# ChanukyaVardhan/Video-Moment-Localization

Measured on AMD Instinct MI355X. Metric: proposals/sec (fwd+bwd), higher is better.
Workload: dtype f32; 1 GPU; activitynet_t256: SMIN T=256 L=64 C=4 d=512 dl=128 Nq=20 Din=500 layers=3, batch 64/GPU, default init seed 43; step = zero_grad+fwd+restated loss+bwd+Adam (torch fused); global_batch=64, parallelism=dp1, dist_world_size=1

## Files before the change

### include/smin_hip.h

```cpp
#ifndef SMIN_HIP_H
#define SMIN_HIP_H
#include <stddef.h>
#include <stdint.h>

#ifdef __cplusplus
extern "C" {
#endif

#define SMIN_HIP_ABI_VERSION 2

int smin_abi_version(void);
int smin_set_gemm_mode(int mode);
int smin_get_gemm_mode(void);
#define SMIN_PROF_MOMENT_FWD 1
#define SMIN_PROF_MOMENT_DX 2
#define SMIN_PROF_MOMENT_DW 3
#define SMIN_PROF_ATTN_FWD 4
#define SMIN_PROF_ATTN_BWD 5
int smin_prof_enable(int on);
int smin_prof_read(int32_t* tags, float* ms, int cap);
const char* smin_target_arch(void);
size_t smin_workspace_bytes(int N, int B, int C, int D, int dl, int Nq);

int smin_proposal_map_fwd(void* stream, const float* f, const int32_t* cells, int N, int B, int T, int L, int C, int D,
                          float* fc, float* fm, float* fb, void* ws, size_t ws_bytes );
int smin_clip_event_table(void* stream, int T, int L, int C, int32_t* counts, const int32_t* offsets, void* table);
int smin_proposal_map_bwd(void* stream, const float* dfc, const float* dfm, const float* dfb,
                          const int32_t* cells, const int32_t* row_ptr, const int32_t* cellmap,
                          int N, int B, int T, int L, int C, int D, float* df, void* ws, size_t ws_bytes,
                          const int32_t* ev_offsets, const void* ev_table);

int smin_gate_fwd(void* stream, const float* fm, const float* fs, const int32_t* cells, int N, int D, float* hbar);
int smin_gate_fwd_sum(void* stream, const float* fm, const float* fs, const int32_t* cells, int N, int D, float* hbar, const float* hsum_in,
                      float* hsum_out);
int smin_gate_bwd(void* stream, const float* const* dhbar, int n_dhbar, const float* const* dres, int n_dres,
                  const float* fm, const float* fs, const int32_t* row_ptr,
                  int N, int B, int L, int D, float* dfm, float* dfs, void* ws, size_t ws_bytes,
                  const int32_t* cells, const float* boundary_A, const float* boundary_dout);

int smin_content_unit_fwd(void* stream, const float* fc, const float* hbar, const int32_t* cells, const int32_t* row_ptr,
                          int N, int B, int L, int C, int D, int dl, int Nq,
                          const float* Wch, const float* bch, const float* Mq, const float* uq,
                          const float* what, const float* shat, const float* qmask, const float* Wc, const float* bc,
                          const float* fcmean_in, int last,
                          float* fc_out, float* fcmean, float* chat, float* cchat);
int smin_content_unit_bwd(void* stream, const float* dfc_out, const float* dfcmean,
                          const float* fc, const int32_t* cells, const int32_t* row_ptr,
                          int N, int B, int L, int C, int D, int dl, int Nq,
                          const float* WchT, const float* Mq, const float* uq,
                          const float* what, const float* shat, const float* qmask, const float* WcT,
                          const float* chat, const float* cchat,
                          float* dfc, float* dhbar, float* dWch, float* dbch, float* dMq, float* duq,
                          float* dwhat, float* dshat, float* dWc, float* dbc, void* ws, size_t ws_bytes, int last);

int smin_boundary_reduce_fwd(void* stream, const float* Ab, const float* hbar, const int32_t* cells,
                             const int32_t* row_ptr, int N, int B, int L, int D, float* fbm);
int smin_boundary_reduce_bwd(void* stream, const float* dfbm, const float* Ab, const float* hbar,
                             const int32_t* cells, const int32_t* row_ptr, int N, int B, int L, int D,
                             float* dAb, float* dhbar);

int smin_boundary_unit_fwd(void* stream, const float* fb, const float* fw, const float* fs, const float* hbar,
                           const int32_t* cells, const int32_t* row_ptr, int N, int B, int L, int Nq, int D,
                           const float* Wq, const float* bq, const float* Wk, const float* bk,
                           const float* qmask, const float* lmask,
                           float* out, float* Qb, float* Kb, float* P, float* baq, float* bqv, float* A);
size_t smin_boundary_unit_bwd_ws_bytes(int B, int L, int Nq, int D);
int smin_boundary_unit_bwd(void* stream, const float* dout, const float* fb, const float* fw, const float* fs, const float* hbar,
                           const int32_t* cells, const int32_t* row_ptr, int N, int B, int L, int Nq, int D,
                           const float* WqT, const float* WkT, const float* qmask, const float* lmask,
                           const float* Qb, const float* Kb, const float* P, const float* baq, const float* bqv, const float* A,
                           float* dfb, float* dfw, float* dfs, float* dhbar, float* dWq, float* dbq, float* dWk, float* dbk,
                           void* ws, size_t ws_bytes);

int smin_moment_unit_fwd(void* stream, const float* fcmean, const float* fm, const float* fb, const int32_t* cells,
                         int N, int B, int L, int D, const float* Wcat, const float* bcat, float* mu,
                         const float* x1 );
int smin_pair_product(void* stream, const float* fb, const int32_t* cells, int N, int L, int D, float* x1);
int smin_moment_unit_bwd(void* stream, const float* dmu, const float* fcmean, const float* fb, const int32_t* cells,
                         const int32_t* row_ptr, const int32_t* cellmap, int N, int B, int L, int D, const float* WcatT,
                         float* dfcmean, float* dfb, float* dWcat, float* dbcat, void* ws, size_t ws_bytes,
                         int all_valid ,
                         const float* dfcmean_acc ,
                         const float* x1 ,
                         const float* dfb_acc );
int smin_pair_product_bf16(void* stream, const float* fb, const int32_t* cells, int N, int L, int D, uint16_t* x1h);
int smin_moment_unit_fwd_x1h(void* stream, const float* fcmean, const float* fm, const float* fb, const int32_t* cells,
                             int N, int B, int L, int D, const float* Wcat, const float* bcat, float* mu, const uint16_t* x1h);
int smin_moment_unit_bwd_x1h(void* stream, const float* dmu, const float* fcmean, const float* fb, const int32_t* cells,
                             const int32_t* row_ptr, const int32_t* cellmap, int N, int B, int L, int D, const float* WcatT,
                             float* dfcmean, float* dfb, float* dWcat, float* dbcat, void* ws, size_t ws_bytes,
                             int all_valid, const float* dfcmean_acc, const uint16_t* x1h, const float* dfb_acc);

int smin_score_map_fwd(void* stream, const float* fm, const float* fb, const int32_t* cells, int N, int B, int L, int D,
                       const float* wm, const float* bm, const float* wb, const float* bb, const float* lmask,
                       float* pm, float* psea);
size_t smin_score_tail_ws_bytes(int B, int L, int D, int dl);
int smin_score_tail_fwd(void* stream, const float* ccmean, const float* cumean, const float* hbar , const float* fm, const float* fs,
                        const float* bu, const int32_t* cells, int N, int B, int L, int D, int dl, const float* Wc, const float* bc,
                        const float* Wcat, const float* bcat, const float* wm, const float* bm, const float* wb ,
                        const float* bb , const float* lmask, float* pm, float* psea, void* ws, size_t ws_bytes);
int smin_score_map_bwd(void* stream, const float* dpm, const float* dpsea, const float* pm, const float* psea,
                       const float* fm, const float* fb, const int32_t* cells, int N, int B, int L, int D,
                       const float* wm, const float* wb, const float* lmask,
                       float* dfm, float* dfb, float* dwm, float* dbm, float* dwb, float* dbb, void* ws, size_t ws_bytes);

int smin_loss_fwd(void* stream, const float* pm, const uint8_t* ym, const float* sm, const uint8_t* mm,
                  const float* ps, const uint8_t* ys, const float* ss, const float* pe, const uint8_t* ye, const float* se,
                  const float* pa, const uint8_t* ya, const uint8_t* lm, int B, int L, float* loss, float* part);
int smin_loss_bwd(void* stream, const float* dloss, const float* part,
                  const float* pm, const uint8_t* ym, const float* sm, const uint8_t* mm,
                  const float* ps, const uint8_t* ys, const float* ss, const float* pe, const uint8_t* ye, const float* se,
                  const float* pa, const uint8_t* ya, const uint8_t* lm, int B, int L,
                  float* dpm, float* dps, float* dpe, float* dpa);

int smin_build_targets(void* stream, const float* times, const float* duration, const int32_t* nfeats, const int32_t* qlen, int B, int T, int L, int Nq,
                       uint8_t* video_mask, uint8_t* query_mask, uint8_t* length_mask, uint8_t* moment_mask, float* sm, uint8_t* ym,
                       float* ss, uint8_t* ys, float* se, uint8_t* ye, uint8_t* ya,
                       const float* two_sigma_sq );

int smin_sample_clips(void* stream, const float* raw, const int64_t* offsets, const int32_t* spos, int B, int T, int Din, int mode,
                      float* video_features, int32_t* nfeats);
int smin_sample_clips_bwd(void* stream, const float* dout, const int64_t* offsets, const int32_t* spos, int B, int T, int Din, int mode,
                          int64_t rows, float* draw);
int smin_sample_windows(void* stream, const float* raw, const int64_t* row_begin, const int32_t* len, int W, int T, int Din, int mode,
                        float* video_features, int32_t* nfeats);
// ... 28 lines not shown
                            int B, int L, int rule, int k, float nms_thresh, const int* n_list, int nn, const float* m_list, int nm,
                            const float* loss, double* acc, void* ws, size_t ws_bytes);

int smin_span_ious(void* stream, const float* span, const int32_t* count, const float* gt, int B, int k, float* iou);
size_t smin_span_meter_ws_bytes(int B, int nn, int nm);
int smin_span_meter_update(void* stream, const float* span, const int32_t* count, const float* gt, int B, int k,
                           const int* n_list, int nn, const float* m_list, int nm, double* acc, void* ws, size_t ws_bytes);

size_t smin_corpus_meter_ws_bytes(int Q, int nn, int nm);
int smin_corpus_meter_update(void* stream, const int64_t* video, const float* span, const int32_t* count, const int64_t* gt_video,
                             const float* gt, int Q, int k, const int* n_list, int nn, const float* m_list, int nm, double* acc,
                             void* ws, size_t ws_bytes);


int smin_clip_window_means_fwd(void* stream, const float* g, const float* bias , int bias_len,
                               const int32_t* cells, int N, int B, int T, int L, int C,
                               int W, int nseg, float* out, void* ws, size_t ws_bytes);
int smin_clip_window_means_bwd(void* stream, const float* const* dout, const int32_t* cells, const int32_t* row_ptr,
                               const int32_t* cellmap, int N, int B, int T, int L, int C, int W, int nseg, float* dg,
                               void* ws, size_t ws_bytes, const int32_t* ev_offsets, const void* ev_table);

int smin_content_attn_fwd(void* stream, const float* chat, const int32_t* cells, const int32_t* row_ptr,
                          int N, int B, int L, int C, int dl, int Nq,
                          const float* Mq, const float* uq, const float* what, const float* shat, const float* qmask,
                          float* cc, float* ccmean);
int smin_content_attn_fwd_cch(void* stream, const float* chat, const int32_t* cells, const int32_t* row_ptr,
                              int N, int B, int L, int C, int dl, int Nq,
                              const float* Mq, const float* uq, const float* what, const float* shat, const float* qmask,
                              uint16_t* cc_h, float* ccmean);
int smin_content_attn_fwd_probs(void* stream, const float* chat, const int32_t* cells, const int32_t* row_ptr,
                                int N, int B, int L, int C, int dl, int Nq,
                                const float* Mq, const float* uq, const float* what, const float* shat, const float* qmask,
                                void* cc, int cc_bf16, float* ccmean, float* probs);
int smin_content_attn_maps_dense(void* stream, const float* probs, const int32_t* cellmap, const int32_t* cells,
                                 int B, int L, int C, int dl, int Nq, const float* uq, const float* qmask, float* out);
#define SMIN_ATTN_MAPS_MAX_LAYERS 8
int smin_attn_maps_gather(void* stream, const float* const* probs, const float* const* bmaps, int nl, const int32_t* cellmap,
                          const int64_t* idx, int B, int L, int C, int Nq, int k, float* content, float* boundary);
size_t smin_content_attn_bwd_workspace_bytes(int N, int B, int C, int dl);
int smin_content_attn_bwd(void* stream, const float* dcc, const float* dccmean, const float* chat,
                          const int32_t* cells, const int32_t* row_ptr, int N, int B, int L, int C, int dl, int Nq,
                          const float* Mq, const float* uq, const float* what, const float* shat, const float* qmask,
                          float* dchat, float* dMq, float* duq, float* dwhat, float* dshat, void* ws, size_t ws_bytes);

int smin_linear_rows_fwd(void* stream, const float* const* xs, int nseg, const float* W, const float* bias, const float* add_rows,
                         const float* add_cells, int C, int R, int O, int K, float* y);
size_t smin_linear_rows_bwd_workspace_bytes(int R, int O, int Ktot);
int smin_linear_rows_bwd(void* stream, const float* dy, const float* const* xs, int nseg, const float* WT, int R, int O, int K,
                         float* const* dxs, float* dW, float* dbias, void* ws, size_t ws_bytes);
int smin_linear_rows_fwd_xh(void* stream, const uint16_t* const* xs, int nseg, const float* W, const float* bias, const float* add_rows,
                            const float* add_cells, int C, int R, int O, int K, float* y);
int smin_linear_rows_bwd_xh(void* stream, const float* dy, const uint16_t* const* xs, int nseg, int R, int O, int K,
                            float* dW, float* dbias, void* ws, size_t ws_bytes);
int smin_linear_rows_dx_acc(void* stream, const float* dy, int nseg, const float* WT, int R, int O, int K, float* const* dxs);
int smin_group_sum(void* stream, const float* x, int groups, int C, int W, float* out);

int smin_word_prep_fwd(void* stream, const float* fw, const float* fs, const float* qmask, const float* const* params, int nl, int B, int Nq, int D,
                       int dl, float* what, float* shat, float* kb, float* Mq, float* uq);
size_t smin_word_prep_bwd_workspace_bytes(int nl, int B, int Nq, int D, int dl);
int smin_word_prep_bwd(void* stream, const float* const* dwhat, const float* const* dshat, const float* const* dMq, const float* const* duq,
                       const float* fw, const float* fs, const float* qmask, const float* what, const float* kb, const float* const* params,
                       int nl, int B, int Nq, int D, int dl, float* dfw, float* dfs, float* const* dparams, void* ws, size_t ws_bytes);

int smin_video_encoder_fwd(void* stream, const float* x, const float* W, const float* bias, const float* pe, const float* vmask,
                           const float* fs, int B, int T, int Din, int D, float* fv, float* f);
int smin_video_encoder_gate(void* stream, const float* fv, const float* fs, int B, int T, int D, float* f);
size_t smin_video_encoder_bwd_workspace_bytes(int B, int T, int Din, int D);
int smin_video_encoder_bwd(void* stream, const float* df, const float* fv, const float* fs, const float* vmask, const float* x,
                           int B, int T, int Din, int D, float* dW, float* dbias, float* dpe, float* dfs, void* ws, size_t ws_bytes);
int smin_video_encoder_bwd_input(void* stream, const float* WT, const float* vmask, int B, int T, int Din, int D, float* dx,
                                 const void* ws, size_t ws_bytes);

int smin_sentence_feature_fwd(void* stream, const float* fw, const int32_t* len, int B, int Nq, int H, float* fs);
int smin_sentence_feature_bwd(void* stream, const float* dfs, const int32_t* len, int B, int Nq, int H, float* dfw);
int smin_lstm_pack(void* stream, const float* const* w, int In, int H, float* Wih, float* bias, float* Whh, float* W4);
int smin_lstm_pack_layers(void* stream, int nlayers, const float* const* w, const int* In, int H, float* const* Wih, float* const* bias,
                          float* const* Whh, float* const* W4);
int smin_bilstm_layer_fwd(void* stream, const float* X, const float* Wih_cat, const float* bias_cat, const float* W4,
                          const int32_t* len, int B, int Nq, int In, int H, float* G, float* Hout, float* Cs);
size_t smin_bilstm_layer_bwd_workspace_bytes(int B, int Nq, int In, int H);
int smin_bilstm_layer_bwd(void* stream, const float* dHout, const float* X, const float* Hout, const float* G, const float* Cs,
                          const float* Wih_catT, const float* Whh, const int32_t* len, int B, int Nq, int In, int H,
                          float* dX, float* dWih_cat, float* dbias_cat, float* dWhh, void* ws, size_t ws_bytes);
int smin_bilstm_layer_bwd_weights(void* stream, int which, const float* X, const float* Hout, int B, int Nq, int In, int H,
                                  float* dWih_cat, float* dbias_cat, float* dbias_cat2, float* dWhh, void* ws, size_t ws_bytes);

int smin_lstm_cluster_error(void);

int smin_build_cells(void* stream, const uint8_t* mask, int B, int L, int all_cells,
                     int32_t* cells, int32_t* row_ptr, int32_t* cellmap);
int smin_build_cells_n(void* stream, const uint8_t* mask, int B, int L, int all_cells, int n_expected,
                       int32_t* cells, int32_t* row_ptr, int32_t* cellmap, int32_t* status);

int smin_step_prologue(void* stream, const uint8_t* query_mask, const uint8_t* video_mask, const uint8_t* length_mask, const uint8_t* moment_mask,
                       const float* const* w, const float* const* b, int B, int Nq, int T, int L, int D, int32_t* len32, float* qmf, float* vmaskf,
                       float* lmf, float* wb, float* bb, int64_t* count, void* acc);

int smin_pack_cells(void* stream, const float* dense, const int32_t* cells, int N, int L, int W, float* packed);
int smin_unpack_cells(void* stream, const float* packed, const int32_t* cells, int N, int L, int W, float* dense );

int smin_param_prep_fwd(void* stream, const float* const* params, int nl, int D, int dl, float* const* Pcat, float* consts, float* Wcat,
                        float* bcat, float* Wch_all);
int smin_param_prep_bwd(void* stream, const float* const* params, int nl, int D, int dl, const float* const* dPcat, const float* dconsts,
                        const float* dWcat, const float* dbcat, const float* dWch_all, const float* const* dWch_base,
                        const float* const* dWc_base, const float* const* dbc_base, float* const* grads);

// ... 41 lines not shown
```

### video-moment-localization_amd/_lib.py

```python
import ctypes
import os
import subprocess

import torch

_HERE = os.path.dirname(os.path.abspath(__file__))
LIB_PATH = os.path.join(_HERE, "libsmin_hip.so")
TORCH_LIB_PATH = os.path.join(_HERE, "libsmin_torch.so")
CSRC = os.path.join(_HERE, "csrc")

_vp, _i, _sz, _f = ctypes.c_void_p, ctypes.c_int, ctypes.c_size_t, ctypes.c_float
_i64, _d = ctypes.c_int64, ctypes.c_double
ABI_VERSION = 2

SIGNATURES = {
    "smin_abi_version": [],
    "smin_target_arch": [],
    "smin_set_gemm_mode": [_i],
    "smin_get_gemm_mode": [],
    "smin_prof_enable": [_i],
    "smin_prof_read": [_vp, _vp, _i],
    "smin_workspace_bytes": [_i] * 6,
    "smin_transpose_batch": [_vp] * 5 + [_i],
    "smin_param_prep_fwd": [_vp, _vp, _i, _i, _i] + [_vp] * 5,
    "smin_param_prep_bwd": [_vp, _vp, _i, _i, _i] + [_vp] * 9,
    "smin_sum_lists": [_vp, _vp, _i, _sz, _vp],
    "smin_col_sum_workspace_bytes": [_i, _i],
    "smin_col_sum": [_vp, _vp, _i, _i, _vp, _vp, _sz],
    "smin_proposal_map_fwd": [_vp, _vp, _vp] + [_i] * 6 + [_vp] * 3 + [_vp, _sz],
    "smin_proposal_map_bwd": [_vp] * 7 + [_i] * 6 + [_vp, _vp, _sz, _vp, _vp],
    "smin_clip_event_table": [_vp] + [_i] * 3 + [_vp] * 3,
    "smin_gate_fwd": [_vp] * 4 + [_i] * 2 + [_vp],
    "smin_gate_fwd_sum": [_vp] * 4 + [_i] * 2 + [_vp] * 3,
    "smin_gate_bwd": [_vp, _vp, _i, _vp, _i, _vp, _vp, _vp] + [_i] * 4 + [_vp] * 2 + [_vp, _sz] + [_vp] * 3,
    "smin_content_unit_fwd": [_vp] * 5 + [_i] * 7 + [_vp] * 9 + [_vp, _i] + [_vp] * 4,
    "smin_content_unit_bwd": [_vp] * 6 + [_i] * 7 + [_vp] * 9 + [_vp] * 10 + [_vp, _sz, _i],
    "smin_boundary_reduce_fwd": [_vp] * 5 + [_i] * 4 + [_vp],
    "smin_boundary_reduce_bwd": [_vp] * 6 + [_i] * 4 + [_vp] * 2,
    "smin_boundary_unit_fwd": [_vp] * 7 + [_i] * 5 + [_vp] * 6 + [_vp] * 7,
    "smin_boundary_unit_bwd_ws_bytes": [_i] * 4,
    "smin_boundary_unit_bwd": [_vp] * 8 + [_i] * 5 + [_vp] * 4 + [_vp] * 6 + [_vp] * 8 + [_vp, _sz],
    "smin_moment_unit_fwd": [_vp] * 5 + [_i] * 4 + [_vp] * 3 + [_vp],
    "smin_pair_product": [_vp] * 3 + [_i] * 3 + [_vp],
    "smin_moment_unit_bwd": [_vp] * 7 + [_i] * 4 + [_vp] * 5 + [_vp, _sz, _i, _vp, _vp, _vp],
    "smin_pair_product_bf16": [_vp] * 3 + [_i] * 3 + [_vp],
    "smin_moment_unit_fwd_x1h": [_vp] * 5 + [_i] * 4 + [_vp] * 3 + [_vp],
    "smin_moment_unit_bwd_x1h": [_vp] * 7 + [_i] * 4 + [_vp] * 5 + [_vp, _sz, _i, _vp, _vp, _vp],
    "smin_score_map_fwd": [_vp] * 4 + [_i] * 4 + [_vp] * 7,
    "smin_score_map_bwd": [_vp] * 8 + [_i] * 4 + [_vp] * 3 + [_vp] * 6 + [_vp, _sz],
    "smin_score_tail_ws_bytes": [_i] * 4,
    "smin_score_tail_fwd": [_vp] * 8 + [_i] * 5 + [_vp] * 11 + [_vp, _sz],
    "smin_loss_fwd": [_vp] * 14 + [_i] * 2 + [_vp] * 2,
    "smin_loss_bwd": [_vp] * 16 + [_i] * 2 + [_vp] * 4,
    "smin_compute_ious": [_vp] * 6 + [_i] * 2 + [_vp] * 2,
    "smin_top_moments_ws_bytes": [_i] * 3,
    "smin_top_moments": [_vp] * 5 + [_i] * 3 + [_f] + [_vp] * 4 + [_sz],
    "smin_merge_window_moments": [_vp] * 7 + [_i] * 6 + [_f] + [_vp] * 5,
    "smin_compute_ious_nms_ws_bytes": [_i] * 5,
    "smin_compute_ious_nms": [_vp] * 6 + [_i] * 3 + [_f, _vp, _i, _vp, _i] + [_vp, _vp, _sz],
    "smin_epoch_meter_ws_bytes": [_i] * 6,
    "smin_epoch_meter_update": [_vp] * 6 + [_i] * 4 + [_f, _vp, _i, _vp, _i] + [_vp, _vp, _vp, _sz],
    "smin_span_ious": [_vp] * 4 + [_i] * 2 + [_vp],
    "smin_span_meter_ws_bytes": [_i] * 3,
    "smin_span_meter_update": [_vp] * 4 + [_i] * 2 + [_vp, _i, _vp, _i] + [_vp, _vp, _sz],
    "smin_build_targets": [_vp] * 5 + [_i] * 4 + [_vp] * 12,
    "smin_sample_clips": [_vp] * 4 + [_i] * 4 + [_vp] * 2,
    "smin_embed_tokens": [_vp] * 3 + [_i] * 5 + [_vp] * 3,
    "smin_sample_clips_bwd": [_vp] * 4 + [_i] * 4 + [ctypes.c_int64, _vp],
    "smin_sample_windows": [_vp] * 4 + [_i] * 4 + [_vp] * 2,
    "smin_embed_tokens_bwd_workspace_bytes": [_i, _i],
    "smin_embed_tokens_bwd": [_vp] * 3 + [_i] * 4 + [_vp, _vp, _sz],
    "smin_embed_tokens_bwd_rows_workspace_bytes": [_i, _i],
    "smin_embed_tokens_bwd_rows": [_vp] * 3 + [_i] * 4 + [_vp] * 4 + [_vp, _sz],
    "smin_word_prep_fwd": [_vp] * 5 + [_i] * 5 + [_vp] * 5,
    "smin_word_prep_bwd_workspace_bytes": [_i] * 5,
    "smin_word_prep_bwd": [_vp] * 11 + [_i] * 5 + [_vp] * 3 + [_vp, _sz],
    "smin_build_cells": [_vp, _vp, _i, _i, _i, _vp, _vp, _vp],
    "smin_build_cells_n": [_vp, _vp, _i, _i, _i, _i, _vp, _vp, _vp, _vp],
    "smin_pack_cells": [_vp, _vp, _vp, _i, _i, _i, _vp],
    "smin_unpack_cells": [_vp, _vp, _vp, _i, _i, _i, _vp],
    "smin_gemm_nt": [_vp] * 4 + [_i] * 3,
    "smin_gemm_nt_acc": [_vp] * 4 + [_i] * 3,
    "smin_clip_window_means_fwd": [_vp] * 3 + [_i, _vp] + [_i] * 7 + [_vp, _vp, _sz],
    "smin_clip_window_means_bwd": [_vp] * 5 + [_i] * 7 + [_vp, _vp, _sz, _vp, _vp],
    "smin_content_attn_fwd": [_vp] * 4 + [_i] * 6 + [_vp] * 7,
    "smin_content_attn_fwd_cch": [_vp] * 4 + [_i] * 6 + [_vp] * 7,
    "smin_content_attn_fwd_probs": [_vp] * 4 + [_i] * 6 + [_vp] * 6 + [_i, _vp, _vp],
    "smin_content_attn_maps_dense": [_vp] * 4 + [_i] * 5 + [_vp] * 3,
    "smin_attn_maps_gather": [_vp] * 3 + [_i] + [_vp] * 2 + [_i] * 5 + [_vp] * 2,
    "smin_content_attn_bwd_workspace_bytes": [_i] * 4,
    "smin_content_attn_bwd": [_vp] * 6 + [_i] * 6 + [_vp] * 10 + [_vp, _sz],
    "smin_linear_rows_fwd": [_vp, _vp, _i] + [_vp] * 4 + [_i] * 4 + [_vp],
    "smin_linear_rows_fwd_xh": [_vp, _vp, _i] + [_vp] * 4 + [_i] * 4 + [_vp],
    "smin_linear_rows_bwd_xh": [_vp, _vp, _vp, _i, _i, _i, _i, _vp, _vp, _vp, _sz],
    "smin_linear_rows_bwd_workspace_bytes": [_i] * 3,
    "smin_linear_rows_bwd": [_vp, _vp, _vp, _i, _vp] + [_i] * 3 + [_vp] * 3 + [_vp, _sz],
    "smin_linear_rows_dx_acc": [_vp, _vp, _i, _vp] + [_i] * 3 + [_vp],
    "smin_group_sum": [_vp, _vp, _i, _i, _i, _vp],
    "smin_video_encoder_fwd": [_vp] * 7 + [_i] * 4 + [_vp] * 2,
    "smin_video_encoder_gate": [_vp] * 3 + [_i] * 3 + [_vp],
    "smin_video_encoder_bwd_workspace_bytes": [_i] * 4,
    "smin_video_encoder_bwd": [_vp] * 6 + [_i] * 4 + [_vp] * 4 + [_vp, _sz],
    "smin_video_encoder_bwd_input": [_vp] * 3 + [_i] * 4 + [_vp, _vp, _sz],
    "smin_bilstm_layer_fwd": [_vp] * 6 + [_i] * 4 + [_vp] * 3,
    "smin_lstm_pack": [_vp, _vp, _i, _i] + [_vp] * 4,
    "smin_lstm_pack_layers": [_vp, _i, _vp, _vp, _i] + [_vp] * 4,
    "smin_lstm_cluster_error": [],
    "smin_sentence_feature_fwd": [_vp, _vp, _vp, _i, _i, _i, _vp],
    "smin_sentence_feature_bwd": [_vp, _vp, _vp, _i, _i, _i, _vp],
    "smin_bilstm_layer_bwd_workspace_bytes": [_i] * 4,
    "smin_bilstm_layer_bwd": [_vp] * 9 + [_i] * 4 + [_vp] * 4 + [_vp, _sz],
    "smin_step_prologue": [_vp] * 7 + [_i] * 5 + [_vp] * 8,
    "smin_bilstm_layer_bwd_weights": [_vp, _i, _vp, _vp] + [_i] * 4 + [_vp] * 4 + [_vp, _sz],
    "smin_adam_ws_bytes": [_i64, _i],
    "smin_grad_norm": [_vp, _vp, _vp, _i, _d, _vp, _vp, _sz],
    "smin_adam_step": [_vp] * 5 + [_i] + [_vp] * 3 + [_d] * 4 + [_i, _i, _vp],
    "smin_row_adam_step": [_vp] * 8 + [_i] * 3 + [_vp] * 2 + [_d] * 3 + [_i],
    "smin_row_lists_merge_workspace_bytes": [_i, _i],
    "smin_row_lists_merge": [_vp] * 5 + [_i] * 3 + [_vp] * 5 + [_vp, _sz],
    "smin_pair_assemble": [_vp] * 6 + [_i] * 6 + [_vp] * 3,
    "smin_corpus_topk": [_vp] * 6 + [_i] * 3 + [_vp] * 4,
    "smin_search_merge": [_vp, _i] + [_vp] * 6 + [_i] * 2 + [_vp] * 4,
    "smin_corpus_meter_ws_bytes": [_i] * 3,
    "smin_corpus_meter_update": [_vp] * 6 + [_i] * 2 + [_vp, _i, _vp, _i] + [_vp, _vp, _sz],
}
_RESTYPE = {"smin_target_arch": ctypes.c_char_p, "smin_workspace_bytes": _sz,
            "smin_content_attn_bwd_workspace_bytes": _sz, "smin_linear_rows_bwd_workspace_bytes": _sz,
            "smin_bilstm_layer_bwd_workspace_bytes": _sz, "smin_video_encoder_bwd_workspace_bytes": _sz, "smin_embed_tokens_bwd_workspace_bytes": _sz,
            "smin_embed_tokens_bwd_rows_workspace_bytes": _sz,
            "smin_word_prep_bwd_workspace_bytes": _sz, "smin_score_tail_ws_bytes": _sz,
            "smin_col_sum_workspace_bytes": _sz, "smin_top_moments_ws_bytes": _sz, "smin_boundary_unit_bwd_ws_bytes": _sz, "smin_compute_ious_nms_ws_bytes": _sz,
            "smin_epoch_meter_ws_bytes": _sz, "smin_span_meter_ws_bytes": _sz, "smin_adam_ws_bytes": _sz,
            "smin_row_lists_merge_workspace_bytes": _sz, "smin_corpus_meter_ws_bytes": _sz}

_lib = None
_ws = {}


class SminHipError(RuntimeError):
    pass


def build(verbose=False):
    res = subprocess.run(["make", "-C", CSRC, "-j8"], capture_output=True, text=True)
    if verbose or res.returncode != 0:
        print(res.stdout[-4000:])
        print(res.stderr[-4000:])
    if res.returncode != 0:
        raise SminHipError("building libsmin_hip.so failed (see output above)")
# ... 110 lines not shown
```

### video-moment-localization_amd/csrc/boundary_unit.hip

```cpp
#include "gemm.h"
#include "smin_hip.h"

namespace smin {

__global__ __launch_bounds__(128)
void boundary_reduce_fwd_kernel(const float* __restrict__ Ab, const float* __restrict__ hbar, const float* base,
                                const int* __restrict__ cells, const int* __restrict__ row_ptr, int L, int D, float* fbm)
{
    const int i = blockIdx.x, b = blockIdx.y;
    const int r0 = row_ptr[b * L + i], r1 = row_ptr[b * L + i + 1];
    const float* arow = Ab + ((size_t)b * L + i) * L;
    for (int d = threadIdx.x * 4; d < D; d += 512) {
        float4 acc = base ? ldg4(base + ((size_t)b * L + i) * D + d) : f4zero();
        for (int n = r0; n < r1; ++n)
            acc = f4fma(ldg4(hbar + (size_t)n * D + d), arow[cells[4 * (size_t)n + 2]], acc);
        stg4(fbm + ((size_t)b * L + i) * D + d, acc);
    }
}

__global__ __launch_bounds__(256)
void boundary_reduce_bwd_kernel(const float* __restrict__ dfbm, const float* __restrict__ Ab, const float* __restrict__ hbar,
                                const int* __restrict__ cells, const int* __restrict__ row_ptr,
                                int L, int D, float* __restrict__ dAb, float* __restrict__ dhbar)
{
    const int i = blockIdx.x, b = blockIdx.y;
    const int r0 = row_ptr[b * L + i], r1 = row_ptr[b * L + i + 1];
    const int wave = threadIdx.x >> 6, lane = threadIdx.x & 63;
    const float* arow = Ab + ((size_t)b * L + i) * L;
    float* darow = dAb + ((size_t)b * L + i) * L;
    for (int j = threadIdx.x; j < L; j += 256) darow[j] = 0.f;
    __syncthreads();
    for (int n = r0 + wave; n < r1; n += 4) {
        const int j = cells[4 * (size_t)n + 2];
        const float a = arow[j];
        float dot = 0.f;
        for (int d = lane * 4; d < D; d += 256) {
            const float4 dy = ldg4(dfbm + ((size_t)b * L + i) * D + d);
            const float4 x = ldg4(hbar + (size_t)n * D + d);
            dot = fmaf(dy.x, x.x, dot); dot = fmaf(dy.y, x.y, dot); dot = fmaf(dy.z, x.z, dot); dot = fmaf(dy.w, x.w, dot);
            if (dhbar) stg4(dhbar + (size_t)n * D + d, f4scale(dy, a));
        }
        dot = wave_sum(dot);
        if (lane == 0) darow[j] = dot;
    }
}


__device__ __forceinline__ float block_dot_row(const float* __restrict__ a, const float* __restrict__ b, int D, int lane)
{
    float s = 0.f;
    for (int d = lane * 4; d < D; d += 256) {
        const float4 x = ldg4(a + d), y = ldg4(b + d);
        s = fmaf(x.x, y.x, s); s = fmaf(x.y, y.y, s); s = fmaf(x.z, y.z, s); s = fmaf(x.w, y.w, s);
    }
    return wave_sum(s);
}

__device__ __forceinline__ float4 block_dot_row4(const float* __restrict__ a, const float* __restrict__ b0, const float* __restrict__ b1,
                                                 const float* __restrict__ b2, const float* __restrict__ b3, int D, int lane)
{
    float s0 = 0.f, s1 = 0.f, s2 = 0.f, s3 = 0.f;
    for (int d = lane * 4; d < D; d += 256) {
        const float4 x = ldg4(a + d), y0 = ldg4(b0 + d), y1 = ldg4(b1 + d), y2 = ldg4(b2 + d), y3 = ldg4(b3 + d);
        s0 = fmaf(x.x, y0.x, s0); s0 = fmaf(x.y, y0.y, s0); s0 = fmaf(x.z, y0.z, s0); s0 = fmaf(x.w, y0.w, s0);
        s1 = fmaf(x.x, y1.x, s1); s1 = fmaf(x.y, y1.y, s1); s1 = fmaf(x.z, y1.z, s1); s1 = fmaf(x.w, y1.w, s1);
        s2 = fmaf(x.x, y2.x, s2); s2 = fmaf(x.y, y2.y, s2); s2 = fmaf(x.z, y2.z, s2); s2 = fmaf(x.w, y2.w, s2);
        s3 = fmaf(x.x, y3.x, s3); s3 = fmaf(x.y, y3.y, s3); s3 = fmaf(x.z, y3.z, s3); s3 = fmaf(x.w, y3.w, s3);
    }
    return make_float4(wave_sum(s0), wave_sum(s1), wave_sum(s2), wave_sum(s3));
}

__device__ __forceinline__ void block_softmax(float* sv, int n, int t)
{
    __syncthreads();
    if (t < 64) {
        float mx = -INFINITY;
        for (int k = t; k < n; k += 64) mx = fmaxf(mx, sv[k]);
        for (int o = 32; o >= 1; o >>= 1) mx = fmaxf(mx, __shfl_xor(mx, o));
        float den = 0.f;
        for (int k = t; k < n; k += 64) { const float e = expf(sv[k] - mx); sv[k] = e; den += e; }
        den = wave_sum(den);
        const float inv = 1.0f / den;
        for (int k = t; k < n; k += 64) sv[k] *= inv;
    }
    __syncthreads();
}

__global__ __launch_bounds__(256)
void boundary_rows_fwd_kernel(const float* __restrict__ Qb, const float* __restrict__ Kb, const float* __restrict__ fw,
                              const float* __restrict__ fb, const float* __restrict__ fs, const float* __restrict__ qmask,
                              const float* __restrict__ lmask, int L, int Nq, int D, float scale,
// ... 161 lines not shown
        stg4(dfw + ((size_t)b * Nq + w) * D + d, f);
    }
}

struct EpBias {
    const float* bias; float* out;
    __device__ __forceinline__ void chunk(const float* Ws, int row0, int col0, int ncols, int M, int N, int lane) const {
        chunk_rows_f4(Ws, row0, col0, ncols, M, N, lane, [&](int row, int col, float4 v) {
            stg4(out + (size_t)row * N + col, f4add(v, ldg4(bias + col)));
        });
    }
};
struct EpAccum {
    float* out;
    __device__ __forceinline__ void chunk(const float* Ws, int row0, int col0, int ncols, int M, int N, int lane) const {
        chunk_rows_f4(Ws, row0, col0, ncols, M, N, lane, [&](int row, int col, float4 v) {
            float* o = out + (size_t)row * N + col;
            stg4(o, f4add(v, ldg4(o)));
        });
    }
};

__global__ __launch_bounds__(256)
void rows_reduce_kernel(const float* __restrict__ partial, int L, int rows_per_slice, int D, float* __restrict__ out)
{
    __shared__ float4 sh[4][64];
    const int b = blockIdx.z, sl = blockIdx.y, c = threadIdx.x & 63, g = threadIdx.x >> 6;
    const int d = (blockIdx.x * 64 + c) * 4;
    const int r0 = sl * rows_per_slice, r1 = min(L, r0 + rows_per_slice);
    float4 s = f4zero();
    if (d < D) {
        const float* p = partial + (size_t)b * L * D + d;
        int i = r0 + g;
        for (; i + 12 < r1; i += 16) {
            const float4 a0 = ldg4(p + (size_t)i * D), a1 = ldg4(p + (size_t)(i + 4) * D), a2 = ldg4(p + (size_t)(i + 8) * D), a3 = ldg4(p + (size_t)(i + 12) * D);
            s = f4add(f4add(f4add(f4add(s, a0), a1), a2), a3);
        }
        for (; i < r1; i += 4) s = f4add(s, ldg4(p + (size_t)i * D));
    }
    sh[g][c] = s;
    __syncthreads();
    if (g == 0 && d < D) stg4(out + ((size_t)b * gridDim.y + sl) * D + d, f4add(f4add(sh[0][c], sh[1][c]), f4add(sh[2][c], sh[3][c])));
}

}

using namespace smin;

extern "C" int smin_boundary_reduce_fwd(void* stream, const float* Ab, const float* hbar, const int32_t* cells,
                                        const int32_t* row_ptr, int N, int B, int L, int D, float* fbm)
{
    (void)N;
    SMIN_REQUIRE(D % 4 == 0);
    hipLaunchKernelGGL(boundary_reduce_fwd_kernel, dim3(L, B), dim3(128), 0, (hipStream_t)stream, Ab, hbar, nullptr, cells, row_ptr, L, D, fbm);
    SMIN_LAUNCH_CHECK();
    return 0;
}

extern "C" int smin_boundary_reduce_bwd(void* stream, const float* dfbm, const float* Ab, const float* hbar,
                                        const int32_t* cells, const int32_t* row_ptr, int N, int B, int L, int D,
                                        float* dAb, float* dhbar)
{
    (void)N;
    hipStream_t st = (hipStream_t)stream;
    SMIN_REQUIRE(D % 4 == 0);
    hipLaunchKernelGGL(boundary_reduce_bwd_kernel, dim3(L, B), dim3(256), 0, st, dfbm, Ab, hbar, cells, row_ptr, L, D, dAb, dhbar);
    SMIN_LAUNCH_CHECK();
    return 0;
}


constexpr int BU_MAX_L = 8192;

static size_t bu_fwd_saved_floats(int B, int L, int Nq, int D)
{
    return (size_t)B * L * D * 3 + (size_t)B * Nq * D + (size_t)B * L * Nq + (size_t)B * L * L;
}

struct BuBwdWs {
    int sp1, sp2, slices;
    size_t dAbm, draw, dbaq_lm, dfs_part, dQK, dQb, dKb, mid, slab1, bslab1, slab2, bslab2, end;
    BuBwdWs(int B, int L, int Nq, int D)
        : sp1(tn_splits(B * L, D, D)), sp2(tn_splits(B * Nq, D, D)), slices(L > 96 ? cdiv(L, 32) : 1)
    {
        size_t off = 0;
        auto take = [&](size_t n) { const size_t o = off; off += (n + 3) & ~(size_t)3; return o; };
        dAbm = take((size_t)B * L * L);
        draw = take((size_t)B * L * L);
        dbaq_lm = take((size_t)B * L * D);
        dfs_part = take((size_t)B * L * D);
        dQK = take((size_t)B * L * Nq);
        dQb = take((size_t)B * L * D);
        dKb = take((size_t)B * Nq * D);
        mid = take(slices > 1 ? (size_t)B * slices * D : 0);
        slab1 = take((size_t)sp1 * D * D); bslab1 = take((size_t)sp1 * D);
        slab2 = take((size_t)sp2 * D * D); bslab2 = take((size_t)sp2 * D);
        end = off;
    }
};

extern "C" int smin_boundary_unit_fwd(void* stream, const float* fb, const float* fw, const float* fs, const float* hbar,
                                      const int32_t* cells, const int32_t* row_ptr, int N, int B, int L, int Nq, int D,
                                      const float* Wq, const float* bq, const float* Wk, const float* bk,
                                      const float* qmask, const float* lmask,
                                      float* out, float* Qb, float* Kb, float* P, float* baq, float* bqv, float* A)
{
    (void)N;
    hipStream_t st = (hipStream_t)stream;
    SMIN_REQUIRE(D % 4 == 0 && Nq >= 1 && Nq <= 64 && L >= 1 && L <= BU_MAX_L);
    const float scale = 1.0f / sqrtf((float)D);
    int rc = launch_gemm_nt(st, PlainMat{fb, D}, PlainMat{Wq, D}, EpBias{bq, Qb}, B * L, D, D);
    if (rc) return rc;
    rc = launch_gemm_nt(st, PlainMat{fw, D}, PlainMat{Wk, D}, EpBias{bk, Kb}, B * Nq, D, D);
    if (rc) return rc;
    hipLaunchKernelGGL(boundary_rows_fwd_kernel, dim3(L, B), dim3(256), 0, st, Qb, Kb, fw, fb, fs, qmask, lmask, L, Nq, D, scale, P, baq, bqv);
    SMIN_LAUNCH_CHECK();
    hipLaunchKernelGGL(boundary_self_fwd_kernel, dim3(L, B), dim3(256), sizeof(float) * L, st, bqv, fb, lmask, L, D, scale, A, out);
    SMIN_LAUNCH_CHECK();
    hipLaunchKernelGGL(boundary_reduce_fwd_kernel, dim3(L, B), dim3(128), 0, st, A, hbar, out, cells, row_ptr, L, D, out);
    SMIN_LAUNCH_CHECK();
    return 0;
}

extern "C" size_t smin_boundary_unit_bwd_ws_bytes(int B, int L, int Nq, int D)
{
    if (B < 1 || L < 1 || L > BU_MAX_L || Nq < 1 || Nq > 64 || D < 4 || D % 4 != 0) return 0;
    return BuBwdWs(B, L, Nq, D).end * sizeof(float);
}

extern "C" int smin_boundary_unit_bwd(void* stream, const float* dout, const float* fb, const float* fw, const float* fs, const float* hbar,
                                      const int32_t* cells, const int32_t* row_ptr, int N, int B, int L, int Nq, int D,
                                      const float* WqT, const float* WkT, const float* qmask, const float* lmask,
                                      const float* Qb, const float* Kb, const float* P, const float* baq, const float* bqv, const float* A,
                                      float* dfb, float* dfw, float* dfs, float* dhbar, float* dWq, float* dbq, float* dWk, float* dbk,
                                      void* ws, size_t ws_bytes)
{
    (void)N;
    hipStream_t st = (hipStream_t)stream;
    SMIN_REQUIRE(D % 4 == 0 && Nq >= 1 && Nq <= 64 && L >= 1 && L <= BU_MAX_L);
    const float scale = 1.0f / sqrtf((float)D);
    const BuBwdWs lay(B, L, Nq, D);
    SMIN_REQUIRE(lay.end * sizeof(float) <= ws_bytes);
    float* w = reinterpret_cast<float*>(ws);
    float* dAbm = w + lay.dAbm;
    float* draw = w + lay.draw;
    float* dbaq_lm = w + lay.dbaq_lm;
    float* dfs_part = w + lay.dfs_part;
    float* dQK = w + lay.dQK;
    float* dQb = w + lay.dQb;
    float* dKb = w + lay.dKb;
    const int sp1 = lay.sp1, sp2 = lay.sp2;
    float* slab1 = w + lay.slab1; float* bslab1 = w + lay.bslab1;
    float* slab2 = w + lay.slab2; float* bslab2 = w + lay.bslab2;
    const size_t cols_lds = sizeof(float) * (2 * (size_t)L + 64);
    if (cols_lds > 48 * 1024)
        if (int e = lds_optin(reinterpret_cast<const void*>(boundary_self_bwd_cols_kernel), cols_lds)) return e;

    hipLaunchKernelGGL(boundary_reduce_bwd_kernel, dim3(L, B), dim3(256), 0, st, dout, A, hbar, cells, row_ptr, L, D, dAbm, dhbar);
    SMIN_LAUNCH_CHECK();
    hipLaunchKernelGGL(boundary_self_bwd_rows_kernel, dim3(L, B), dim3(256), sizeof(float) * L, st, dout, dAbm, A, fb, lmask, L, D, scale, draw);
    SMIN_LAUNCH_CHECK();
    hipLaunchKernelGGL(boundary_self_bwd_cols_kernel, dim3(L, B), dim3(256), cols_lds, st, dout, draw, A, bqv, baq, fb, fs, fw, Kb,
                       P, qmask, lmask, L, Nq, D, scale, dfb, dbaq_lm, dfs_part, dQK, dQb);
    SMIN_LAUNCH_CHECK();
    {
        const int slices = lay.slices;
        if (slices == 1) {
            hipLaunchKernelGGL(rows_reduce_kernel, dim3(cdiv(D, 256), 1, B), dim3(256), 0, st, dfs_part, L, L, D, dfs);
        } else {
            float* mid = w + lay.mid;
            hipLaunchKernelGGL(rows_reduce_kernel, dim3(cdiv(D, 256), slices, B), dim3(256), 0, st, dfs_part, L, 32, D, mid);
            SMIN_LAUNCH_CHECK();
            hipLaunchKernelGGL(rows_reduce_kernel, dim3(cdiv(D, 256), 1, B), dim3(256), 0, st, mid, slices, slices, D, dfs);
        }
    }
    SMIN_LAUNCH_CHECK();
    hipLaunchKernelGGL(boundary_words_bwd_kernel, dim3(Nq, B), dim3(256), 0, st, dQK, P, Qb, dbaq_lm, L, Nq, D, dKb, dfw);
    SMIN_LAUNCH_CHECK();
    int rc = launch_gemm_nt(st, PlainMat{dQb, D}, PlainMat{WqT, D}, EpAccum{dfb}, B * L, D, D); if (rc) return rc;
    rc = launch_gemm_tn(st, PlainMat{dQb, D}, PlainMat{fb, D}, slab1, bslab1, B * L, D, D, sp1); if (rc) return rc;
    rc = launch_reduce_slabs2(st, slab1, dWq, D * D, bslab1, dbq, D, sp1); if (rc) return rc;
    rc = launch_gemm_nt(st, PlainMat{dKb, D}, PlainMat{WkT, D}, EpAccum{dfw}, B * Nq, D, D); if (rc) return rc;
    rc = launch_gemm_tn(st, PlainMat{dKb, D}, PlainMat{fw, D}, slab2, bslab2, B * Nq, D, D, sp2); if (rc) return rc;
    rc = launch_reduce_slabs2(st, slab2, dWk, D * D, bslab2, dbk, D, sp2); if (rc) return rc;
    return 0;
}
```

### video-moment-localization_amd/csrc/common.h

```cpp
#pragma once
#include <hip/hip_runtime.h>
#include <stdint.h>

typedef float f32x16 __attribute__((ext_vector_type(16)));

#define SMIN_LAUNCH_CHECK()                                  \
    do {                                                     \
        hipError_t e__ = hipGetLastError();                  \
        if (e__ != hipSuccess) return (int)e__;              \
    } while (0)

#define SMIN_REQUIRE(cond)                                   \
    do {                                                     \
        if (!(cond)) return -1000 - __LINE__;                \
    } while (0)

namespace smin {
extern volatile int g_prof_on;
void prof_record(hipStream_t st, int tag, bool begin);
struct ProfScope {
    hipStream_t st; int tag; bool on;
    ProfScope(hipStream_t s, int t) : st(s), tag(t), on(g_prof_on != 0) { if (on) prof_record(st, tag, true); }
    ~ProfScope() { if (on) prof_record(st, tag, false); }
};
// ... 23 lines not shown
    if (mc > 512) mc = 512;
    if (mc < 1) mc = 1;
    const int cpc = cdiv(max_cells, mc);
    *cells_per_chunk = cpc;
    *max_chunks = cdiv(max_cells, cpc);
}

struct Cell { int b, i, j, m; };

__device__ __forceinline__ Cell load_cell(const int* __restrict__ cells, int n) {
    const int4 v = *reinterpret_cast<const int4*>(cells + 4 * (size_t)n);
    Cell c; c.b = v.x; c.i = v.y; c.j = v.z; c.m = v.w; return c;
}

__device__ __forceinline__ float sigmoidf_(float x) { return 1.0f / (1.0f + __expf(-x)); }

template <int CTRL, int ROW_MASK>
__device__ __forceinline__ float dpp_f(float v) {
    return __int_as_float(__builtin_amdgcn_update_dpp(0, __float_as_int(v), CTRL, ROW_MASK, 0xF, false));
}
__device__ __forceinline__ float wave_sum(float v) {
    v += dpp_f<0xB1, 0xF>(v);
    v += dpp_f<0x4E, 0xF>(v);
    v += dpp_f<0x141, 0xF>(v);
    v += dpp_f<0x140, 0xF>(v);
    v += dpp_f<0x142, 0xA>(v);
    v += dpp_f<0x143, 0xC>(v);
    return __int_as_float(__builtin_amdgcn_readlane(__float_as_int(v), 63));
}
__device__ __forceinline__ float half_sum(float v) {
    v += dpp_f<0xB1, 0xF>(v);
    v += dpp_f<0x4E, 0xF>(v);
    v += dpp_f<0x141, 0xF>(v);
    v += dpp_f<0x140, 0xF>(v);
    v += __shfl_xor(v, 16);
    return v;
}
__device__ __forceinline__ float half_max(float v) {
    v = fmaxf(v, __shfl_xor(v, 1));
    v = fmaxf(v, __shfl_xor(v, 2));
    v = fmaxf(v, __shfl_xor(v, 4));
    v = fmaxf(v, __shfl_xor(v, 8));
    v = fmaxf(v, __shfl_xor(v, 16));
    return v;
}

__device__ __forceinline__ float4 f4zero() { return make_float4(0.f, 0.f, 0.f, 0.f); }
__device__ __forceinline__ float4 f4add(float4 a, float4 b) { return make_float4(a.x + b.x, a.y + b.y, a.z + b.z, a.w + b.w); }
__device__ __forceinline__ float4 f4mul(float4 a, float4 b) { return make_float4(a.x * b.x, a.y * b.y, a.z * b.z, a.w * b.w); }
__device__ __forceinline__ float4 f4scale(float4 a, float s) { return make_float4(a.x * s, a.y * s, a.z * s, a.w * s); }
__device__ __forceinline__ float4 f4fma(float4 a, float s, float4 c) { return make_float4(fmaf(a.x, s, c.x), fmaf(a.y, s, c.y), fmaf(a.z, s, c.z), fmaf(a.w, s, c.w)); }
__device__ __forceinline__ float4 ldg4(const float* p) { return *reinterpret_cast<const float4*>(p); }
__device__ __forceinline__ void stg4(float* p, float4 v) { *reinterpret_cast<float4*>(p) = v; }
```

### video-moment-localization_amd/csrc/gate.hip

```cpp
#include "common.h"
#include "smin_hip.h"

namespace smin {

template <bool SUM>
__global__ void gate_fwd_kernel(const float* __restrict__ fm, const float* __restrict__ fs, const int* __restrict__ cells,
                                int N, int D4, float* __restrict__ hbar, const float* __restrict__ hsum_in, float* __restrict__ hsum_out)
{
    const size_t idx = (size_t)blockIdx.x * blockDim.x + threadIdx.x;
    if (idx >= (size_t)N * D4) return;
    const size_t n = idx / D4; const int d4 = (int)(idx % D4);
    const int b = cells[4 * n];
    const float4 x = ldg4(fm + idx * 4), s = ldg4(fs + ((size_t)b * D4 + d4) * 4);
    const float4 h = make_float4(x.x / (1.0f + expf(-x.x * s.x)), x.y / (1.0f + expf(-x.y * s.y)),
                                 x.z / (1.0f + expf(-x.z * s.z)), x.w / (1.0f + expf(-x.w * s.w)));
    stg4(hbar + idx * 4, h);
    if (SUM) stg4(hsum_out + idx * 4, f4add(ldg4(hsum_in + idx * 4), h));
}

struct GradList { const float* p[4]; int n; };

__device__ __forceinline__ float4 grad_sum(const GradList& g, size_t off) {
    float4 v = ldg4(g.p[0] + off);
    if (g.n > 1) v = f4add(v, ldg4(g.p[1] + off));
    if (g.n > 2) v = f4add(v, ldg4(g.p[2] + off));
    if (g.n > 3) v = f4add(v, ldg4(g.p[3] + off));
    return v;
}

__global__ __launch_bounds__(128)
void gate_bwd_kernel(GradList dh, GradList dres, const float* __restrict__ fm, const float* __restrict__ fs,
                     const int* __restrict__ row_ptr, int L, int D, int cells_per_chunk, int max_chunks,
                     float* __restrict__ dfm, float* __restrict__ partial,
                     const int* __restrict__ cells, const float* __restrict__ bA, const float* __restrict__ dbm)
{
    const int b = blockIdx.y, chunk = blockIdx.x;
    const int s0 = row_ptr[b * L], s1 = row_ptr[(b + 1) * L];
    const int n_begin = s0 + chunk * cells_per_chunk;
    if (n_begin >= s1) return;
    const int n_end = min(s1, n_begin + cells_per_chunk);
    for (int d = threadIdx.x * 4; d < D; d += 512) {
        const float4 s4 = ldg4(fs + (size_t)b * D + d);
        float4 acc = f4zero();
        for (int n0 = n_begin; n0 < n_end; n0 += 4) {
            float4 ds[4], x[4], dr[4];
#pragma unroll
            for (int u = 0; u < 4; ++u) {
                const int nn = min(n0 + u, n_end - 1);
                const size_t off = (size_t)nn * D + d;
                ds[u] = grad_sum(dh, off);
                if (bA) {
                    const int ci = cells[4 * (size_t)nn + 1], cj = cells[4 * (size_t)nn + 2];
                    const float a = bA[((size_t)b * L + ci) * L + cj];
                    ds[u] = f4fma(ldg4(dbm + ((size_t)b * L + ci) * D + d), a, ds[u]);
                }
                x[u] = ldg4(fm + off);
                dr[u] = dres.n > 0 ? grad_sum(dres, off) : f4zero();
            }
#pragma unroll
            for (int u = 0; u < 4; ++u) {
                if (n0 + u >= n_end) break;
                float4 o;
#define GATE1(F)                                                                  \
                {                                                                 \
                    const float g = 1.0f / (1.0f + expf(-x[u].F * s4.F));         \
                    const float gg = g * (1.0f - g);                              \
                    o.F = ds[u].F * (g + x[u].F * gg * s4.F);                     \
                    acc.F = fmaf(ds[u].F, x[u].F * x[u].F * gg, acc.F);           \
// ... 79 lines not shown
```

### video-moment-localization_amd/csrc/linear_rows.hip

```cpp
#include "gemm.h"
#include "smin_hip.h"

namespace smin {

template <bool HAS_BIAS, bool HAS_ROWS, bool HAS_CELLS>
struct EpLinearRows {
    const float* bias; const float* add_rows; const float* add_cells; int C; float* out;
    struct Add { float4 r, c; };
    __device__ __forceinline__ void chunk(const float* Ws, int row0, int col0, int ncols, int M, int N, int lane) const {
        chunk_rows_f4_pre<Add>(Ws, row0, col0, ncols, M, N, lane,
            [&](int row, int col) {
                Add a;
                a.r = HAS_ROWS ? ldg4(add_rows + (size_t)row * N + col) : f4zero();
                a.c = HAS_CELLS ? ldg4(add_cells + (size_t)(row / C) * N + col) : f4zero();
                return a;
            },
            [&](int row, int col, float4 v, const Add& a) {
                if (HAS_BIAS) v = f4add(v, ldg4(bias + col));
                if (HAS_ROWS) v = f4add(v, a.r);
                if (HAS_CELLS) v = f4add(v, a.c);
                stg4(out + (size_t)row * N + col, v);
            });
    }
};
template <bool ACC = false>
struct EpStoreRows {
    float* out;
    __device__ __forceinline__ void chunk(const float* Ws, int row0, int col0, int ncols, int M, int N, int lane) const {
        chunk_rows_f4(Ws, row0, col0, ncols, M, N, lane, [&](int row, int col, float4 v) {
            float* o = out + (size_t)row * N + col;
            stg4(o, ACC ? f4add(v, ldg4(o)) : v);
        });
    }
};

template <bool ACC = false>
struct EpSplitCols {
    float* out[4]; int w;
    __device__ __forceinline__ void chunk(const float* Ws, int row0, int col0, int ncols, int M, int N, int lane) const {
        chunk_rows_f4(Ws, row0, col0, ncols, M, N, lane, [&](int row, int col, float4 v) {
            const int sg = (col >= w) + (col >= 2 * w) + (col >= 3 * w);
            float* q = sg == 0 ? out[0] : sg == 1 ? out[1] : sg == 2 ? out[2] : out[3];
            float* o = q + (size_t)row * w + (col - sg * w);
            stg4(o, ACC ? f4add(v, ldg4(o)) : v);
        });
    }
};

__global__ void group_sum_kernel(const float* __restrict__ x, float* __restrict__ out, size_t groups, int C, int W4)
{
    const size_t idx = (size_t)blockIdx.x * blockDim.x + threadIdx.x;
    if (idx >= groups * W4) return;
    const size_t g = idx / W4; const int d4 = (int)(idx % W4);
    float4 s = f4zero();
    for (int c = 0; c < C; ++c) s = f4add(s, ldg4(x + ((g * C + c) * W4 + d4) * 4));
    stg4(out + idx * 4, s);
}

}

using namespace smin;

static CatMat cat_of(const float* const* xs, int nseg, int K)
{
    CatMat m;
    for (int k = 0; k < 4; ++k) m.p[k] = xs[k < nseg ? k : 0];
    m.w = K;
    return m;
}

extern "C" int smin_linear_rows_fwd(void* stream, const float* const* xs, int nseg, const float* W, const float* bias, const float* add_rows,
                                    const float* add_cells, int C, int R, int O, int K, float* y)
{
    SMIN_REQUIRE(O % 4 == 0 && K % 4 == 0 && C >= 1 && nseg >= 1 && nseg <= 4);
    if (R == 0) return 0;
    hipStream_t st = (hipStream_t)stream;
    auto run = [&](auto ep) {
        if (nseg == 1) return launch_gemm_nt(st, PlainMat{xs[0], K}, PlainMat{W, K}, ep, R, O, K);
        return launch_gemm_nt(st, cat_of(xs, nseg, K), PlainMat{W, nseg * K}, ep, R, O, nseg * K);
    };
    if (!add_rows && !add_cells) return bias ? run(EpLinearRows<true, false, false>{bias, add_rows, add_cells, C, y})
                                             : run(EpLinearRows<false, false, false>{bias, add_rows, add_cells, C, y});
    if (add_rows && add_cells) return bias ? run(EpLinearRows<true, true, true>{bias, add_rows, add_cells, C, y})
                                           : run(EpLinearRows<false, true, true>{bias, add_rows, add_cells, C, y});
    if (add_rows) return bias ? run(EpLinearRows<true, true, false>{bias, add_rows, add_cells, C, y})
                              : run(EpLinearRows<false, true, false>{bias, add_rows, add_cells, C, y});
    return bias ? run(EpLinearRows<true, false, true>{bias, add_rows, add_cells, C, y})
                : run(EpLinearRows<false, false, true>{bias, add_rows, add_cells, C, y});
}

extern "C" size_t smin_linear_rows_bwd_workspace_bytes(int R, int O, int Ktot)
{
    const int sp = R > 0 ? tn_splits(R, O, Ktot) : 1;
    return sizeof(float) * ((size_t)sp * O * Ktot + (size_t)sp * O + 64);
}

extern "C" int smin_linear_rows_bwd(void* stream, const float* dy, const float* const* xs, int nseg, const float* WT, int R, int O, int K,
                                    float* const* dxs, float* dW, float* dbias, void* ws, size_t ws_bytes)
{
    hipStream_t st = (hipStream_t)stream;
    SMIN_REQUIRE(O % 4 == 0 && K % 4 == 0 && nseg >= 1 && nseg <= 4);
    const int Kt = nseg * K;
    if (R == 0) {
        if (dW) (void)hipMemsetAsync(dW, 0, sizeof(float) * (size_t)O * Kt, st);
        if (dW && dbias) (void)hipMemsetAsync(dbias, 0, sizeof(float) * (size_t)O, st);
        return 0;
    }
    SMIN_REQUIRE(ws_bytes >= smin_linear_rows_bwd_workspace_bytes(R, O, Kt));
    SMIN_REQUIRE(dW != nullptr || dbias == nullptr);
    int rc;
    if (dxs) {
        if (nseg == 1) {
            rc = launch_gemm_nt(st, PlainMat{dy, O}, PlainMat{WT, O}, EpStoreRows<false>{dxs[0]}, R, K, O);
        } else {
            EpSplitCols<false> ep;
            for (int k = 0; k < 4; ++k) ep.out[k] = dxs[k < nseg ? k : 0];
            ep.w = K;
            rc = launch_gemm_nt(st, PlainMat{dy, O}, PlainMat{WT, O}, ep, R, Kt, O);
        }
        if (rc) return rc;
    }
    if (!dW) return 0;
    const int sp = tn_splits(R, O, Kt);
    float* slab = reinterpret_cast<float*>(ws);
    float* bslab = slab + (size_t)sp * O * Kt;
    if (nseg == 1) rc = launch_gemm_tn(st, PlainMat{dy, O}, PlainMat{xs[0], K}, slab, bslab, R, O, Kt, sp);
    else rc = launch_gemm_tn(st, PlainMat{dy, O}, cat_of(xs, nseg, K), slab, bslab, R, O, Kt, sp);
    if (rc) return rc;
    rc = launch_reduce_slabs2(st, slab, dW, O * Kt, bslab, dbias, O, sp); if (rc) return rc;
    return 0;
}

static CatMatH cat_of_h(const uint16_t* const* xs, int nseg, int K)
{
    CatMatH m;
    for (int k = 0; k < 4; ++k) m.p[k] = xs[k < nseg ? k : 0];
    m.w = K;
    return m;
}

extern "C" int smin_linear_rows_fwd_xh(void* stream, const uint16_t* const* xs, int nseg, const float* W, const float* bias, const float* add_rows,
                                       const float* add_cells, int C, int R, int O, int K, float* y)
{
// ... 55 lines not shown
```

### video-moment-localization_amd/csrc/score_tail.hip

```cpp
#include "common.h"
#include "smin_hip.h"

namespace smin {

constexpr int TAIL_COLS = 64;
constexpr int TAIL_CPW = 8;

__device__ __forceinline__ void column_dots(const float* __restrict__ M, int rows, int ld, int cols, int col0, const float* __restrict__ v,
                                            float* __restrict__ out, float (*part)[TAIL_COLS])
{
    const int lc = threadIdx.x & (TAIL_COLS - 1), g = threadIdx.x / TAIL_COLS, col = col0 + lc;
    float s = 0.f;
    if (col < cols)
        for (int r = g; r < rows; r += 16) s = fmaf(M[(size_t)r * ld + col], v[r], s);
    part[g][lc] = s;
    __syncthreads();
    if (g == 0 && col < cols) {
        float t = part[0][lc];
        for (int k = 1; k < 16; ++k) t += part[k][lc];
        out[col] = t;
    }
    __syncthreads();
}

__global__ __launch_bounds__(1024)
void tail_vectors_kernel(const float* __restrict__ Wcat, const float* __restrict__ wm, int D, float* __restrict__ ac)
{
    __shared__ float part[16][TAIL_COLS];
    column_dots(Wcat, D, 2 * D, 2 * D, blockIdx.x * TAIL_COLS, wm, ac, part);
}

__global__ __launch_bounds__(1024)
void tail_consts_kernel(const float* __restrict__ Wc, const float* __restrict__ bc, const float* __restrict__ bcat, const float* __restrict__ wm,
                        const float* __restrict__ bm, int D, int dl, const float* __restrict__ c, float* __restrict__ u, float* __restrict__ k0)
{
    __shared__ float part[16][TAIL_COLS];
    for (int col0 = 0; col0 < dl; col0 += TAIL_COLS) column_dots(Wc, D, dl, dl, col0, c, u, part);
    if (threadIdx.x < 64) {
        float s = 0.f;
        for (int d = threadIdx.x; d < D; d += 64) { s = fmaf(bc[d], c[d], s); s = fmaf(wm[d], bcat[d], s); }
        s = wave_sum(s);
        if (threadIdx.x == 0) k0[0] = s + bm[0];
    }
}

__device__ __forceinline__ float4 gate4(float4 x, float4 s)
{
    return make_float4(x.x / (1.0f + expf(-x.x * s.x)), x.y / (1.0f + expf(-x.y * s.y)), x.z / (1.0f + expf(-x.z * s.z)), x.w / (1.0f + expf(-x.w * s.w)));
}
__device__ __forceinline__ float tail_dot4(float acc, float4 a, float4 c, float4 w, float4 bi, float4 bj, float4 q, float4 h, float4 x)
{
    acc = fmaf(a.x, bi.x * bj.x, acc); acc = fmaf(c.x, q.x + h.x, acc); acc = fmaf(w.x, x.x, acc);
    acc = fmaf(a.y, bi.y * bj.y, acc); acc = fmaf(c.y, q.y + h.y, acc); acc = fmaf(w.y, x.y, acc);
    acc = fmaf(a.z, bi.z * bj.z, acc); acc = fmaf(c.z, q.z + h.z, acc); acc = fmaf(w.z, x.z, acc);
    acc = fmaf(a.w, bi.w * bj.w, acc); acc = fmaf(c.w, q.w + h.w, acc); acc = fmaf(w.w, x.w, acc);
    return acc;
}
__device__ __forceinline__ float dot4(float acc, float4 u, float4 x)
{
    acc = fmaf(u.x, x.x, acc); acc = fmaf(u.y, x.y, acc); acc = fmaf(u.z, x.z, acc); acc = fmaf(u.w, x.w, acc);
    return acc;
}

template <int NV, bool HBAR>
__global__ __launch_bounds__(256)
void score_tail_kernel(const float* __restrict__ ccmean, const float* __restrict__ cumean, const float* __restrict__ hbar, const float* __restrict__ fm,
                       const float* __restrict__ fs, const float* __restrict__ bu, const int* __restrict__ cells, int N, int L, int D, int dl,
                       const float* __restrict__ ac, const float* __restrict__ u, const float* __restrict__ k0p, const float* __restrict__ wm,
                       float* __restrict__ pm)
{
    const int lane = threadIdx.x & 63;
    const int n0 = (blockIdx.x * 4 + (threadIdx.x >> 6)) * TAIL_CPW;
    if (n0 >= N) return;
    const int n1 = min(N, n0 + TAIL_CPW);
    const float k0 = k0p[0];
    constexpr int NR = NV > 0 ? NV : 1;
    float4 a4[NR], c4[NR], w4[NR], u4 = f4zero();
    if (NV > 0) {
#pragma unroll
        for (int v = 0; v < NR; ++v) {
            const int d = lane * 4 + v * 256;
            const bool ok = d < D;
            a4[v] = ok ? ldg4(ac + d) : f4zero(); c4[v] = ok ? ldg4(ac + D + d) : f4zero(); w4[v] = ok ? ldg4(wm + d) : f4zero();
        }
        if (lane * 4 < dl) u4 = ldg4(u + lane * 4);
    }
    for (int n = n0; n < n1; ++n) {
        const Cell cl = load_cell(cells, n);
        const float* __restrict__ bi = bu + ((size_t)cl.b * L + cl.i) * D;
        const float* __restrict__ bj = bu + ((size_t)cl.b * L + cl.j) * D;
        const float* __restrict__ sb = fs + (size_t)cl.b * D;
        const size_t row = (size_t)n * D;
        float acc = 0.f;
        if (NV > 0) {
#pragma unroll
            for (int v = 0; v < NR; ++v) {
                const int d = lane * 4 + v * 256;
                if (d < D) {
                    const float4 x = ldg4(fm + row + d);
                    const float4 h = HBAR ? ldg4(hbar + row + d) : gate4(x, ldg4(sb + d));
                    acc = tail_dot4(acc, a4[v], c4[v], w4[v], ldg4(bi + d), ldg4(bj + d), ldg4(cumean + row + d), h, x);
                }
// ... 79 lines not shown
```

### video-moment-localization_amd/csrc/torch_binding.cpp

```cpp
#include <ATen/ATen.h>
#include <c10/hip/HIPGuard.h>
#include <c10/hip/HIPStream.h>
#include <hip/hip_runtime_api.h>
#include <torch/csrc/autograd/custom_function.h>
#include <torch/library.h>
#include <ATen/core/dispatch/Dispatcher.h>
#include <ATen/core/stack.h>

#include <cmath>
#include <map>
#include <mutex>
#include <tuple>
#include <vector>

#include "smin_hip.h"

namespace {

using at::Tensor;
using torch::autograd::AutogradContext;
using torch::autograd::variable_list;
using HStream = c10::hip::HIPStream;

#define SMIN_CK(call)                                                                           \
// ... 257 lines not shown
    if (ts.size() == 1) return ts[0];
    const float* p[SMIN_BATCH_MAX];
    for (size_t k = 0; k < ts.size(); ++k) { TORCH_CHECK(ts[k].is_contiguous() && ts[k].numel() == ts[0].numel(), "sum_list: shapes differ"); p[k] = fp(ts[k]); }
    Tensor out = at::empty_like(ts[0]);
    SMIN_CK(smin_sum_lists(cur(), p, i32(ts.size()), (size_t)ts[0].numel(), fpm(out)));
    return out;
}

struct PairBank { Tensor fv, fw, fs, vi, qi; };

std::pair<Tensor, Tensor> query_encoder(LstmState (&lstm)[2], const std::vector<Tensor>& all, const Tensor& query_features, const Tensor& len32, int64_t maxq,
                                        int64_t H, bool scoring)
{
    const auto opt = query_features.options();
    Tensor x = cont(query_features);
    const int64_t Bq = x.size(0), Nq_in = x.size(1);
    const int B = i32(Bq);
    Tensor lstm_bias[2], lstm_W4[2];
    {
        const float* raw[16]; int ins[2]; float *wih[2], *bs[2], *whh[2], *w4[2];
        for (int layer = 0; layer < 2; ++layer) {
            LstmState& ls = lstm[layer];
            const int64_t In = layer == 0 ? x.size(2) : 2 * H;
            ls.Wih = at::empty({8 * H, In}, opt);
            lstm_bias[layer] = at::empty({8 * H}, opt);
            ls.Whh = at::empty({2, 4 * H, H}, opt);
            lstm_W4[layer] = at::empty({2, H, H, 4}, opt);
            for (int q = 0; q < 8; ++q) raw[8 * layer + q] = fp(all[P_LSTM + 8 * layer + q]);
            ins[layer] = i32(In); wih[layer] = fpm(ls.Wih); bs[layer] = fpm(lstm_bias[layer]); whh[layer] = fpm(ls.Whh); w4[layer] = fpm(lstm_W4[layer]);
        }
        SMIN_CK(smin_lstm_pack_layers(cur(), 2, raw, ins, i32(H), wih, bs, whh, w4));
    }
    for (int layer = 0; layer < 2; ++layer) {
        LstmState& ls = lstm[layer];
        const int In = i32(x.size(2)), Hh = i32(H);
        ls.x = x;
        const Tensor &bias = lstm_bias[layer], &W4 = lstm_W4[layer];
        ls.G = at::empty({Bq, Nq_in, 2, 4 * H}, opt); ls.Hout = at::empty({Bq, Nq_in, 2 * H}, opt); ls.Cs = at::empty({Bq, Nq_in, 2, H}, opt);
        SMIN_CK(smin_bilstm_layer_fwd(cur(), fp(x), fp(ls.Wih), fp(bias), fp(W4), ip(len32), B, i32(Nq_in), In, Hh, fpm(ls.G), fpm(ls.Hout), fpm(ls.Cs)));
        x = ls.Hout;
    }
    if (scoring)
        for (auto& l : lstm) { l.G = Tensor(); l.Cs = Tensor(); }
    Tensor fw = x;
    if (Nq_in < maxq) fw = at::constant_pad_nd(fw, {0, 0, 0, maxq - Nq_in}, 0);
    fw = fw.contiguous();
    Tensor fs = at::empty({Bq, 2 * H}, opt);
    SMIN_CK(smin_sentence_feature_fwd(cur(), fp(fw), ip(len32), B, i32(fw.size(1)), i32(H), fpm(fs)));
    return {fw, fs};
}

struct SminCore : torch::autograd::Function<SminCore> {
    enum { F_OVERLAP_BOUNDARY = 1, F_OVERLAP_PREP = 2, F_ASYNC_WEIGHTS = 4, F_BF16_OPERANDS = 8, F_GRAD_SYNC = 16, F_TAIL_SPLIT = 32, F_KEEP_ATTENTION = 64,
           F_ATTN_PACKED = 128, F_INPUT_GRADS = 256, F_PARAM_PREP_KERNEL = 512 };
    enum { N_FIXED = 14 };

    static int64_t run(CoreState& st, std::vector<Tensor>& all, std::vector<Tensor>& cmaps, std::vector<Tensor>& bmaps, bool scoring, const Tensor& video_features,
                       const Tensor& video_mask, const Tensor& query_features, const Tensor& query_mask, const Tensor& length_mask, const Tensor& moment_mask, int64_t T,
                       int64_t L, int64_t C, int64_t nl, int64_t maxq, int64_t H, int64_t flags, int64_t n_known, at::TensorList prm_in, const PairBank* bank = nullptr)
    {
        TORCH_CHECK(!bank || scoring, "banks are scored, not trained through");
        for (const Tensor& p : prm_in) all.push_back(cont(p));
        std::vector<Tensor> prm(all.begin() + P_LAYER0, all.end());
        const at::Device dev = bank ? bank->fv.device() : video_features.device();
        const auto opt = bank ? bank->fv.options() : video_features.options();
        const int64_t Bq = bank ? bank->vi.size(0) : video_features.size(0), Tn = bank ? bank->fv.size(1) : video_features.size(1);
        TORCH_CHECK(Tn == T, "ProposalGeneration was built for T=", T, " but got ", Tn, " frames");
        const int B = i32(Bq), D = i32(all[P_VE_W].size(0)), Nq = i32(maxq), dl = i32(prm[L_CH_W].size(0)), Li = i32(L), Ci = i32(C), Ti = i32(T);
        auto lp = [&](int64_t k, int which) -> const Tensor& { return prm[k * L_COUNT + which]; };
        const Tensor* loc = &prm[nl * L_COUNT];
        HStream curs = c10::hip::getCurrentHIPStream(dev.index());
        HStream side = (flags & F_OVERLAP_BOUNDARY) ? side_stream(dev.index()) : curs;
        HStream prep = (flags & F_OVERLAP_PREP) ? side : curs;
        size_state(st, nl);

        auto mark = [](HStream on) { hipEvent_t e = next_event(); TORCH_CHECK(hipEventRecord(e, on.stream()) == hipSuccess, "hipEventRecord failed"); return e; };
        auto await = [](HStream waiter, hipEvent_t e) { TORCH_CHECK(hipStreamWaitEvent(waiter.stream(), e, 0) == hipSuccess, "hipStreamWaitEvent failed"); };
        std::vector<Tensor> bcat(nl);
        Tensor bb;
        hipEvent_t products_ready;
        const bool prep_kernel = (flags & F_PARAM_PREP_KERNEL) != 0;
        wait_stream(prep, curs);
        {
            StreamScope sc(prep);
            if (prep_kernel) {
                Tensor consts_all = at::empty({nl, dl}, opt), Wcat_all = at::empty({nl, D, 2 * D}, opt), bcat_all = at::empty({nl, D}, opt);
                st.Wch_all = at::empty({nl * dl, D}, opt);
                std::vector<const float*> pp;
                std::vector<float*> pc(nl * 2, nullptr);
                for (int64_t k = 0; k < nl; ++k) {
                    for (int which : {L_CH_W, L_CH_B, L_C_W, L_C_B, L_FB_W, L_FB_B, L_FC_W, L_FC_B}) pp.push_back(fp(lp(k, which)));
                    LayerState& ls = st.layer[k];
                    for (int64_t lo = 0; lo < k; lo += 4) {
                        ls.Pcat[lo / 4] = at::empty({dl, std::min<int64_t>(4, k - lo) * dl}, opt);
                        pc[k * 2 + lo / 4] = fpm(ls.Pcat[lo / 4]);
                    }
                    ls.consts = consts_all[k]; ls.Wcat = Wcat_all[k]; bcat[k] = bcat_all[k];
                }
                SMIN_CK(smin_param_prep_fwd(cur(), pp.data(), i32(nl), D, dl, pc.data(), fpm(consts_all), fpm(Wcat_all), fpm(bcat_all), fpm(st.Wch_all)));
            } else {
                Tensor bsum;
                std::vector<Tensor> wch;
                for (int64_t k = 0; k < nl; ++k) {
                    LayerState& ls = st.layer[k];
                    ls.consts = bsum.defined() ? lp(k, L_CH_B) + at::mv(lp(k, L_CH_W), bsum) : lp(k, L_CH_B);
                    bsum = bsum.defined() ? bsum + lp(k, L_C_B) : lp(k, L_C_B);
                    wch.push_back(lp(k, L_CH_W));
// ... 83 lines not shown
        const int64_t N = n_known < 0 ? host_n.const_data_ptr<int64_t>()[0] : n_known;
        const int n = i32(N);
        Tensor cells, row_ptr, cellmap;
        Tensor mask8 = mm.contiguous().view(at::kByte);
        hipEvent_t layout_ready;
        if (prep != curs) await(prep, count_ready);
        {
            StreamScope sc(prep);
            auto io = at::TensorOptions().dtype(at::kInt).device(dev);
            cells = at::empty({N, 4}, io); row_ptr = at::empty({Bq * L + 1}, io); cellmap = at::empty({Bq, L, L}, io);
            if (n_known < 0)
                SMIN_CK(smin_build_cells(cur(), static_cast<const uint8_t*>(mask8.const_data_ptr()), B, Li, 0, cells.data_ptr<int32_t>(), row_ptr.data_ptr<int32_t>(),
                                         cellmap.data_ptr<int32_t>()));
            else
                SMIN_CK(smin_build_cells_n(cur(), static_cast<const uint8_t*>(mask8.const_data_ptr()), B, Li, 0, n, cells.data_ptr<int32_t>(), row_ptr.data_ptr<int32_t>(),
                                           cellmap.data_ptr<int32_t>(), layout_status(dev).data_ptr<int32_t>()));
            layout_ready = mark(prep);
        }
        st.f = f; st.fw = fw; st.fs = fs; st.qmf = qmf; st.lmf = lmf; st.cells = cells; st.row_ptr = row_ptr; st.cellmap = cellmap;

        hipEvent_t words_ready;
        wait_stream(prep, curs);
        {
            StreamScope sc(prep);
            std::vector<const float*> pp;
            for (int64_t k = 0; k < nl; ++k)
                for (int which : {L_WH_W, L_WH_B, L_SH_W, L_SH_B, L_AK_W, L_AK_B, L_AQ_W, L_AQ_B}) pp.push_back(fp(lp(k, which)));
            st.what = at::empty({nl, B, Nq, dl}, opt); st.kb = at::empty({nl, B, Nq, dl}, opt); st.Mq = at::empty({nl, B, Nq, dl}, opt);
            st.shat = at::empty({nl, B, dl}, opt); st.uq = at::empty({nl, B, Nq}, opt);
            SMIN_CK(smin_word_prep_fwd(cur(), fp(fw), fp(fs), fp(qmf), pp.data(), i32(nl), B, Nq, D, dl, fpm(st.what), fpm(st.shat), fpm(st.kb), fpm(st.Mq), fpm(st.uq)));
            words_ready = mark(prep);
        }
        if (prep != curs) { await(curs, products_ready); await(curs, layout_ready); }

        Tensor fm = at::empty({N, D}, opt), fb = at::empty({B, L, D}, opt);
        {
            auto ws = scratch((size_t)8 * B * (T + 1) * std::max<int64_t>(D, nl * dl), dev);
            SMIN_CK(smin_proposal_map_fwd(cur(), fp(f), ip(cells), n, B, Ti, Li, Ci, D, nullptr, fpm(fm), fpm(fb), ws.p, ws.n));
        }
        Tensor pgs = at::empty({nl, N * C, dl}, opt);
        {
            Tensor g_all = at::empty({(int64_t)B * T, nl * dl}, opt);
            const float* xs[1] = {fp(f)};
            SMIN_CK(smin_linear_rows_fwd(cur(), xs, 1, fp(st.Wch_all), nullptr, nullptr, nullptr, 1, i32(B * T), i32(nl * dl), D, fpm(g_all)));
            auto ws = scratch((size_t)8 * B * (T + 1) * std::max<int64_t>(D, nl * dl), dev);
            SMIN_CK(smin_clip_window_means_fwd(cur(), fp(g_all), fp(st.layer[0].consts), dl, ip(cells), n, B, Ti, Li, Ci, dl, i32(nl), fpm(pgs), ws.p, ws.n));
        }

        Tensor cumean = fm, Hs;
        const bool bf16_operands = (flags & F_BF16_OPERANDS) && smin_get_gemm_mode() == 2;
        const bool cc_bf16 = bf16_operands && dl % 8 == 0;
        const bool keep_maps = (flags & F_KEEP_ATTENTION) != 0;
        TORCH_CHECK(!(scoring && keep_maps), "smin_score keeps no attention maps");
        for (int64_t k = 0; k < nl; ++k) {
            LayerState& ls = st.layer[k];
            const bool lastl = k == nl - 1;
            ls.fm = fm; ls.fb = fb;
            ls.hbar = at::empty_like(fm);
            ls.Hs = Hs;
            if (k > 0 && !lastl && N > 0) {
                Tensor Hs_next = at::empty_like(fm);
                SMIN_CK(smin_gate_fwd_sum(cur(), fp(fm), fp(fs), ip(cells), n, D, fpm(ls.hbar), fp(Hs), fpm(Hs_next)));
                Hs = Hs_next;
            } else {
                SMIN_CK(smin_gate_fwd(cur(), fp(fm), fp(fs), ip(cells), n, D, fpm(ls.hbar)));
                if (!lastl) Hs = Hs.defined() ? Hs + ls.hbar : ls.hbar;
            }
            Tensor bmap = keep_maps ? at::empty({B, L, Nq}, opt) : Tensor();
            wait_stream(side, curs);
            {
                StreamScope sc(side);
                ls.bu = at::empty_like(fb); ls.Qb = at::empty_like(fb); ls.baq = at::empty_like(fb); ls.bqv = at::empty_like(fb); ls.Kb = at::empty_like(fw);
                ls.P = at::empty({B, L, Nq}, opt); ls.A = at::empty({B, L, L}, opt);
                SMIN_CK(smin_boundary_unit_fwd(cur(), fp(fb), fp(fw), fp(fs), fp(ls.hbar), ip(cells), ip(row_ptr), n, B, Li, Nq, D, fp(lp(k, L_BQ_W)), fp(lp(k, L_BQ_B)),
                                               fp(lp(k, L_BK_W)), fp(lp(k, L_BK_B)), fp(qmf), fp(lmf), fpm(ls.bu), fpm(ls.Qb), fpm(ls.Kb), fpm(ls.P), fpm(ls.baq),
                                               fpm(ls.bqv), fpm(ls.A)));
                if (keep_maps)
                    TORCH_CHECK(hipMemcpyAsync(bmap.data_ptr(), ls.P.const_data_ptr(), sizeof(float) * ls.P.numel(), hipMemcpyDeviceToDevice, side.stream()) == hipSuccess,
                                "hipMemcpyAsync failed");
            }
            if (keep_maps) bmaps.push_back(bmap);
            Tensor chat = pgs[k];
            const Tensor& Hs_k = ls.Hs;
            for (int64_t part = 0, lo = 0; lo < k; ++part, lo += 4) {
                Tensor hp;
                if (lo == 0) {
                    hp = at::empty({N, dl}, opt);
                    const float* xs[1] = {fp(Hs_k)};
                    SMIN_CK(smin_linear_rows_fwd(cur(), xs, 1, fp(lp(k, L_CH_W)), nullptr, nullptr, nullptr, 1, n, dl, D, fpm(hp)));
                }
                const int nseg = i32(std::min<int64_t>(4, k - lo));
                Tensor y = at::empty({N * C, dl}, opt);
                if (cc_bf16) {
                    const uint16_t* xh[4];
                    for (int sgm = 0; sgm < nseg; ++sgm) xh[sgm] = hp16(st.layer[lo + sgm].cc);
                    SMIN_CK(smin_linear_rows_fwd_xh(cur(), xh, nseg, fp(ls.Pcat[part]), lo == 0 ? fp(ls.consts) : nullptr, fp(chat), fp(hp), Ci, i32(N * C), dl, dl, fpm(y)));
                } else {
                    const float* xs[4];
                    for (int sgm = 0; sgm < nseg; ++sgm) xs[sgm] = fp(st.layer[lo + sgm].cc);
                    SMIN_CK(smin_linear_rows_fwd(cur(), xs, nseg, fp(ls.Pcat[part]), lo == 0 ? fp(ls.consts) : nullptr, fp(chat), fp(hp), Ci, i32(N * C), dl, dl, fpm(y)));
                }
                chat = y;
            }
            ls.chat = chat;
            if (k == 0 && prep != curs) await(curs, words_ready);
            ls.cc = at::empty({lastl ? 0 : N * C, dl}, cc_bf16 ? opt.dtype(at::kBFloat16) : opt); ls.ccmean = at::empty({N, dl}, opt);
            if (keep_maps) {
                Tensor probs = at::empty({N * C, (int64_t)Nq}, opt);
                SMIN_CK(smin_content_attn_fwd_probs(cur(), fp(chat), ip(cells), ip(row_ptr), n, B, Li, Ci, dl, Nq, fp(st.Mq[k]), fp(st.uq[k]), fp(st.what[k]),
                                                    fp(st.shat[k]), fp(qmf), lastl ? nullptr : ls.cc.data_ptr(), cc_bf16 && !lastl ? 1 : 0, fpm(ls.ccmean), fpm(probs)));
                if (flags & F_ATTN_PACKED) {
                    cmaps.push_back(probs);
                } else {
                    Tensor dense = at::empty({Bq, L, L, C, (int64_t)Nq}, opt);
                    SMIN_CK(smin_content_attn_maps_dense(cur(), fp(probs), ip(cellmap), ip(cells), B, Li, Ci, dl, Nq, fp(st.uq[k]), fp(qmf), fpm(dense)));
                    cmaps.push_back(dense);
                }
            } else if (cc_bf16 && !lastl)
                SMIN_CK(smin_content_attn_fwd_cch(cur(), fp(chat), ip(cells), ip(row_ptr), n, B, Li, Ci, dl, Nq, fp(st.Mq[k]), fp(st.uq[k]), fp(st.what[k]), fp(st.shat[k]),
                                                  fp(qmf), reinterpret_cast<uint16_t*>(ls.cc.data_ptr()), fpm(ls.ccmean)));
            else
                SMIN_CK(smin_content_attn_fwd(cur(), fp(chat), ip(cells), ip(row_ptr), n, B, Li, Ci, dl, Nq, fp(st.Mq[k]), fp(st.uq[k]), fp(st.what[k]), fp(st.shat[k]), fp(qmf),
                                              lastl ? nullptr : fpm(ls.cc), fpm(ls.ccmean)));
            if (scoring && lastl) {
                wait_stream(curs, side);
                st.pm = at::empty({B, L, L}, opt); st.psea = at::empty({3, B, L}, opt);
                SMIN_CK(smin_score_tail_fwd(cur(), fp(ls.ccmean), fp(cumean), nullptr, fp(fm), fp(fs), fp(ls.bu), ip(cells), n, B, Li, D, dl, nullptr, nullptr, nullptr,
                                            nullptr, fp(loc[0]), nullptr, fp(st.wb), fp(bb), fp(lmf), fpm(st.pm), fpm(st.psea), st.tailv.data_ptr(),
                                            (size_t)st.tailv.numel()));
                break;
            }
            ls.cum = at::empty({N, D}, opt);
            {
                const float* xs[1] = {fp(ls.ccmean)};
                SMIN_CK(smin_linear_rows_fwd(cur(), xs, 1, fp(lp(k, L_C_W)), fp(lp(k, L_C_B)), fp(cumean), fp(ls.hbar), 1, n, D, dl, fpm(ls.cum)));
            }
            wait_stream(curs, side);
            const bool x1h = bf16_operands;
            Tensor mu = at::empty_like(fm);
            if (!scoring) ls.x1 = x1h ? at::empty({N, D}, opt.dtype(at::kBFloat16)) : at::empty_like(fm);
            if (scoring) {
                SMIN_CK(smin_moment_unit_fwd(cur(), fp(ls.cum), fp(fm), fp(ls.bu), ip(cells), n, B, Li, D, fp(ls.Wcat), fp(bcat[k]), fpm(mu), nullptr));
            } else if (x1h) {
                uint16_t* xh = reinterpret_cast<uint16_t*>(ls.x1.data_ptr());
                SMIN_CK(smin_pair_product_bf16(cur(), fp(ls.bu), ip(cells), n, Li, D, xh));
                SMIN_CK(smin_moment_unit_fwd_x1h(cur(), fp(ls.cum), fp(fm), fp(ls.bu), ip(cells), n, B, Li, D, fp(ls.Wcat), fp(bcat[k]), fpm(mu), xh));
            } else {
                SMIN_CK(smin_pair_product(cur(), fp(ls.bu), ip(cells), n, Li, D, fpm(ls.x1)));
                SMIN_CK(smin_moment_unit_fwd(cur(), fp(ls.cum), fp(fm), fp(ls.bu), ip(cells), n, B, Li, D, fp(ls.Wcat), fp(bcat[k]), fpm(mu), fp(ls.x1)));
            }
            fm = mu; cumean = ls.cum; fb = ls.bu;
            if (scoring) {
                LayerState keep;
                keep.cc = ls.cc;
                ls = keep;
            }
        }
        if (scoring) return N;
        Tensor pm = at::empty({B, L, L}, opt), psea = at::empty({3, B, L}, opt);
        SMIN_CK(smin_score_map_fwd(cur(), fp(fm), fp(fb), ip(cells), n, B, Li, D, fp(loc[0]), fp(loc[1]), fp(st.wb), fp(bb), fp(lmf), fpm(pm), fpm(psea)));
        st.pm = pm; st.psea = psea; st.fm_out = fm;
        return N;
    }

    static variable_list forward(AutogradContext* ctx, Tensor video_features, Tensor video_mask, Tensor query_features, Tensor query_mask, Tensor length_mask,
                                 Tensor moment_mask, int64_t T, int64_t L, int64_t C, int64_t nl, int64_t maxq, int64_t H, int64_t flags, int64_t n_known,
                                 at::TensorList prm_in)
    {
        CoreState st;
        std::vector<Tensor> all, cmaps, bmaps;
        const int64_t N = run(st, all, cmaps, bmaps, false, video_features, video_mask, query_features, query_mask, length_mask, moment_mask, T, L, C, nl, maxq, H, flags,
                              n_known, prm_in);
        const bool keep_maps = (flags & F_KEEP_ATTENTION) != 0;
        const int64_t Nq_in = query_features.size(1);
        const Tensor &pm = st.pm, &psea = st.psea, &cellmap = st.cellmap;

        variable_list flat;
        visit_state(st, [&](Tensor& t) { flat.push_back(t); });
        for (auto& p : all) flat.push_back(p);
        ctx->save_for_backward(flat);
        ctx->saved_data["d"] = std::vector<int64_t>{N, T, L, C, nl, flags, H, Nq_in};
        if (!keep_maps) return {pm, psea[0], psea[1], psea[2]};
        if (flags & F_ATTN_PACKED) cmaps.push_back(cellmap.clone());
        variable_list out{pm, psea[0], psea[1], psea[2]};
        for (auto& t : cmaps) out.push_back(t);
        for (auto& t : bmaps) out.push_back(t);
        ctx->mark_non_differentiable(variable_list(out.begin() + 4, out.end()));
        return out;
    }

    static variable_list backward(AutogradContext* ctx, variable_list g)
    {
        auto d = ctx->saved_data["d"].toIntVector();
        const int64_t N = d[0], T = d[1], L = d[2], C = d[3], nl = d[4], flags = d[5], H = d[6], Nq_in = d[7];
        const bool prep_kernel = (flags & F_PARAM_PREP_KERNEL) != 0;
        auto sv = ctx->get_saved_variables();
        CoreState st;
        size_state(st, nl);
        size_t cursor = 0;
        visit_state(st, [&](Tensor& t) { t = sv[cursor++]; });
        std::vector<Tensor> all(sv.begin() + cursor, sv.end());
        std::vector<Tensor> prm(all.begin() + P_LAYER0, all.end());
        auto lp = [&](int64_t k, int which) -> const Tensor& { return prm[k * L_COUNT + which]; };
        const Tensor* loc = &prm[nl * L_COUNT];
        const Tensor &f = st.f, &fw = st.fw, &fs = st.fs, &qmf = st.qmf, &lmf = st.lmf, &cells = st.cells, &row_ptr = st.row_ptr, &cellmap = st.cellmap;
        const at::Device dev = f.device();
        const auto opt = f.options();
        const int B = i32(f.size(0)), D = i32(f.size(2)), Nq = i32(fw.size(1)), dl = i32(prm[L_CH_W].size(0)), n = i32(N), Li = i32(L), Ci = i32(C), Ti = i32(T);
        HStream curs = c10::hip::getCurrentHIPStream(dev.index());
        HStream side = (flags & F_OVERLAP_BOUNDARY) ? side_stream(dev.index()) : curs;
        HStream wstr = (flags & F_ASYNC_WEIGHTS) ? weight_stream(dev.index()) : curs;
        std::vector<Tensor> keep;
        GradSync sync;
        sync.on = (flags & F_GRAD_SYNC) != 0;
        TORCH_CHECK(!sync.on || prep_kernel, "smin_forward: the in-node gradient exchange needs param_prep_kernel (SMIN._param_prep_kernel)");
        const bool want_dx = (flags & F_INPUT_GRADS) && ctx->needs_input_grad(0), want_dX = (flags & F_INPUT_GRADS) && ctx->needs_input_grad(2);
        TORCH_CHECK(!sync.on || !grad_sync_config().group.empty(), "smin_forward: grad_sync requested but no process group was set (smin_hip::set_grad_sync)");
        std::vector<Tensor> dprm(prm.size());
        auto dlp = [&](int64_t k, int which) -> Tensor& { return dprm[k * L_COUNT + which]; };
        auto acc = [](Tensor& into, const Tensor& t) { if (into.defined()) into.add_(t); else into = t; };

        enum { TR_CH = 0, TR_C, TR_CAT, TR_BQ, TR_BK, TR_PER_LAYER };
        std::vector<Tensor> tr_in;
        for (int64_t k = 0; k < nl; ++k) {
            tr_in.push_back(lp(k, L_CH_W)); tr_in.push_back(lp(k, L_C_W)); tr_in.push_back(st.layer[k].Wcat); tr_in.push_back(lp(k, L_BQ_W)); tr_in.push_back(lp(k, L_BK_W));
        }
        const size_t tr_pcat0 = tr_in.size();
        for (int64_t k = 0; k < nl; ++k) for (auto& p : st.layer[k].Pcat) tr_in.push_back(p);
        const size_t tr_tail = tr_in.size();
        tr_in.push_back(st.Wch_all);
        tr_in.push_back(st.lstm[0].Wih); tr_in.push_back(st.lstm[1].Wih);
        if (want_dx) tr_in.push_back(all[P_VE_W]);
        HStream early = (side != curs && (flags & F_OVERLAP_PREP)) ? side : curs;
        auto mark0 = [](HStream on) { hipEvent_t e = next_event(); TORCH_CHECK(hipEventRecord(e, on.stream()) == hipSuccess, "hipEventRecord failed"); return e; };
        wait_stream(early, curs);
        std::vector<Tensor> tr;
        {
            StreamScope sc(early);
            tr = transpose_all(tr_in);
        }
        auto trk = [&](int64_t k, int which) -> const Tensor& { return tr[k * TR_PER_LAYER + which]; };
        std::vector<std::vector<Tensor>> PcatT(nl);
        { size_t i = tr_pcat0; for (int64_t k = 0; k < nl; ++k) for (size_t p = 0; p < st.layer[k].Pcat.size(); ++p) PcatT[k].push_back(tr[i++]); }
        const Tensor &Wch_allT = tr[tr_tail], *WihT = &tr[tr_tail + 1];

        const Tensor& bu_last = st.layer[nl - 1].bu;
        Tensor dpm = g[0].defined() ? cont(g[0]) : at::zeros_like(st.pm), dpsea;
        {
// ... 1 lines not shown
            bool rows = g[1].defined() && g[2].defined() && g[3].defined();
            for (int h = 1; rows && h <= 3; ++h) rows = g[h].scalar_type() == at::kFloat && g[h].is_contiguous() && g[h].numel() == BL;
            if (rows && fp(g[2]) == fp(g[1]) + BL && fp(g[3]) == fp(g[1]) + 2 * BL) dpsea = g[1];
            else {
                std::vector<Tensor> parts;
                for (int h = 1; h <= 3; ++h) parts.push_back(g[h].defined() ? fl(g[h]).reshape({B, L}) : at::zeros({B, L}, opt));
                dpsea = at::stack(parts);
            }
        }
        Tensor dfm = at::empty({N, D}, opt), dfb_next = at::empty({B, L, D}, opt);
        std::vector<Tensor> loc_bufs;
        {
            Tensor dwm = at::empty({D}, opt), dbm = at::empty({1}, opt), dwb = at::empty({3, D}, opt), dbb = at::empty({3}, opt);
            if (early != curs) {
                wait_stream(early, curs);
                {
                    StreamScope sc(early);
                    auto ws = scratch(smin_workspace_bytes(n, B, 4, D, 4, 1), dev);
                    SMIN_CK(smin_score_map_bwd(cur(), nullptr, fp(dpsea), fp(st.pm), fp(st.psea), fp(st.fm_out), fp(bu_last), ip(cells), n, B, Li, D, fp(loc[0]), fp(st.wb),
                                               fp(lmf), nullptr, fpm(dfb_next), nullptr, nullptr, fpm(dwb), fpm(dbb), ws.p, ws.n));
                }
                hipEvent_t early_done = mark0(early);
                auto ws = scratch(smin_workspace_bytes(n, B, 4, D, 4, 1), dev);
                SMIN_CK(smin_score_map_bwd(cur(), fp(dpm), nullptr, fp(st.pm), fp(st.psea), fp(st.fm_out), fp(bu_last), ip(cells), n, B, Li, D, fp(loc[0]), fp(st.wb), fp(lmf),
                                           fpm(dfm), nullptr, fpm(dwm), fpm(dbm), nullptr, nullptr, ws.p, ws.n));
                TORCH_CHECK(hipStreamWaitEvent(curs.stream(), early_done, 0) == hipSuccess, "hipStreamWaitEvent failed");
            } else {
                auto ws = scratch(smin_workspace_bytes(n, B, 4, D, 4, 1), dev);
                SMIN_CK(smin_score_map_bwd(cur(), fp(dpm), fp(dpsea), fp(st.pm), fp(st.psea), fp(st.fm_out), fp(bu_last), ip(cells), n, B, Li, D, fp(loc[0]), fp(st.wb), fp(lmf),
                                           fpm(dfm), fpm(dfb_next), fpm(dwm), fpm(dbm), fpm(dwb), fpm(dbb), ws.p, ws.n));
            }
            Tensor* dloc = &dprm[nl * L_COUNT];
            loc_bufs = {dwm, dbm, dwb, dbb};
            dloc[0] = dwm.view_as(loc[0]); dloc[1] = dbm.view_as(loc[1]);
            for (int h = 0; h < 3; ++h) { dloc[2 + 2 * h] = dwb[h].view_as(loc[2 + 2 * h]); dloc[3 + 2 * h] = dbb.slice(0, h, h + 1).view_as(loc[3 + 2 * h]); }
        }

        std::vector<Tensor> dcc(nl), dHs(nl), dchat(nl), dconsts(nl), dfs_parts, dfw_parts;
        Tensor dconsts_all, dWcat_all, dbcat_all, dWch_all;
        std::vector<Tensor> base_ch(nl), base_c(nl), base_bc(nl);
        if (prep_kernel) {
            dconsts_all = at::empty({nl, dl}, opt); dWcat_all = at::empty({nl, D, 2 * D}, opt); dbcat_all = at::empty({nl, D}, opt);
            for (int64_t k = 0; k < nl; ++k) dconsts[k] = dconsts_all[k];
        }
        std::vector<std::vector<Tensor>> dPcat(nl);
        Tensor dwhat = at::empty_like(st.what), dshat = at::empty_like(st.shat), dMq = at::empty_like(st.Mq), duq = at::empty_like(st.uq);
        if (N == 0) { dwhat.zero_(); dshat.zero_(); dMq.zero_(); duq.zero_(); }
        Tensor dcum_next;
        auto mark_on = [](HStream on) { hipEvent_t e = next_event(); TORCH_CHECK(hipEventRecord(e, on.stream()) == hipSuccess, "hipEventRecord failed"); return e; };
        hipEvent_t attn0_done = nullptr;
        hipEvent_t boundary_done = nullptr;
        for (int64_t k = nl - 1; k >= 0; --k) {
            LayerState& ls = st.layer[k];
            Tensor dcum = at::empty({N, D}, opt), dfb_mu = at::empty({B, L, D}, opt);
            keep.push_back(dfm); keep.push_back(dcum);
            {
                wait_stream(wstr, curs);
                StreamScope sc(wstr);
                Tensor dWcat = prep_kernel ? dWcat_all[k] : at::empty_like(ls.Wcat), dbcat = prep_kernel ? dbcat_all[k] : at::empty({D}, opt);
                auto ws = scratch(smin_workspace_bytes(n, B, 4, D, 4, 1), dev);
                if (ls.x1.scalar_type() == at::kBFloat16)
                    SMIN_CK(smin_moment_unit_bwd_x1h(cur(), fp(dfm), fp(ls.cum), fp(ls.bu), ip(cells), ip(row_ptr), ip(cellmap), n, B, Li, D, fp(trk(k, TR_CAT)), nullptr, nullptr,
                                                     fpm(dWcat), fpm(dbcat), ws.p, ws.n, 1, nullptr, reinterpret_cast<const uint16_t*>(ls.x1.const_data_ptr()), nullptr));
                else
                    SMIN_CK(smin_moment_unit_bwd(cur(), fp(dfm), fp(ls.cum), fp(ls.bu), ip(cells), ip(row_ptr), ip(cellmap), n, B, Li, D, fp(trk(k, TR_CAT)), nullptr, nullptr,
                                                 fpm(dWcat), fpm(dbcat), ws.p, ws.n, 1, nullptr, fp(ls.x1), nullptr));
                if (!prep_kernel) {
                    dlp(k, L_FB_W) = dWcat.slice(1, 0, D).contiguous().view_as(lp(k, L_FB_W)); dlp(k, L_FC_W) = dWcat.slice(1, D).contiguous().view_as(lp(k, L_FC_W));
                    dlp(k, L_FB_B) = dbcat; dlp(k, L_FC_B) = dbcat;
                }
                sync.reduce({dWcat, dbcat}, wstr);
            }
            if (boundary_done) { TORCH_CHECK(hipStreamWaitEvent(curs.stream(), boundary_done, 0) == hipSuccess, "hipStreamWaitEvent failed"); boundary_done = nullptr; }
            {
                auto ws = scratch(smin_workspace_bytes(n, B, 4, D, 4, 1), dev);
                SMIN_CK(smin_moment_unit_bwd(cur(), fp(dfm), fp(ls.cum), fp(ls.bu), ip(cells), ip(row_ptr), ip(cellmap), n, B, Li, D, fp(trk(k, TR_CAT)), fpm(dcum), fpm(dfb_mu),
                                             nullptr, nullptr, ws.p, ws.n, 1, fp(dcum_next), nullptr, fp(dfb_next)));
            }
            Tensor dfb_k, dbu;
            wait_stream(side, curs);
            {
                StreamScope sc(side);
                dbu = dfb_mu;
                dfb_k = at::empty({B, L, D}, opt);
                Tensor dfw = at::empty_like(fw), dfs = at::empty_like(fs);
                Tensor dWq = at::empty({D, D}, opt), dbq = at::empty({D}, opt), dWk = at::empty({D, D}, opt), dbk = at::empty({D}, opt);
                auto ws = scratch(smin_boundary_unit_bwd_ws_bytes(B, Li, Nq, D), dev);
                SMIN_CK(smin_boundary_unit_bwd(cur(), fp(dbu), fp(ls.fb), fp(fw), fp(fs), fp(ls.hbar), ip(cells), ip(row_ptr), n, B, Li, Nq, D, fp(trk(k, TR_BQ)), fp(trk(k, TR_BK)),
                                               fp(qmf), fp(lmf), fp(ls.Qb), fp(ls.Kb), fp(ls.P), fp(ls.baq), fp(ls.bqv), fp(ls.A), fpm(dfb_k), fpm(dfw), fpm(dfs), nullptr,
                                               fpm(dWq), fpm(dbq), fpm(dWk), fpm(dbk), ws.p, ws.n));
                dlp(k, L_BQ_W) = dWq; dlp(k, L_BQ_B) = dbq; dlp(k, L_BK_W) = dWk; dlp(k, L_BK_B) = dbk;
                sync.reduce({dWq, dbq, dWk, dbk}, side);
                dfs_parts.push_back(dfs); dfw_parts.push_back(dfw);
                keep.push_back(dfb_next); keep.push_back(dfb_mu); keep.push_back(dbu);
            }
            if (side != curs) boundary_done = mark_on(side);
            Tensor dccmean = at::empty({N, dl}, opt);
            {
                const float* xs[1] = {fp(ls.ccmean)}; float* dxs[1] = {fpm(dccmean)};
                auto ws = scratch(smin_linear_rows_bwd_workspace_bytes(n, D, dl), dev);
                SMIN_CK(smin_linear_rows_bwd(cur(), fp(dcum), xs, 1, fp(trk(k, TR_C)), n, D, dl, dxs, nullptr, nullptr, ws.p, ws.n));
            }
            dchat[k] = at::empty({N * C, dl}, opt);
            if (N > 0) {
                auto ws = scratch(smin_content_attn_bwd_workspace_bytes(n, B, Ci, dl), dev);
                SMIN_CK(smin_content_attn_bwd(cur(), fp(dcc[k]), fp(dccmean), fp(ls.chat), ip(cells), ip(row_ptr), n, B, Li, Ci, dl, Nq, fp(st.Mq[k]), fp(st.uq[k]), fp(st.what[k]),
                                              fp(st.shat[k]), fp(qmf), fpm(dchat[k]), fpm(dMq[k]), fpm(duq[k]), fpm(dwhat[k]), fpm(dshat[k]), ws.p, ws.n));
            }
            if (k == 0) attn0_done = mark_on(curs);
            Tensor dhp;
            for (int64_t part = 0, lo = 0; lo < k; ++part, lo += 4) {
                const int nseg = i32(std::min<int64_t>(4, k - lo));
                const float* xs[4]; float* dxs[4];
                const bool have = dcc[lo].defined();
                for (int sgm = 0; sgm < nseg; ++sgm) {
                    TORCH_CHECK(dcc[lo + sgm].defined() == have, "content stream: inconsistent gradient state of the attention outputs");
                    xs[sgm] = nullptr;
                    if (!have) dcc[lo + sgm] = at::empty({N * C, dl}, opt);
                    dxs[sgm] = fpm(dcc[lo + sgm]);
                }
                if (have) {
                    SMIN_CK(smin_linear_rows_dx_acc(cur(), fp(dchat[k]), nseg, fp(PcatT[k][part]), i32(N * C), dl, dl, dxs));
                } else {
                    auto ws = scratch(smin_linear_rows_bwd_workspace_bytes(i32(N * C), dl, nseg * dl), dev);
                    SMIN_CK(smin_linear_rows_bwd(cur(), fp(dchat[k]), xs, nseg, fp(PcatT[k][part]), i32(N * C), dl, dl, dxs, nullptr, nullptr, ws.p, ws.n));
                }
            }
            if (k > 0) {
                dhp = at::empty({N, dl}, opt);
                keep.push_back(dhp);
                SMIN_CK(smin_group_sum(cur(), fp(dchat[k]), n, Ci, dl, fpm(dhp)));
                dHs[k] = at::empty({N, D}, opt);
                const float* xs[1] = {fp(ls.Hs)}; float* dxs[1] = {fpm(dHs[k])};
                auto ws = scratch(smin_linear_rows_bwd_workspace_bytes(n, dl, D), dev);
                SMIN_CK(smin_linear_rows_bwd(cur(), fp(dhp), xs, 1, fp(trk(k, TR_CH)), n, dl, D, dxs, nullptr, nullptr, ws.p, ws.n));
            }
            wait_stream(wstr, curs);
            {
                StreamScope sc(wstr);
                {
                    Tensor dWc = at::empty_like(lp(k, L_C_W)), dbc = at::empty({D}, opt);
                    const float* xs[1] = {fp(ls.ccmean)};
                    auto ws = scratch(smin_linear_rows_bwd_workspace_bytes(n, D, dl), dev);
                    SMIN_CK(smin_linear_rows_bwd(cur(), fp(dcum), xs, 1, nullptr, n, D, dl, nullptr, fpm(dWc), fpm(dbc), ws.p, ws.n));
                    if (prep_kernel) { base_c[k] = dWc; base_bc[k] = dbc; }
                    else { acc(dlp(k, L_C_W), dWc); acc(dlp(k, L_C_B), dbc); }
                }
                for (int64_t part = 0, lo = 0; lo < k; ++part, lo += 4) {
                    const int nseg = i32(std::min<int64_t>(4, k - lo));
                    Tensor dP = at::empty_like(ls.Pcat[part]);
                    if (lo == 0 && !prep_kernel) dconsts[k] = at::empty({dl}, opt);
                    auto ws = scratch(smin_linear_rows_bwd_workspace_bytes(i32(N * C), dl, nseg * dl), dev);
                    if (st.layer[lo].cc.scalar_type() == at::kBFloat16) {
                        const uint16_t* xh[4];
                        for (int sgm = 0; sgm < nseg; ++sgm) xh[sgm] = hp16(st.layer[lo + sgm].cc);
                        SMIN_CK(smin_linear_rows_bwd_xh(cur(), fp(dchat[k]), xh, nseg, i32(N * C), dl, dl, fpm(dP), lo == 0 ? fpm(dconsts[k]) : nullptr, ws.p, ws.n));
                    } else {
                        const float* xs[4];
                        for (int sgm = 0; sgm < nseg; ++sgm) xs[sgm] = fp(st.layer[lo + sgm].cc);
                        SMIN_CK(smin_linear_rows_bwd(cur(), fp(dchat[k]), xs, nseg, nullptr, i32(N * C), dl, dl, nullptr, fpm(dP), lo == 0 ? fpm(dconsts[k]) : nullptr, ws.p, ws.n));
                    }
                    dPcat[k].push_back(dP);
                }
                if (k > 0) {
                    Tensor dWch = at::empty_like(lp(k, L_CH_W));
                    const float* xs[1] = {fp(ls.Hs)};
                    auto ws = scratch(smin_linear_rows_bwd_workspace_bytes(n, dl, D), dev);
                    SMIN_CK(smin_linear_rows_bwd(cur(), fp(dhp), xs, 1, nullptr, n, dl, D, nullptr, fpm(dWch), nullptr, ws.p, ws.n));
                    if (prep_kernel) base_ch[k] = dWch; else acc(dlp(k, L_CH_W), dWch);
                }
            }
            {
                std::vector<Tensor> later;
                for (int64_t kk = k + 1; kk < nl; ++kk) later.push_back(dHs[kk]);
                std::vector<const float*> dh{fp(dcum)}, dr{fp(dfm)};
                Tensor later_sum;
                if (later.size() <= 3) for (auto& t : later) dh.push_back(fp(t));
                else { later_sum = sum_list(later); dh.push_back(fp(later_sum)); }
                if (k == 0) dr.push_back(fp(dcum));
                Tensor dfm_k = at::empty({N, D}, opt), dfs = at::empty_like(fs);
                auto ws = scratch((size_t)4 * B * 512 * D + 4096, dev);
                SMIN_CK(smin_gate_bwd(cur(), dh.data(), i32(dh.size()), dr.data(), i32(dr.size()), fp(ls.fm), fp(fs), ip(row_ptr), n, B, Li, D, fpm(dfm_k), fpm(dfs), ws.p, ws.n,
                                      ip(cells), fp(ls.A), fp(dbu)));
                dfs_parts.push_back(dfs);
                dfm = dfm_k;
            }
            dcum_next = dcum; dfb_next = dfb_k;
        }

        hipStreamCaptureStatus capture = hipStreamCaptureStatusNone;
        TORCH_CHECK(hipStreamIsCapturing(curs.stream(), &capture) == hipSuccess, "hipStreamIsCapturing failed");
        const bool tail_split = (flags & F_TAIL_SPLIT) && capture == hipStreamCaptureStatusNone;
        HStream tail = (flags & F_OVERLAP_PREP) ? side_stream(dev.index()) : curs;
        HStream wordst = !(flags & F_OVERLAP_PREP) ? curs : tail_split ? side_stream(dev.index(), 1) : tail;
        HStream cw = tail_split ? tail : curs;
        auto mark = mark_on;
        auto await = [](HStream waiter, hipEvent_t e) { TORCH_CHECK(hipStreamWaitEvent(waiter.stream(), e, 0) == hipSuccess, "hipStreamWaitEvent failed"); };
        if (!attn0_done) attn0_done = mark(curs);
        hipEvent_t words_done;
        if (!tail_split) wait_stream(wordst, curs);
        else if (wordst != curs) await(wordst, attn0_done);
        {
            StreamScope sc(wordst);
            std::vector<const float*> gp[4], pp;
            std::vector<float*> dp;
            for (int64_t k = 0; k < nl; ++k) {
                gp[0].push_back(fp(dwhat[k])); gp[1].push_back(fp(dshat[k])); gp[2].push_back(fp(dMq[k])); gp[3].push_back(fp(duq[k]));
                for (int which : {L_WH_W, L_WH_B, L_SH_W, L_SH_B, L_AK_W, L_AK_B, L_AQ_W, L_AQ_B}) {
                    pp.push_back(fp(lp(k, which)));
                    dlp(k, which) = at::empty_like(lp(k, which));
                    dp.push_back(fpm(dlp(k, which)));
                }
            }
            Tensor dfw = at::empty_like(fw), dfs = at::empty_like(fs);
            auto ws = scratch(smin_word_prep_bwd_workspace_bytes(i32(nl), B, Nq, D, dl), dev);
            SMIN_CK(smin_word_prep_bwd(cur(), gp[0].data(), gp[1].data(), gp[2].data(), gp[3].data(), fp(fw), fp(fs), fp(qmf), fp(st.what), fp(st.kb), pp.data(), i32(nl), B, Nq, D,
                                       dl, fpm(dfw), fpm(dfs), dp.data(), ws.p, ws.n));
            dfw_parts.push_back(dfw); dfs_parts.push_back(dfs);
            words_done = mark(wordst);
            if (sync.on) {
                std::vector<Tensor> ws_grads = loc_bufs;
// ... 139 lines not shown
                for (int pc = 0; pc < 3; ++pc) {
                    int which = 1 << pc;
                    while (pc + 1 < 3 && piece[pc + 1] == piece[pc]) which |= 1 << ++pc;
                    wait_stream(piece[pc], curs);
                    StreamScope sc(piece[pc]);
                    SMIN_CK(smin_bilstm_layer_bwd_weights(cur(), which, fp(ls.x), fp(ls.Hout), B, i32(Nq_in), In, Hh, fpm(dWih), fpm(dbias), fpm(dbias2), fpm(dWhh),
                                                          wsl.data_ptr(), (size_t)wsl.numel()));
                }
                if (dX.defined()) keep.push_back(dX);
                const int64_t H4 = 4 * H;
                Tensor* o = &dbb[P_LSTM + 8 * layer];
                o[0] = dWih.slice(0, 0, H4); o[1] = dWhh[0]; o[2] = dbias.slice(0, 0, H4); o[3] = dbias2.slice(0, 0, H4);
                o[4] = dWih.slice(0, H4); o[5] = dWhh[1]; o[6] = dbias.slice(0, H4); o[7] = dbias2.slice(0, H4);
                dH = dX;
            }
            dquery = dH;
            if (want_dx) {
                dvideo = at::empty_like(st.vx);
                SMIN_CK(smin_video_encoder_bwd_input(cur(), fp(tr[tr_tail + 3]), fp(st.vmaskf), B, Ti, Din, D, fpm(dvideo), wsv.data_ptr(), (size_t)wsv.numel()));
            }
        }
        wait_stream(curs, tail);
        wait_stream(curs, wstr);
        wait_stream(curs, wordst);
        if (sync.on) {
            std::vector<Tensor> late{dbb[P_VE_W], dbb[P_VE_B], dbb[P_PE]};
            for (auto& t : lstm_bufs) late.push_back(t);
            sync.reduce(late, curs);
            sync.join(curs);
        }

        variable_list out(N_FIXED + all.size());
        if (want_dx) out[0] = dvideo;
        if (want_dX) out[2] = dquery;
        for (size_t i = 0; i < all.size(); ++i) out[N_FIXED + i] = i < (size_t)P_LAYER0 ? dbb[i] : dprm[i - P_LAYER0];
        return out;
    }
};


Tensor padded_query_mask(const char* op, const Tensor& query_features, const Tensor& query_mask_in, int64_t maxq)
{
    TORCH_CHECK(query_features.dim() == 3, op, ": query_features (B, words, dim)");
    Tensor query_mask = query_mask_in.reshape({query_features.size(0), -1});
    TORCH_CHECK((query_mask.size(1) == query_features.size(1) || query_mask.size(1) == maxq) && query_features.size(1) <= maxq, op, ": query_mask has ",
                query_mask.size(1), " columns for ", query_features.size(1), " words (max_query_length ", maxq, ")");
    if (query_mask.size(1) < maxq) query_mask = at::constant_pad_nd(query_mask, {0, maxq - query_mask.size(1)}, 0);
    return query_mask;
}

std::tuple<Tensor, Tensor, Tensor, Tensor, std::vector<Tensor>, std::vector<Tensor>> smin_forward(
    const Tensor& video_features, const Tensor& video_mask, const Tensor& query_features, const Tensor& query_mask_in, const Tensor& length_mask,
    const Tensor& moment_mask, at::TensorList prm, int64_t T, int64_t L, int64_t C, int64_t num_smi_layers, int64_t max_query_length, int64_t lstm_hidden_size,
    bool overlap_boundary, bool overlap_prep, bool param_prep_kernel, bool async_weights, bool bf16_operand_storage, bool grad_sync,
    std::optional<int64_t> known_cell_count, bool tail_split, bool input_grads, std::optional<c10::string_view> attention)
{
    TORCH_CHECK(video_features.is_cuda(), "smin_forward runs on a HIP device only (there is no CPU fallback)");
    TORCH_CHECK(input_grads || (!video_features.requires_grad() && !query_features.requires_grad()), "smin_forward forms no gradients of video_features / "
                "query_features unless input_grads = True (SMIN.input_grads); otherwise inputs that require grad go through the Python host "
                "(SMIN.fused_core = False)");
    const bool packed = attention && *attention == "packed";
    TORCH_CHECK(!attention || packed || *attention == "dense", "smin_forward: attention is None, \"dense\" or \"packed\" (got \"", *attention, "\")");
    const int64_t nl = num_smi_layers, maxq = max_query_length;
    Tensor query_mask = padded_query_mask("smin_forward", query_features, query_mask_in, maxq);
    TORCH_CHECK((int64_t)prm.size() == P_LAYER0 + nl * L_COUNT + 8, "smin_forward: expected ", P_LAYER0 + nl * L_COUNT + 8, " parameters, got ", prm.size());
    c10::hip::HIPGuard device_guard(video_features.device().index());
    const int64_t flags = (overlap_boundary ? SminCore::F_OVERLAP_BOUNDARY : 0) | (overlap_prep ? SminCore::F_OVERLAP_PREP : 0) |
                          (param_prep_kernel ? SminCore::F_PARAM_PREP_KERNEL : 0) | (async_weights ? SminCore::F_ASYNC_WEIGHTS : 0) |
                          (bf16_operand_storage ? SminCore::F_BF16_OPERANDS : 0) | (grad_sync ? SminCore::F_GRAD_SYNC : 0) |
                          (tail_split ? SminCore::F_TAIL_SPLIT : 0) | (input_grads ? SminCore::F_INPUT_GRADS : 0) |
                          (attention ? SminCore::F_KEEP_ATTENTION : 0) | (packed ? SminCore::F_ATTN_PACKED : 0);
    auto out = SminCore::apply(video_features, video_mask, query_features, query_mask, length_mask, moment_mask, T, L, C, nl, maxq, lstm_hidden_size, flags,
                               known_cell_count.value_or(-1), prm);
    const int64_t nc = attention ? nl + (packed ? 1 : 0) : 0, nb = attention ? nl : 0;
    TORCH_CHECK((int64_t)out.size() == 4 + nc + nb, "smin_forward: ", out.size(), " outputs");
    std::vector<Tensor> content(out.begin() + 4, out.begin() + 4 + nc), boundary(out.begin() + 4 + nc, out.end());
    return std::make_tuple(out[0], out[1], out[2], out[3], content, boundary);
}

std::tuple<Tensor, Tensor, Tensor, Tensor> smin_score(
    const Tensor& video_features, const Tensor& video_mask, const Tensor& query_features, const Tensor& query_mask_in, const Tensor& length_mask,
    const Tensor& moment_mask, at::TensorList prm, int64_t T, int64_t L, int64_t C, int64_t num_smi_layers, int64_t max_query_length, int64_t lstm_hidden_size,
    bool overlap_boundary, bool overlap_prep, bool param_prep_kernel, bool bf16_operand_storage, std::optional<int64_t> known_cell_count)
{
    TORCH_CHECK(video_features.is_cuda(), "smin_score runs on a HIP device only (there is no CPU fallback)");
    at::NoGradGuard no_grad;
    const int64_t nl = num_smi_layers;
    Tensor query_mask = padded_query_mask("smin_score", query_features, query_mask_in, max_query_length);
    TORCH_CHECK((int64_t)prm.size() == P_LAYER0 + nl * L_COUNT + 8, "smin_score: expected ", P_LAYER0 + nl * L_COUNT + 8, " parameters, got ", prm.size());
    c10::hip::HIPGuard device_guard(video_features.device().index());
    const int64_t flags = (overlap_boundary ? SminCore::F_OVERLAP_BOUNDARY : 0) | (overlap_prep ? SminCore::F_OVERLAP_PREP : 0) |
                          (param_prep_kernel ? SminCore::F_PARAM_PREP_KERNEL : 0) | (bf16_operand_storage ? SminCore::F_BF16_OPERANDS : 0);
    CoreState st;
    std::vector<Tensor> all, cmaps, bmaps;
    SminCore::run(st, all, cmaps, bmaps, true, video_features.detach(), video_mask, query_features.detach(), query_mask, length_mask, moment_mask, T, L, C, nl,
                  max_query_length, lstm_hidden_size, flags, known_cell_count.value_or(-1), prm);
    return std::make_tuple(st.pm, st.psea[0], st.psea[1], st.psea[2]);
}


Tensor smin_encode_videos(const Tensor& video_features, const Tensor& video_mask, at::TensorList prm)
{
    TORCH_CHECK(video_features.is_cuda() && video_mask.is_cuda(), "smin_encode_videos runs on a HIP device only (there is no CPU fallback)");
    at::NoGradGuard no_grad;
    TORCH_CHECK(video_features.dim() == 3 && video_features.scalar_type() == at::kFloat, "smin_encode_videos: video_features float32 (V, T, Din)");
    TORCH_CHECK((int64_t)prm.size() >= P_LSTM, "smin_encode_videos: the parameter list starts with the video encoder's three");
    const int64_t V = video_features.size(0), T = video_features.size(1), Din = video_features.size(2);
    Tensor W = cont(prm[P_VE_W].detach()), bias = cont(prm[P_VE_B].detach()), pe = cont(prm[P_PE].detach());
    const int64_t D = W.size(0);
    TORCH_CHECK(W.dim() == 2 && W.size(1) == Din && bias.numel() == D && pe.dim() == 2 && pe.size(1) == D && pe.size(0) >= T && video_mask.numel() == V * T,
                "smin_encode_videos: shapes of the video encoder's parameters or of video_mask do not fit video_features");
    c10::hip::HIPGuard device_guard(video_features.device().index());
    Tensor vx = cont(video_features.detach());
    Tensor vm = video_mask.reshape({V * T});
    Tensor vmaskf = cont(vm.is_floating_point() ? fl(vm) : vm.ne(0).to(at::kFloat));
    Tensor fv = at::empty({V, T, D}, vx.options());
    SMIN_CK(smin_video_encoder_fwd(cur(), fp(vx), fp(W), fp(bias), fp(pe), fp(vmaskf), nullptr, i32(V), i32(T), i32(Din), i32(D), fpm(fv), nullptr));
    return fv;
}

std::tuple<Tensor, Tensor> smin_encode_queries(const Tensor& query_features, const Tensor& query_mask_in, at::TensorList prm, int64_t max_query_length,
                                               int64_t lstm_hidden_size)
{
    TORCH_CHECK(query_features.is_cuda() && query_mask_in.is_cuda(), "smin_encode_queries runs on a HIP device only (there is no CPU fallback)");
    at::NoGradGuard no_grad;
    TORCH_CHECK(query_features.scalar_type() == at::kFloat, "smin_encode_queries: query_features float32 (Q, words, dim)");
    TORCH_CHECK((int64_t)prm.size() >= P_LAYER0, "smin_encode_queries: the parameter list starts with the video encoder's three and the LSTM's sixteen");
    Tensor query_mask = padded_query_mask("smin_encode_queries", query_features, query_mask_in, max_query_length);
    c10::hip::HIPGuard device_guard(query_features.device().index());
    std::vector<Tensor> all;
    for (int64_t i = 0; i < P_LAYER0; ++i) all.push_back(cont(prm[i].detach()));
    Tensor len32 = query_mask.ne(0).sum(1).to(at::kInt).contiguous();
    LstmState lstm[2];
    auto out = query_encoder(lstm, all, query_features.detach(), len32, max_query_length, lstm_hidden_size, true);
    return std::make_tuple(out.first, out.second);
}

std::tuple<Tensor, Tensor, Tensor, Tensor> smin_score_pairs(
    const Tensor& fv, const Tensor& fw, const Tensor& fs, const Tensor& video_mask, const Tensor& query_mask_in, const Tensor& length_mask, const Tensor& moment_mask,
    const Tensor& video_index, const Tensor& query_index, at::TensorList prm, int64_t T, int64_t L, int64_t C, int64_t num_smi_layers, int64_t max_query_length,
    int64_t lstm_hidden_size, bool overlap_boundary, bool overlap_prep, bool param_prep_kernel, bool bf16_operand_storage, std::optional<int64_t> known_cell_count)
{
    for (const Tensor* t : {&fv, &fw, &fs, &video_mask, &query_mask_in, &length_mask, &moment_mask, &video_index, &query_index})
        TORCH_CHECK(t->is_cuda(), "smin_score_pairs runs on a HIP device only (there is no CPU fallback)");
    at::NoGradGuard no_grad;
// ... 33 lines not shown

void adam_step(at::TensorList params, at::TensorList grads, const Tensor& exp_avg_flat, const Tensor& exp_avg_sq_flat, at::IntArrayRef offsets,
               const Tensor& state, const std::optional<Tensor>& ws, double beta1, double beta2, double eps, double weight_decay, bool decoupled,
               double max_norm, bool skip_nonfinite)
{
    const size_t n = params.size();
    TORCH_CHECK(grads.size() == n && offsets.size() == n, "adam_step: ", n, " parameters, ", grads.size(), " gradients, ", offsets.size(), " offsets");
    TORCH_CHECK(exp_avg_flat.is_cuda(), "adam_step runs on a HIP device only (there is no CPU fallback)");
    const auto dev = exp_avg_flat.device();
    auto flat_ok = [&](const Tensor& t, at::ScalarType ty) { return t.device() == dev && t.scalar_type() == ty && t.is_contiguous(); };
    TORCH_CHECK(flat_ok(exp_avg_flat, at::kFloat) && flat_ok(exp_avg_sq_flat, at::kFloat) && exp_avg_flat.numel() == exp_avg_sq_flat.numel(),
                "adam_step: the moment buffers must be contiguous fp32 tensors of one size on one HIP device");
    TORCH_CHECK(flat_ok(state, at::kDouble) && state.numel() == 8, "adam_step: state must be 8 contiguous doubles on the parameters' device");
    std::vector<float*> pp(n);
    std::vector<const float*> gp(n);
    std::vector<int64_t> ne(n), mo(n);
    int64_t total = 0;
    for (size_t i = 0; i < n; ++i) {
        const Tensor &p = params[i], &g = grads[i];
        TORCH_CHECK(p.is_cuda() && g.is_cuda(), "adam_step runs on a HIP device only (there is no CPU fallback): parameter ", i);
        TORCH_CHECK(p.device() == dev && g.device() == dev, "adam_step: parameter ", i, " or its gradient is on another device");
        TORCH_CHECK(p.scalar_type() == at::kFloat && g.scalar_type() == at::kFloat, "adam_step: parameter ", i, " or its gradient is not fp32");
        TORCH_CHECK(p.is_contiguous() && g.is_contiguous(), "adam_step: parameter ", i, " or its gradient is not contiguous");
        TORCH_CHECK(p.sizes() == g.sizes(), "adam_step: gradient ", i, " has not its parameter's shape");
        ne[i] = p.numel();
        mo[i] = offsets[i];
        TORCH_CHECK(mo[i] >= 0 && mo[i] + ne[i] <= exp_avg_flat.numel(), "adam_step: moment segment ", i, " lies outside the flat buffers");
        pp[i] = p.numel() ? p.data_ptr<float>() : nullptr;
        gp[i] = g.numel() ? g.const_data_ptr<float>() : nullptr;
        total += ne[i];
        torch::autograd::impl::bump_version(p);
    }
    const bool norm = max_norm >= 0.0 || skip_nonfinite;
    c10::hip::HIPGuard device_guard(dev.index());
    void* wsp = nullptr;
    if (norm) {
        const size_t need = smin_adam_ws_bytes(total, i32((int64_t)n));
        TORCH_CHECK(ws && ws->defined() && ws->device() == dev && ws->scalar_type() == at::kByte && ws->is_contiguous() && (size_t)ws->numel() >= need,
                    "adam_step: the norm needs a uint8 workspace of ", need, " bytes on the parameters' device");
        wsp = ws->data_ptr();
        SMIN_CK(smin_grad_norm(cur(), gp.data(), ne.data(), i32((int64_t)n), max_norm >= 0.0 ? max_norm : -1.0, state.data_ptr<double>(), wsp,
                               (size_t)ws->numel()));
    }
    SMIN_CK(smin_adam_step(cur(), pp.data(), gp.data(), ne.data(), mo.data(), i32((int64_t)n), exp_avg_flat.data_ptr<float>(),
                           exp_avg_sq_flat.data_ptr<float>(), state.data_ptr<double>(), beta1, beta2, eps, weight_decay, decoupled ? 1 : 0,
                           skip_nonfinite ? 1 : 0, wsp));
}

}

TORCH_LIBRARY(smin_hip, m)
{
    m.def("smin_forward(Tensor video_features, Tensor video_mask, Tensor query_features, Tensor query_mask, Tensor length_mask, Tensor moment_mask, "
          "Tensor[] params, int T, int L, int C, int num_smi_layers, int max_query_length, int lstm_hidden_size, *, bool overlap_boundary, "
          "bool overlap_prep, bool param_prep_kernel, bool async_weights, bool bf16_operand_storage, bool grad_sync, int? known_cell_count, "
          "bool tail_split, bool input_grads, str? attention) -> (Tensor, Tensor, Tensor, Tensor, Tensor[], Tensor[])", &smin_forward);
    m.def("smin_score(Tensor video_features, Tensor video_mask, Tensor query_features, Tensor query_mask, Tensor length_mask, Tensor moment_mask, "
          "Tensor[] params, int T, int L, int C, int num_smi_layers, int max_query_length, int lstm_hidden_size, *, bool overlap_boundary, "
          "bool overlap_prep, bool param_prep_kernel, bool bf16_operand_storage, int? known_cell_count) -> (Tensor, Tensor, Tensor, Tensor)", &smin_score);
    m.def("smin_encode_videos(Tensor video_features, Tensor video_mask, Tensor[] params) -> Tensor", &smin_encode_videos);
    m.def("smin_encode_queries(Tensor query_features, Tensor query_mask, Tensor[] params, int max_query_length, int lstm_hidden_size) -> (Tensor, Tensor)",
          &smin_encode_queries);
    m.def("smin_score_pairs(Tensor fv, Tensor fw, Tensor fs, Tensor video_mask, Tensor query_mask, Tensor length_mask, Tensor moment_mask, Tensor video_index, "
          "Tensor query_index, Tensor[] params, int T, int L, int C, int num_smi_layers, int max_query_length, int lstm_hidden_size, *, bool overlap_boundary, "
          "bool overlap_prep, bool param_prep_kernel, bool bf16_operand_storage, int? known_cell_count) -> (Tensor, Tensor, Tensor, Tensor)", &smin_score_pairs);
    m.def("smin_loss(Tensor pm, Tensor ym, Tensor sm, Tensor moment_mask, Tensor ps, Tensor ys, Tensor ss, Tensor pe, Tensor ye, Tensor se, Tensor pa, Tensor ya, "
          "Tensor length_mask) -> Tensor", &smin_loss);
    m.def("adam_step(Tensor[] params, Tensor[] grads, Tensor exp_avg_flat, Tensor exp_avg_sq_flat, int[] offsets, Tensor state, Tensor? ws, float beta1, "
          "float beta2, float eps, float weight_decay, bool decoupled, float max_norm, bool skip_nonfinite) -> ()", &adam_step);
    m.def("abi_version() -> int", []() -> int64_t { return smin_abi_version(); });
    m.def("layout_status(Device device) -> Tensor", [](c10::Device dev) { return layout_status(dev); });
    m.def("set_grad_sync(str group_name, int world, bool coalesced_avg) -> ()", [](std::string group, int64_t world, bool coalesced_avg) {
        GradSyncConfig& c = grad_sync_config();
        c.group = std::move(group); c.world = (int)world; c.coalesced_avg = coalesced_avg;
    });
}
```

### video-moment-localization_amd/modules.py

```python
import functools
import math

import os

import torch
import torch.nn as nn

from . import _lib
from ._host import _AttnMaps, query_mask_rows
from ._lib import SminHipError

from .cells import CellLayout
from .functional import (VideoFuseFn, WordPrepFn, BiLstmLayerFn, BoundaryUnitFn, ClipWindowMeansFn, ContentAttnFn, ContentUnitFn, GateFn, LinearRowsFn, MomentUnitFn,
                         ProposalMapFn, ProposalMeansFn, ScoreMapFn, content_attn_maps_dense)
from .retrieval import QueryBank, VideoBank, _Retrieval


def _hip_forward(fn):
    @functools.wraps(fn)
    def wrapper(self, x, *args, **kwargs):
        if not (isinstance(x, torch.Tensor) and x.is_cuda):
            raise SminHipError(f"{type(self).__name__}.forward runs on a HIP device only (got a CPU tensor); there is no CPU fallback")
        if x.device.index != torch.cuda.current_device():
            with torch.cuda.device(x.device):
# ... 313 lines not shown

    def __init__(self, D):
        super().__init__()
        self.conv_layer_pm = nn.Conv2d(D, 1, 1)
        self.conv_layer_ps = nn.Conv1d(D, 1, 1)
        self.conv_layer_pe = nn.Conv1d(D, 1, 1)
        self.conv_layer_pa = nn.Conv1d(D, 1, 1)
        self.sigmoid = nn.Sigmoid()

    def forward_packed(self, fm, f_b, length_mask, layout):
        D = f_b.shape[-1]
        heads = (self.conv_layer_ps, self.conv_layer_pe, self.conv_layer_pa)
        wb = torch.stack([h.weight.view(D) for h in heads])
        bb = torch.cat([h.bias for h in heads])
        pm, psea = ScoreMapFn.apply(fm, f_b, self.conv_layer_pm.weight.view(D), self.conv_layer_pm.bias, wb, bb,
                                    length_mask.float(), layout)
        return pm, psea[0], psea[1], psea[2]

    @_hip_forward
    def forward(self, f_m, f_b, length_mask, moment_mask):
        layout = CellLayout.all_cells(moment_mask)
        return self.forward_packed(layout.pack(f_m), f_b, length_mask, layout)


class SMIN(nn.Module, _Retrieval):

    def __init__(self, T, L, C, D, dl, num_smi_layers, input_video_dim, max_query_length, lstm_hidden_size, device='cpu'):
        super().__init__()
        self.T, self.L, self.C, self.D, self.dl = T, L, C, D, dl
        self.num_smi_layers, self.input_video_dim = num_smi_layers, input_video_dim
        self.max_query_length, self.lstm_hidden_size, self.device = max_query_length, lstm_hidden_size, device
        if D != 2 * lstm_hidden_size:
            raise ValueError("SMIN needs D == 2 * lstm_hidden_size (reference models.py:62,81)")
        limits = [(T % L == 0, f"L | T (T={T}, L={L}): the reference's AvgPool1d gives {T // max(T // L, 1)} != L boundary rows otherwise (SURVEY 8a-2)"),
                  (2 <= C <= 4, f"2 <= C <= 4 clips per moment (C={C}): csrc/content_attn.hip keeps the clips of a cell in one lane quad"),
                  (D % 4 == 0, f"D % 4 == 0 (D={D}): 16-byte row segments everywhere"),
                  (dl % 16 == 0 and 16 <= dl <= 128, f"dl a multiple of 16 in [16, 128] (dl={dl}): csrc/content_attn.hip tiles the attention rows in 16-feature blocks, csrc/word_prep.hip holds dl <= 128"),
                  (1 <= max_query_length <= 32, f"max_query_length <= 32 (got {max_query_length}): the word-side kernels keep a query in 32 LDS slots"),
                  (num_smi_layers >= 1, f"num_smi_layers >= 1 (got {num_smi_layers})")]
        bad = [msg for ok, msg in limits if not ok]
        if bad:
            raise ValueError("SMIN: outside the limits of the HIP kernels -- needs " + "; ".join(bad))
        self.backbone = Backbone(T, D, input_video_dim, max_query_length, lstm_hidden_size, device)
        self.pgm = ProposalGeneration(T, L, C, device)
        self.smis = nn.ModuleList([SMI(D, dl) for _ in range(num_smi_layers)])
        self.localization = Localization(D)

    fused_core = True
    async_weights = True
    known_cell_count = None
    tail_split = True
    grad_sync = False
    bf16_operand_storage = True
    content_stream = True
    overlap_boundary = True
    overlap_prep = True
    keep_attention = False
    forward_only_scoring = False
    input_grads = False

    def _forward_stream(self, f, fs, fw, query_mask, length_mask, layout, maps=None):
        T, L, C, dl = self.T, self.L, self.C, self.dl
        N = layout.N
        nl = len(self.smis)
        cus = [smi.content_unit for smi in self.smis]
        cur = torch.cuda.current_stream(f.device)
        side = _side_stream(f.device) if self.overlap_boundary else cur
        prep = side if (self.overlap_prep and self._torch_beside_contractions()) else cur
        prep.wait_stream(cur)
        with torch.cuda.stream(prep):
            consts, bsum = [], None
            for cu in cus:
                consts.append(cu.linear_c_hat.bias if bsum is None else cu.linear_c_hat.bias + torch.mv(cu.linear_c_hat.weight, bsum))
                bsum = cu.linear_c.bias if bsum is None else bsum + cu.linear_c.bias
            Wch_all = torch.cat([cu.linear_c_hat.weight for cu in cus])
            const_all = consts[0]
            qmr = _rows(query_mask)
            wo = WordPrepFn.apply(fw, fs, qmr, *[p for cu in cus for p in cu.word_params()])
            words = [(wo[4 * k + 2], wo[4 * k + 3], wo[4 * k], wo[4 * k + 1], qmr) for k in range(nl)]
            Pcats = [[torch.cat([torch.matmul(cus[k].linear_c_hat.weight, cus[l].linear_c.weight) for l in range(lo, min(lo + 4, k))], dim=1)
                      for lo in range(0, k, 4)] for k in range(nl)]
            mu_w = [smi.moment_unit.cat_weights() for smi in self.smis]
        cur.wait_stream(prep)
        if prep is not cur:
            for t in [Wch_all] + consts + [x for w in words for x in w] + [x for ps in Pcats for x in ps] + [x for w in mu_w for x in w]:
                t.record_stream(cur)
        if side is not cur:
            for t in (fw, fs, query_mask, length_mask, layout.cells, layout.row_ptr, layout.cellmap):
                t.record_stream(side)
        fm, fb = ProposalMeansFn.apply(f, layout, T, L, C)
        g_all = LinearRowsFn.apply(Wch_all, None, None, None, 1, f.reshape(-1, self.D))
        pgs = ClipWindowMeansFn.apply(g_all.view(f.shape[0], T, -1), const_all, layout, T, L, C, nl)
        cumean, H, hist = None, None, []
        for k, smi in enumerate(self.smis):
            last = k == nl - 1
            cu = smi.content_unit
            n_hbar = 2 if last else (3 if k > 0 or nl < 3 else 4)
            views = GateFn.apply(fm, fs, layout, n_hbar, 2 if k == 0 else 1)
            hbar_c, hbar_b, fm_res = views[0], views[1], views[n_hbar]
            if k == 0:
                cumean = views[n_hbar + 1]
            side.wait_stream(cur)
            with torch.cuda.stream(side):
                bu = smi.boundary_unit.forward_packed(fb, fw, fs, hbar_b, query_mask, length_mask, layout, maps is not None)
                if maps is not None:
                    bu, bmap = bu
# ... 34 lines not shown

    def _native_params(self):
        ve, lstm = self.backbone.videoencoder, self.backbone.queryencoder.lstm
        ps = [ve.ve.weight, ve.ve.bias, ve.pe.weight]
        for layer in range(2):
            for sfx in ("", "_reverse"):
                ps += [getattr(lstm, f"{n}_l{layer}{sfx}") for n in ("weight_ih", "weight_hh", "bias_ih", "bias_hh")]
        for smi in self.smis:
            cu, bu, mu = smi.content_unit, smi.boundary_unit.attn_layer, smi.moment_unit
            for m in (cu.linear_c_hat, cu.linear_w_hat, cu.linear_s_hat, cu.linear_c, cu.attn_layer.W_q, cu.attn_layer.W_k, bu.W_q, bu.W_k,
                      mu.conv_layer_fb, mu.conv_layer_fc):
                ps += [m.weight, m.bias]
        lo = self.localization
        for m in (lo.conv_layer_pm, lo.conv_layer_ps, lo.conv_layer_pe, lo.conv_layer_pa):
            ps += [m.weight, m.bias]
        return ps

    @staticmethod
    def _torch_beside_contractions():
        return _lib.get_gemm_mode() == "f32" or bool(os.environ.get("SMIN_STREAMS_IN_ALL_MODES"))

    def _param_prep_kernel(self):
        return self.D % 32 == 0 and self.D <= 1056 and self.dl % 32 == 0 and len(self.smis) <= 8

    def _plan(self, video_features, query_features):
        nl = len(self.smis)
        if not (self.content_stream and self.dl < self.D and nl <= 8 and nl * self.dl <= 2048):
            return "units"
        node = (self.fused_core and (self.input_grads or not (video_features.requires_grad or query_features.requires_grad))
                and self.backbone.queryencoder.fused() and query_features.dtype == torch.float32
                and self.backbone.videoencoder.fused(video_features) and video_features.shape[1] == self.T)
        return "node" if node else "stream"

    def _node_options(self, attention=None):
        o = self._score_options()
        bf16, known = o.pop("bf16_operand_storage"), o.pop("known_cell_count")
        return dict(**o, async_weights=self.async_weights, bf16_operand_storage=bf16, grad_sync=self.grad_sync and torch.is_grad_enabled(),
                    known_cell_count=known, tail_split=self.tail_split, input_grads=self.input_grads, attention=attention)

    def _score_options(self):
        prep_kernel = self._param_prep_kernel()
        return dict(overlap_boundary=self.overlap_boundary, overlap_prep=self.overlap_prep and (prep_kernel or self._torch_beside_contractions()),
                    param_prep_kernel=prep_kernel, bf16_operand_storage=self.bf16_operand_storage,
                    known_cell_count=None if self.known_cell_count is None else int(self.known_cell_count))

    @_hip_forward
    def score(self, video_features, video_mask, query_features, query_mask, length_mask, moment_mask):
        with torch.no_grad():
            if self.keep_attention or self._plan(video_features, query_features) != "node":
                return self(video_features, video_mask, query_features, query_mask, length_mask, moment_mask)
            query_mask = query_mask_rows(query_features, query_mask, self.max_query_length)
            return _lib.load_torch().smin_score(
                video_features, video_mask, query_features, query_mask, length_mask, moment_mask, self._native_params(), self.T, self.L, self.C,
                len(self.smis), self.max_query_length, self.lstm_hidden_size, **self._score_options())

    def _record_attention(self, maps):
        for smi, (cmap, bmap) in zip(self.smis, maps):
            smi.content_unit.attn_layer.attn_weights = cmap
            smi.boundary_unit.attn_layer.attn_weights = bmap

    @_hip_forward
    def forward(self, video_features, video_mask, query_features, query_mask, length_mask, moment_mask):
        maps = None
        if self.keep_attention:
            for smi in self.smis:
                smi.content_unit.attn_layer.keep_weights = smi.boundary_unit.attn_layer.keep_weights = True
            maps = _AttnMaps("dense")
        out = self._forward(video_features, video_mask, query_features, query_mask, length_mask, moment_mask, maps)
        if maps is not None:
            self._record_attention(maps)
        return out

    @_hip_forward
    def _forward(self, video_features, video_mask, query_features, query_mask, length_mask, moment_mask, maps):
        query_mask = query_mask_rows(query_features, query_mask, self.max_query_length)
        if query_mask.shape[1] < self.max_query_length:
            query_mask = torch.nn.functional.pad(query_mask, (0, self.max_query_length - query_mask.shape[1]))
        plan = self._plan(video_features, query_features)
        if self.grad_sync and not self._torch_beside_contractions():
            raise RuntimeError("SMIN.grad_sync: the in-node gradient exchange runs RCCL beside the contraction kernels and is limited to the exact "
                               "fp32 mode; call distributed.wrap after set_gemm_mode (it then uses torch DDP)")
        if self.grad_sync and plan != "node":
            raise RuntimeError("SMIN.grad_sync (distributed.wrap's in-node gradient exchange) needs the one-node extension path; this "
                               "call does not qualify (see SMIN._plan) -- wrap the model with SMIN_TORCH_DDP=1 instead")
        if plan == "node":
            pm, ps, pe, pa, content, boundary = _lib.load_torch().smin_forward(
                video_features, video_mask, query_features, query_mask, length_mask, moment_mask, self._native_params(), self.T, self.L, self.C,
                len(self.smis), self.max_query_length, self.lstm_hidden_size, **self._node_options(None if maps is None else maps.mode))
            if maps is not None:
                if maps.mode == "packed":
                    maps.cellmap, content = content[-1], content[:-1]
                maps.extend(zip(content, boundary))
            return pm, ps, pe, pa
        if maps is not None and plan == "units":
            raise RuntimeError("SMIN.keep_attention / localize(attention=True): the word-attention maps come out of the content stream's attention "
                               "core; this configuration runs the content units as written (ContentUnitFn, see SMIN._plan), which cannot "
                               "deliver them")
        pending = CellLayout.begin(moment_mask)
        f, fs, fw = self.backbone(video_features, video_mask, query_features, query_mask, input_grads=self.input_grads)
        layout = pending.finish()
        if plan == "stream":
            if maps is not None:
                maps.cellmap = layout.cellmap
            return self._forward_stream(f, fs, fw, query_mask, length_mask, layout, maps)
        fc, fm, fb = self.pgm.forward_packed(f, layout)
        fcmean = fm
        for k, smi in enumerate(self.smis):
            last = k == len(self.smis) - 1
            fc, fm, fb, fcmean = smi.forward_packed(fc, fm, fb, fw, fs, query_mask, length_mask, layout, fcmean if last else None)
        return self.localization.forward_packed(fm, fb, length_mask, layout)
```

Before: 15.17 million proposals/s.

## Recompute the sigmoid gate inside consumers instead of storing hbar

Adds gated variants of the boundary reduce kernels, a gated row-linear forward, and gate-sum row kernels. They recompute hbar = fm*sigmoid(fm*fs) on the fly from fm and fs instead of reading a stored hbar or running hidden-state sums. The old materialising path is kept behind a new store_gate flag, which defaults to False, so the recompute path is the default. This cuts memory traffic and the separate gate kernel launch, at the cost of repeated expf work in each consumer and in backward.

Result: slower. 15.01 million proposals/s (-1.0%).

```diff
diff --git a/include/smin_hip.h b/include/smin_hip.h
--- a/include/smin_hip.h
+++ b/include/smin_hip.h
@@ -71,6 +71,17 @@
                            const float* Qb, const float* Kb, const float* P, const float* baq, const float* bqv, const float* A,
                            float* dfb, float* dfw, float* dfs, float* dhbar, float* dWq, float* dbq, float* dWk, float* dbk,
                            void* ws, size_t ws_bytes);
+int smin_boundary_unit_fwd_fm(void* stream, const float* fb, const float* fw, const float* fs, const float* fm,
+                              const int32_t* cells, const int32_t* row_ptr, int N, int B, int L, int Nq, int D,
+                              const float* Wq, const float* bq, const float* Wk, const float* bk,
+                              const float* qmask, const float* lmask,
+                              float* out, float* Qb, float* Kb, float* P, float* baq, float* bqv, float* A);
+int smin_boundary_unit_bwd_fm(void* stream, const float* dout, const float* fb, const float* fw, const float* fs, const float* fm,
+                              const int32_t* cells, const int32_t* row_ptr, int N, int B, int L, int Nq, int D,
+                              const float* WqT, const float* WkT, const float* qmask, const float* lmask,
+                              const float* Qb, const float* Kb, const float* P, const float* baq, const float* bqv, const float* A,
+                              float* dfb, float* dfw, float* dfs, float* dhbar, float* dWq, float* dbq, float* dWk, float* dbk,
+                              void* ws, size_t ws_bytes);
 
 int smin_moment_unit_fwd(void* stream, const float* fcmean, const float* fm, const float* fb, const int32_t* cells,
                          int N, int B, int L, int D, const float* Wcat, const float* bcat, float* mu,
@@ -205,6 +216,12 @@
                             const float* add_cells, int C, int R, int O, int K, float* y);
 int smin_linear_rows_bwd_xh(void* stream, const float* dy, const uint16_t* const* xs, int nseg, int R, int O, int K,
                             float* dW, float* dbias, void* ws, size_t ws_bytes);
+int smin_linear_rows_gate_fwd(void* stream, const float* x, const float* W, const float* bias, const float* add_rows, const float* fm,
+                              const float* fs, const int32_t* cells, int R, int O, int K, float* y);
+int smin_gate_sum_rows_fwd(void* stream, const float* const* fms, int nfm, const float* fs, const int32_t* cells, const float* W,
+                           int R, int O, int K, float* y);
+int smin_gate_sum_rows_bwd_w(void* stream, const float* dy, const float* const* fms, int nfm, const float* fs, const int32_t* cells,
+                             int R, int O, int K, float* dW, void* ws, size_t ws_bytes);
 int smin_linear_rows_dx_acc(void* stream, const float* dy, int nseg, const float* WT, int R, int O, int K, float* const* dxs);
 int smin_group_sum(void* stream, const float* x, int groups, int C, int W, float* out);
 
diff --git a/video-moment-localization_amd/_lib.py b/video-moment-localization_amd/_lib.py
--- a/video-moment-localization_amd/_lib.py
+++ b/video-moment-localization_amd/_lib.py
@@ -40,6 +40,8 @@
     "smin_boundary_unit_fwd": [_vp] * 7 + [_i] * 5 + [_vp] * 6 + [_vp] * 7,
     "smin_boundary_unit_bwd_ws_bytes": [_i] * 4,
     "smin_boundary_unit_bwd": [_vp] * 8 + [_i] * 5 + [_vp] * 4 + [_vp] * 6 + [_vp] * 8 + [_vp, _sz],
+    "smin_boundary_unit_fwd_fm": [_vp] * 7 + [_i] * 5 + [_vp] * 6 + [_vp] * 7,
+    "smin_boundary_unit_bwd_fm": [_vp] * 8 + [_i] * 5 + [_vp] * 4 + [_vp] * 6 + [_vp] * 8 + [_vp, _sz],
     "smin_moment_unit_fwd": [_vp] * 5 + [_i] * 4 + [_vp] * 3 + [_vp],
     "smin_pair_product": [_vp] * 3 + [_i] * 3 + [_vp],
     "smin_moment_unit_bwd": [_vp] * 7 + [_i] * 4 + [_vp] * 5 + [_vp, _sz, _i, _vp, _vp, _vp],
@@ -95,6 +97,9 @@
     "smin_linear_rows_bwd_xh": [_vp, _vp, _vp, _i, _i, _i, _i, _vp, _vp, _vp, _sz],
     "smin_linear_rows_bwd_workspace_bytes": [_i] * 3,
     "smin_linear_rows_bwd": [_vp, _vp, _vp, _i, _vp] + [_i] * 3 + [_vp] * 3 + [_vp, _sz],
+    "smin_linear_rows_gate_fwd": [_vp] * 8 + [_i] * 3 + [_vp],
+    "smin_gate_sum_rows_fwd": [_vp, _vp, _i] + [_vp] * 3 + [_i] * 3 + [_vp],
+    "smin_gate_sum_rows_bwd_w": [_vp, _vp, _vp, _i, _vp, _vp] + [_i] * 3 + [_vp, _vp, _sz],
     "smin_linear_rows_dx_acc": [_vp, _vp, _i, _vp] + [_i] * 3 + [_vp],
     "smin_group_sum": [_vp, _vp, _i, _i, _i, _vp],
     "smin_video_encoder_fwd": [_vp] * 7 + [_i] * 4 + [_vp] * 2,
diff --git a/video-moment-localization_amd/csrc/boundary_unit.hip b/video-moment-localization_amd/csrc/boundary_unit.hip
--- a/video-moment-localization_amd/csrc/boundary_unit.hip
+++ b/video-moment-localization_amd/csrc/boundary_unit.hip
@@ -3,8 +3,9 @@
 
 namespace smin {
 
+template <bool GATED>
 __global__ __launch_bounds__(128)
-void boundary_reduce_fwd_kernel(const float* __restrict__ Ab, const float* __restrict__ hbar, const float* base,
+void boundary_reduce_fwd_kernel(const float* __restrict__ Ab, const float* __restrict__ hbar, const float* __restrict__ fs, const float* base,
                                 const int* __restrict__ cells, const int* __restrict__ row_ptr, int L, int D, float* fbm)
 {
     const int i = blockIdx.x, b = blockIdx.y;
@@ -12,15 +13,19 @@
     const float* arow = Ab + ((size_t)b * L + i) * L;
     for (int d = threadIdx.x * 4; d < D; d += 512) {
         float4 acc = base ? ldg4(base + ((size_t)b * L + i) * D + d) : f4zero();
-        for (int n = r0; n < r1; ++n)
-            acc = f4fma(ldg4(hbar + (size_t)n * D + d), arow[cells[4 * (size_t)n + 2]], acc);
+        const float4 s4 = GATED ? ldg4(fs + (size_t)b * D + d) : f4zero();
+        for (int n = r0; n < r1; ++n) {
+            const float4 x = ldg4(hbar + (size_t)n * D + d);
+            acc = f4fma(GATED ? gate4(x, s4) : x, arow[cells[4 * (size_t)n + 2]], acc);
+        }
         stg4(fbm + ((size_t)b * L + i) * D + d, acc);
     }
 }
 
+template <bool GATED>
 __global__ __launch_bounds__(256)
 void boundary_reduce_bwd_kernel(const float* __restrict__ dfbm, const float* __restrict__ Ab, const float* __restrict__ hbar,
-                                const int* __restrict__ cells, const int* __restrict__ row_ptr,
+                                const float* __restrict__ fs, const int* __restrict__ cells, const int* __restrict__ row_ptr,
                                 int L, int D, float* __restrict__ dAb, float* __restrict__ dhbar)
 {
     const int i = blockIdx.x, b = blockIdx.y;
@@ -36,7 +41,8 @@
         float dot = 0.f;
         for (int d = lane * 4; d < D; d += 256) {
             const float4 dy = ldg4(dfbm + ((size_t)b * L + i) * D + d);
-            const float4 x = ldg4(hbar + (size_t)n * D + d);
+            const float4 h = ldg4(hbar + (size_t)n * D + d);
+            const float4 x = GATED ? gate4(h, ldg4(fs + (size_t)b * D + d)) : h;
             dot = fmaf(dy.x, x.x, dot); dot = fmaf(dy.y, x.y, dot); dot = fmaf(dy.z, x.z, dot); dot = fmaf(dy.w, x.w, dot);
             if (dhbar) stg4(dhbar + (size_t)n * D + d, f4scale(dy, a));
         }
@@ -304,7 +310,8 @@
 {
     (void)N;
     SMIN_REQUIRE(D % 4 == 0);
-    hipLaunchKernelGGL(boundary_reduce_fwd_kernel, dim3(L, B), dim3(128), 0, (hipStream_t)stream, Ab, hbar, nullptr, cells, row_ptr, L, D, fbm);
+    hipLaunchKernelGGL(boundary_reduce_fwd_kernel<false>, dim3(L, B), dim3(128), 0, (hipStream_t)stream, Ab, hbar, (const float*)nullptr, (const float*)nullptr, cells,
+                       row_ptr, L, D, fbm);
     SMIN_LAUNCH_CHECK();
     return 0;
 }
@@ -316,7 +323,7 @@
     (void)N;
     hipStream_t st = (hipStream_t)stream;
     SMIN_REQUIRE(D % 4 == 0);
-    hipLaunchKernelGGL(boundary_reduce_bwd_kernel, dim3(L, B), dim3(256), 0, st, dfbm, Ab, hbar, cells, row_ptr, L, D, dAb, dhbar);
+    hipLaunchKernelGGL(boundary_reduce_bwd_kernel<false>, dim3(L, B), dim3(256), 0, st, dfbm, Ab, hbar, (const float*)nullptr, cells, row_ptr, L, D, dAb, dhbar);
     SMIN_LAUNCH_CHECK();
     return 0;
 }
@@ -351,11 +358,11 @@
     }
 };
 
-extern "C" int smin_boundary_unit_fwd(void* stream, const float* fb, const float* fw, const float* fs, const float* hbar,
-                                      const int32_t* cells, const int32_t* row_ptr, int N, int B, int L, int Nq, int D,
-                                      const float* Wq, const float* bq, const float* Wk, const float* bk,
-                                      const float* qmask, const float* lmask,
-                                      float* out, float* Qb, float* Kb, float* P, float* baq, float* bqv, float* A)
+static int boundary_unit_fwd(bool gated, void* stream, const float* fb, const float* fw, const float* fs, const float* hbar,
+                             const int32_t* cells, const int32_t* row_ptr, int N, int B, int L, int Nq, int D,
+                             const float* Wq, const float* bq, const float* Wk, const float* bk,
+                             const float* qmask, const float* lmask,
+                             float* out, float* Qb, float* Kb, float* P, float* baq, float* bqv, float* A)
 {
     (void)N;
     hipStream_t st = (hipStream_t)stream;
@@ -369,9 +376,28 @@
     SMIN_LAUNCH_CHECK();
     hipLaunchKernelGGL(boundary_self_fwd_kernel, dim3(L, B), dim3(256), sizeof(float) * L, st, bqv, fb, lmask, L, D, scale, A, out);
     SMIN_LAUNCH_CHECK();
-    hipLaunchKernelGGL(boundary_reduce_fwd_kernel, dim3(L, B), dim3(128), 0, st, A, hbar, out, cells, row_ptr, L, D, out);
+    if (gated) hipLaunchKernelGGL(boundary_reduce_fwd_kernel<true>, dim3(L, B), dim3(128), 0, st, A, hbar, fs, out, cells, row_ptr, L, D, out);
+    else hipLaunchKernelGGL(boundary_reduce_fwd_kernel<false>, dim3(L, B), dim3(128), 0, st, A, hbar, fs, out, cells, row_ptr, L, D, out);
     SMIN_LAUNCH_CHECK();
     return 0;
+}
+
+extern "C" int smin_boundary_unit_fwd(void* stream, const float* fb, const float* fw, const float* fs, const float* hbar,
+                                      const int32_t* cells, const int32_t* row_ptr, int N, int B, int L, int Nq, int D,
+                                      const float* Wq, const float* bq, const float* Wk, const float* bk,
+                                      const float* qmask, const float* lmask,
+                                      float* out, float* Qb, float* Kb, float* P, float* baq, float* bqv, float* A)
+{
+    return boundary_unit_fwd(false, stream, fb, fw, fs, hbar, cells, row_ptr, N, B, L, Nq, D, Wq, bq, Wk, bk, qmask, lmask, out, Qb, Kb, P, baq, bqv, A);
+}
+
+extern "C" int smin_boundary_unit_fwd_fm(void* stream, const float* fb, const float* fw, const float* fs, const float* fm,
+                                         const int32_t* cells, const int32_t* row_ptr, int N, int B, int L, int Nq, int D,
+                                         const float* Wq, const float* bq, const float* Wk, const float* bk,
+                                         const float* qmask, const float* lmask,
+                                         float* out, float* Qb, float* Kb, float* P, float* baq, float* bqv, float* A)
+{
+    return boundary_unit_fwd(true, stream, fb, fw, fs, fm, cells, row_ptr, N, B, L, Nq, D, Wq, bq, Wk, bk, qmask, lmask, out, Qb, Kb, P, baq, bqv, A);
 }
 
 extern "C" size_t smin_boundary_unit_bwd_ws_bytes(int B, int L, int Nq, int D)
@@ -380,12 +406,12 @@
     return BuBwdWs(B, L, Nq, D).end * sizeof(float);
 }
 
-extern "C" int smin_boundary_unit_bwd(void* stream, const float* dout, const float* fb, const float* fw, const float* fs, const float* hbar,
-                                      const int32_t* cells, const int32_t* row_ptr, int N, int B, int L, int Nq, int D,
-                                      const float* WqT, const float* WkT, const float* qmask, const float* lmask,
-                                      const float* Qb, const float* Kb, const float* P, const float* baq, const float* bqv, const float* A,
-                                      float* dfb, float* dfw, float* dfs, float* dhbar, float* dWq, float* dbq, float* dWk, float* dbk,
-                                      void* ws, size_t ws_bytes)
+static int boundary_unit_bwd(bool gated, void* stream, const float* dout, const float* fb, const float* fw, const float* fs, const float* hbar,
+                             const int32_t* cells, const int32_t* row_ptr, int N, int B, int L, int Nq, int D,
+                             const float* WqT, const float* WkT, const float* qmask, const float* lmask,
+                             const float* Qb, const float* Kb, const float* P, const float* baq, const float* bqv, const float* A,
+                             float* dfb, float* dfw, float* dfs, float* dhbar, float* dWq, float* dbq, float* dWk, float* dbk,
+                             void* ws, size_t ws_bytes)
 {
     (void)N;
     hipStream_t st = (hipStream_t)stream;
@@ -408,7 +434,8 @@
     if (cols_lds > 48 * 1024)
         if (int e = lds_optin(reinterpret_cast<const void*>(boundary_self_bwd_cols_kernel), cols_lds)) return e;
 
-    hipLaunchKernelGGL(boundary_reduce_bwd_kernel, dim3(L, B), dim3(256), 0, st, dout, A, hbar, cells, row_ptr, L, D, dAbm, dhbar);
+    if (gated) hipLaunchKernelGGL(boundary_reduce_bwd_kernel<true>, dim3(L, B), dim3(256), 0, st, dout, A, hbar, fs, cells, row_ptr, L, D, dAbm, dhbar);
+    else hipLaunchKernelGGL(boundary_reduce_bwd_kernel<false>, dim3(L, B), dim3(256), 0, st, dout, A, hbar, fs, cells, row_ptr, L, D, dAbm, dhbar);
     SMIN_LAUNCH_CHECK();
     hipLaunchKernelGGL(boundary_self_bwd_rows_kernel, dim3(L, B), dim3(256), sizeof(float) * L, st, dout, dAbm, A, fb, lmask, L, D, scale, draw);
     SMIN_LAUNCH_CHECK();
@@ -437,3 +464,25 @@
     rc = launch_reduce_slabs2(st, slab2, dWk, D * D, bslab2, dbk, D, sp2); if (rc) return rc;
     return 0;
 }
+
+extern "C" int smin_boundary_unit_bwd(void* stream, const float* dout, const float* fb, const float* fw, const float* fs, const float* hbar,
+                                      const int32_t* cells, const int32_t* row_ptr, int N, int B, int L, int Nq, int D,
+                                      const float* WqT, const float* WkT, const float* qmask, const float* lmask,
+                                      const float* Qb, const float* Kb, const float* P, const float* baq, const float* bqv, const float* A,
+                                      float* dfb, float* dfw, float* dfs, float* dhbar, float* dWq, float* dbq, float* dWk, float* dbk,
+                                      void* ws, size_t ws_bytes)
+{
+    return boundary_unit_bwd(false, stream, dout, fb, fw, fs, hbar, cells, row_ptr, N, B, L, Nq, D, WqT, WkT, qmask, lmask, Qb, Kb, P, baq, bqv, A, dfb, dfw, dfs,
+                             dhbar, dWq, dbq, dWk, dbk, ws, ws_bytes);
+}
+
+extern "C" int smin_boundary_unit_bwd_fm(void* stream, const float* dout, const float* fb, const float* fw, const float* fs, const float* fm,
+                                         const int32_t* cells, const int32_t* row_ptr, int N, int B, int L, int Nq, int D,
+                                         const float* WqT, const float* WkT, const float* qmask, const float* lmask,
+                                         const float* Qb, const float* Kb, const float* P, const float* baq, const float* bqv, const float* A,
+                                         float* dfb, float* dfw, float* dfs, float* dhbar, float* dWq, float* dbq, float* dWk, float* dbk,
+                                         void* ws, size_t ws_bytes)
+{
+    return boundary_unit_bwd(true, stream, dout, fb, fw, fs, fm, cells, row_ptr, N, B, L, Nq, D, WqT, WkT, qmask, lmask, Qb, Kb, P, baq, bqv, A, dfb, dfw, dfs,
+                             dhbar, dWq, dbq, dWk, dbk, ws, ws_bytes);
+}
diff --git a/video-moment-localization_amd/csrc/common.h b/video-moment-localization_amd/csrc/common.h
--- a/video-moment-localization_amd/csrc/common.h
+++ b/video-moment-localization_amd/csrc/common.h
@@ -99,3 +99,6 @@
 __device__ __forceinline__ float4 f4fma(float4 a, float s, float4 c) { return make_float4(fmaf(a.x, s, c.x), fmaf(a.y, s, c.y), fmaf(a.z, s, c.z), fmaf(a.w, s, c.w)); }
 __device__ __forceinline__ float4 ldg4(const float* p) { return *reinterpret_cast<const float4*>(p); }
 __device__ __forceinline__ void stg4(float* p, float4 v) { *reinterpret_cast<float4*>(p) = v; }
+
+__device__ __forceinline__ float gate1(float x, float s) { return x / (1.0f + expf(-x * s)); }
+__device__ __forceinline__ float4 gate4(float4 x, float4 s) { return make_float4(gate1(x.x, s.x), gate1(x.y, s.y), gate1(x.z, s.z), gate1(x.w, s.w)); }
diff --git a/video-moment-localization_amd/csrc/gate.hip b/video-moment-localization_amd/csrc/gate.hip
--- a/video-moment-localization_amd/csrc/gate.hip
+++ b/video-moment-localization_amd/csrc/gate.hip
@@ -12,8 +12,7 @@
     const size_t n = idx / D4; const int d4 = (int)(idx % D4);
     const int b = cells[4 * n];
     const float4 x = ldg4(fm + idx * 4), s = ldg4(fs + ((size_t)b * D4 + d4) * 4);
-    const float4 h = make_float4(x.x / (1.0f + expf(-x.x * s.x)), x.y / (1.0f + expf(-x.y * s.y)),
-                                 x.z / (1.0f + expf(-x.z * s.z)), x.w / (1.0f + expf(-x.w * s.w)));
+    const float4 h = gate4(x, s);
     stg4(hbar + idx * 4, h);
     if (SUM) stg4(hsum_out + idx * 4, f4add(ldg4(hsum_in + idx * 4), h));
 }
diff --git a/video-moment-localization_amd/csrc/gate_ops.h b/video-moment-localization_amd/csrc/gate_ops.h
--- /dev/null
+++ b/video-moment-localization_amd/csrc/gate_ops.h
@@ -0,0 +1,69 @@
+#pragma once
+#include "gemm.h"
+
+namespace smin {
+
+template <int NT>
+struct GateSumMat {
+    const float* fm[4]; const float* fs; const int* cells; int D;
+    struct Row { size_t off; const float* s; };
+    struct Key { int b; };
+    __device__ __forceinline__ Row row(int r) const { return resolve(key(r), r); }
+    __device__ __forceinline__ Key key(int r) const { return Key{cells[4 * (size_t)r]}; }
+    __device__ __forceinline__ Row resolve(const Key& k, int r) const { return Row{(size_t)r * D, fs + (size_t)k.b * D}; }
+    __device__ __forceinline__ float4 at(const Row& r, int c) const {
+        const float4 s = ldg4(r.s + c);
+        float4 x[NT];
+#pragma unroll
+        for (int l = 0; l < NT; ++l) x[l] = ldg4(fm[l] + r.off + c);
+        float4 v = gate4(x[0], s);
+#pragma unroll
+        for (int l = 1; l < NT; ++l) v = f4add(v, gate4(x[l], s));
+        return v;
+    }
+};
+
+template <class K, class A, class KEY, class PRE, class POST>
+__device__ __forceinline__ void chunk_rows_f4_keyed(const float* Ws, int row0, int col0, int ncols, int M, int N, int lane, KEY key, PRE pre, POST post)
+{
+    K k[8];
+#pragma unroll
+    for (int it = 0; it < 8; ++it) k[it] = key(min(row0 + ((lane + 64 * it) >> 4), M - 1));
+    A add[8];
+#pragma unroll
+    for (int it = 0; it < 8; ++it) {
+        const int idx = lane + 64 * it, r = idx >> 4, c4 = (idx & 15) * 4;
+        add[it] = pre(min(row0 + r, M - 1), min(col0 + c4, N - 4), k[it]);
+    }
+#pragma unroll
+    for (int it = 0; it < 8; ++it) {
+        const int idx = lane + 64 * it, r = idx >> 4, c4 = (idx & 15) * 4;
+        const int row = row0 + r, col = col0 + c4;
+        if (c4 < ncols && row < M && col < N) post(row, col, ldg4(Ws + r * GEMM_LDW + c4), add[it]);
+    }
+}
+
+template <bool HAS_BIAS, bool SHARED>
+struct EpLinearRowsGate {
+    const float* bias; const float* add_rows; const float* fm; const float* fs; const int* cells; float* out;
+    struct Add { float4 r, x, s; };
+    __device__ __forceinline__ void chunk(const float* Ws, int row0, int col0, int ncols, int M, int N, int lane) const {
+        chunk_rows_f4_keyed<int, Add>(Ws, row0, col0, ncols, M, N, lane,
+            [&](int row) { return cells[4 * (size_t)row]; },
+            [&](int row, int col, int b) {
+                Add a;
+                a.r = ldg4(add_rows + (size_t)row * N + col);
+                a.x = SHARED ? a.r : ldg4(fm + (size_t)row * N + col);
+                a.s = ldg4(fs + (size_t)b * N + col);
+                return a;
+            },
+            [&](int row, int col, float4 v, const Add& a) {
+                if (HAS_BIAS) v = f4add(v, ldg4(bias + col));
+                v = f4add(v, a.r);
+                v = f4add(v, gate4(a.x, a.s));
+                stg4(out + (size_t)row * N + col, v);
+            });
+    }
+};
+
+}
diff --git a/video-moment-localization_amd/csrc/linear_rows.hip b/video-moment-localization_amd/csrc/linear_rows.hip
--- a/video-moment-localization_amd/csrc/linear_rows.hip
+++ b/video-moment-localization_amd/csrc/linear_rows.hip
@@ -1,4 +1,5 @@
 #include "gemm.h"
+#include "gate_ops.h"
 #include "smin_hip.h"
 
 namespace smin {
@@ -89,6 +90,64 @@
                 : run(EpLinearRows<false, false, true>{bias, add_rows, add_cells, C, y});
 }
 
+extern "C" int smin_linear_rows_gate_fwd(void* stream, const float* x, const float* W, const float* bias, const float* add_rows, const float* fm,
+                                         const float* fs, const int32_t* cells, int R, int O, int K, float* y)
+{
+    SMIN_REQUIRE(O % 4 == 0 && K % 4 == 0 && add_rows != nullptr && fm != nullptr && fs != nullptr && cells != nullptr);
+    if (R == 0) return 0;
+    hipStream_t st = (hipStream_t)stream;
+    auto run = [&](auto ep) { return launch_gemm_nt(st, PlainMat{x, K}, PlainMat{W, K}, ep, R, O, K); };
+    if (add_rows == fm) return bias ? run(EpLinearRowsGate<true, true>{bias, add_rows, fm, fs, cells, y})
+                                    : run(EpLinearRowsGate<false, true>{bias, add_rows, fm, fs, cells, y});
+    return bias ? run(EpLinearRowsGate<true, false>{bias, add_rows, fm, fs, cells, y})
+                : run(EpLinearRowsGate<false, false>{bias, add_rows, fm, fs, cells, y});
+}
+
+template <int NT>
+static GateSumMat<NT> gate_sum_of(const float* const* fms, const float* fs, const int32_t* cells, int K)
+{
+    GateSumMat<NT> m;
+    for (int l = 0; l < 4; ++l) m.fm[l] = fms[l < NT ? l : 0];
+    m.fs = fs; m.cells = cells; m.D = K;
+    return m;
+}
+
+extern "C" int smin_gate_sum_rows_fwd(void* stream, const float* const* fms, int nfm, const float* fs, const int32_t* cells, const float* W,
+                                      int R, int O, int K, float* y)
+{
+    SMIN_REQUIRE(O % 4 == 0 && K % 4 == 0 && nfm >= 1 && nfm <= 4 && fs != nullptr && cells != nullptr && g_gemm_mode != 3);
+    if (R == 0) return 0;
+    hipStream_t st = (hipStream_t)stream;
+    const EpLinearRows<false, false, false> ep{nullptr, nullptr, nullptr, 1, y};
+    switch (nfm) {
+    case 1: return launch_gemm_nt(st, gate_sum_of<1>(fms, fs, cells, K), PlainMat{W, K}, ep, R, O, K);
+    case 2: return launch_gemm_nt(st, gate_sum_of<2>(fms, fs, cells, K), PlainMat{W, K}, ep, R, O, K);
+    case 3: return launch_gemm_nt(st, gate_sum_of<3>(fms, fs, cells, K), PlainMat{W, K}, ep, R, O, K);
+    default: return launch_gemm_nt(st, gate_sum_of<4>(fms, fs, cells, K), PlainMat{W, K}, ep, R, O, K);
+    }
+}
+
+extern "C" int smin_gate_sum_rows_bwd_w(void* stream, const float* dy, const float* const* fms, int nfm, const float* fs, const int32_t* cells,
+                                        int R, int O, int K, float* dW, void* ws, size_t ws_bytes)
+{
+    hipStream_t st = (hipStream_t)stream;
+    SMIN_REQUIRE(O % 4 == 0 && K % 4 == 0 && nfm >= 1 && nfm <= 4 && dW != nullptr && g_gemm_mode != 3);
+    if (R == 0) { (void)hipMemsetAsync(dW, 0, sizeof(float) * (size_t)O * K, st); return 0; }
+    SMIN_REQUIRE(fs != nullptr && cells != nullptr && ws_bytes >= smin_linear_rows_bwd_workspace_bytes(R, O, K));
+    const int sp = tn_splits(R, O, K);
+    float* slab = reinterpret_cast<float*>(ws);
+    float* bslab = slab + (size_t)sp * O * K;
+    int rc;
+    switch (nfm) {
+    case 1: rc = launch_gemm_tn(st, PlainMat{dy, O}, gate_sum_of<1>(fms, fs, cells, K), slab, bslab, R, O, K, sp); break;
+    case 2: rc = launch_gemm_tn(st, PlainMat{dy, O}, gate_sum_of<2>(fms, fs, cells, K), slab, bslab, R, O, K, sp); break;
+    case 3: rc = launch_gemm_tn(st, PlainMat{dy, O}, gate_sum_of<3>(fms, fs, cells, K), slab, bslab, R, O, K, sp); break;
+    default: rc = launch_gemm_tn(st, PlainMat{dy, O}, gate_sum_of<4>(fms, fs, cells, K), slab, bslab, R, O, K, sp); break;
+    }
+    if (rc) return rc;
+    return launch_reduce_slabs2(st, slab, dW, O * K, nullptr, nullptr, O, sp);
+}
+
 extern "C" size_t smin_linear_rows_bwd_workspace_bytes(int R, int O, int Ktot)
 {
     const int sp = R > 0 ? tn_splits(R, O, Ktot) : 1;
diff --git a/video-moment-localization_amd/csrc/score_tail.hip b/video-moment-localization_amd/csrc/score_tail.hip
--- a/video-moment-localization_amd/csrc/score_tail.hip
+++ b/video-moment-localization_amd/csrc/score_tail.hip
@@ -44,10 +44,6 @@
     }
 }
 
-__device__ __forceinline__ float4 gate4(float4 x, float4 s)
-{
-    return make_float4(x.x / (1.0f + expf(-x.x * s.x)), x.y / (1.0f + expf(-x.y * s.y)), x.z / (1.0f + expf(-x.z * s.z)), x.w / (1.0f + expf(-x.w * s.w)));
-}
 __device__ __forceinline__ float tail_dot4(float acc, float4 a, float4 c, float4 w, float4 bi, float4 bj, float4 q, float4 h, float4 x)
 {
     acc = fmaf(a.x, bi.x * bj.x, acc); acc = fmaf(c.x, q.x + h.x, acc); acc = fmaf(w.x, x.x, acc);
diff --git a/video-moment-localization_amd/csrc/torch_binding.cpp b/video-moment-localization_amd/csrc/torch_binding.cpp
--- a/video-moment-localization_amd/csrc/torch_binding.cpp
+++ b/video-moment-localization_amd/csrc/torch_binding.cpp
@@ -333,7 +333,13 @@
 
 struct SminCore : torch::autograd::Function<SminCore> {
     enum { F_OVERLAP_BOUNDARY = 1, F_OVERLAP_PREP = 2, F_ASYNC_WEIGHTS = 4, F_BF16_OPERANDS = 8, F_GRAD_SYNC = 16, F_TAIL_SPLIT = 32, F_KEEP_ATTENTION = 64,
-           F_ATTN_PACKED = 128, F_INPUT_GRADS = 256, F_PARAM_PREP_KERNEL = 512 };
+           F_ATTN_PACKED = 128, F_INPUT_GRADS = 256, F_PARAM_PREP_KERNEL = 512, F_STORE_GATE = 1024, F_STORE_GATE_BUT_LAST = 2048 };
+    static int gate_mode(int64_t flags, int64_t nl)
+    {
+        if (const char* e = getenv("SMIN_GATE_MODE_EXPERIMENT")) return atoi(e);
+        if ((flags & F_STORE_GATE) != 0 || nl > 5 || smin_get_gemm_mode() == 3) return 1;
+        return (flags & F_STORE_GATE_BUT_LAST) ? 2 : 0;
+    }
     enum { N_FIXED = 14 };
 
     static int64_t run(CoreState& st, std::vector<Tensor>& all, std::vector<Tensor>& cmaps, std::vector<Tensor>& bmaps, bool scoring, const Tensor& video_features,
@@ -523,19 +529,25 @@
         const bool cc_bf16 = bf16_operands && dl % 8 == 0;
         const bool keep_maps = (flags & F_KEEP_ATTENTION) != 0;
         TORCH_CHECK(!(scoring && keep_maps), "smin_score keeps no attention maps");
+        const int gmode = gate_mode(flags, nl);
+        auto fms_before = [&](int64_t k, const float* (&out)[4]) { for (int64_t l = 0; l < k; ++l) out[l] = fp(st.layer[l].fm); };
         for (int64_t k = 0; k < nl; ++k) {
             LayerState& ls = st.layer[k];
             const bool lastl = k == nl - 1;
             ls.fm = fm; ls.fb = fb;
-            ls.hbar = at::empty_like(fm);
-            ls.Hs = Hs;
-            if (k > 0 && !lastl && N > 0) {
-                Tensor Hs_next = at::empty_like(fm);
-                SMIN_CK(smin_gate_fwd_sum(cur(), fp(fm), fp(fs), ip(cells), n, D, fpm(ls.hbar), fp(Hs), fpm(Hs_next)));
-                Hs = Hs_next;
-            } else {
-                SMIN_CK(smin_gate_fwd(cur(), fp(fm), fp(fs), ip(cells), n, D, fpm(ls.hbar)));
-                if (!lastl) Hs = Hs.defined() ? Hs + ls.hbar : ls.hbar;
+            const bool store_gate = gmode == 1 || (gmode == 2 && !lastl);
+            if (gmode != 0) ls.Hs = Hs;
+            if (store_gate) {
+                ls.hbar = at::empty_like(fm);
+                ls.Hs = Hs;
+                if (k > 0 && !lastl && N > 0) {
+                    Tensor Hs_next = at::empty_like(fm);
+                    SMIN_CK(smin_gate_fwd_sum(cur(), fp(fm), fp(fs), ip(cells), n, D, fpm(ls.hbar), fp(Hs), fpm(Hs_next)));
+                    Hs = Hs_next;
+                } else {
+                    SMIN_CK(smin_gate_fwd(cur(), fp(fm), fp(fs), ip(cells), n, D, fpm(ls.hbar)));
+                    if (!lastl) Hs = Hs.defined() ? Hs + ls.hbar : ls.hbar;
+                }
             }
             Tensor bmap = keep_maps ? at::empty({B, L, Nq}, opt) : Tensor();
             wait_stream(side, curs);
@@ -543,9 +555,9 @@
                 StreamScope sc(side);
                 ls.bu = at::empty_like(fb); ls.Qb = at::empty_like(fb); ls.baq = at::empty_like(fb); ls.bqv = at::empty_like(fb); ls.Kb = at::empty_like(fw);
                 ls.P = at::empty({B, L, Nq}, opt); ls.A = at::empty({B, L, L}, opt);
-                SMIN_CK(smin_boundary_unit_fwd(cur(), fp(fb), fp(fw), fp(fs), fp(ls.hbar), ip(cells), ip(row_ptr), n, B, Li, Nq, D, fp(lp(k, L_BQ_W)), fp(lp(k, L_BQ_B)),
-                                               fp(lp(k, L_BK_W)), fp(lp(k, L_BK_B)), fp(qmf), fp(lmf), fpm(ls.bu), fpm(ls.Qb), fpm(ls.Kb), fpm(ls.P), fpm(ls.baq),
-                                               fpm(ls.bqv), fpm(ls.A)));
+                SMIN_CK((store_gate ? smin_boundary_unit_fwd : smin_boundary_unit_fwd_fm)(
+                    cur(), fp(fb), fp(fw), fp(fs), store_gate ? fp(ls.hbar) : fp(fm), ip(cells), ip(row_ptr), n, B, Li, Nq, D, fp(lp(k, L_BQ_W)), fp(lp(k, L_BQ_B)),
+                    fp(lp(k, L_BK_W)), fp(lp(k, L_BK_B)), fp(qmf), fp(lmf), fpm(ls.bu), fpm(ls.Qb), fpm(ls.Kb), fpm(ls.P), fpm(ls.baq), fpm(ls.bqv), fpm(ls.A)));
                 if (keep_maps)
                     TORCH_CHECK(hipMemcpyAsync(bmap.data_ptr(), ls.P.const_data_ptr(), sizeof(float) * ls.P.numel(), hipMemcpyDeviceToDevice, side.stream()) == hipSuccess,
                                 "hipMemcpyAsync failed");
@@ -557,8 +569,14 @@
                 Tensor hp;
                 if (lo == 0) {
                     hp = at::empty({N, dl}, opt);
-                    const float* xs[1] = {fp(Hs_k)};
-                    SMIN_CK(smin_linear_rows_fwd(cur(), xs, 1, fp(lp(k, L_CH_W)), nullptr, nullptr, nullptr, 1, n, dl, D, fpm(hp)));
+                    if (gmode != 0) {
+                        const float* xs[1] = {fp(Hs_k)};
+                        SMIN_CK(smin_linear_rows_fwd(cur(), xs, 1, fp(lp(k, L_CH_W)), nullptr, nullptr, nullptr, 1, n, dl, D, fpm(hp)));
+                    } else {
+                        const float* fms[4];
+                        fms_before(k, fms);
+                        SMIN_CK(smin_gate_sum_rows_fwd(cur(), fms, i32(k), fp(fs), ip(cells), fp(lp(k, L_CH_W)), n, dl, D, fpm(hp)));
+                    }
                 }
                 const int nseg = i32(std::min<int64_t>(4, k - lo));
                 Tensor y = at::empty({N * C, dl}, opt);
@@ -604,7 +622,8 @@
             ls.cum = at::empty({N, D}, opt);
             {
                 const float* xs[1] = {fp(ls.ccmean)};
-                SMIN_CK(smin_linear_rows_fwd(cur(), xs, 1, fp(lp(k, L_C_W)), fp(lp(k, L_C_B)), fp(cumean), fp(ls.hbar), 1, n, D, dl, fpm(ls.cum)));
+                if (store_gate) SMIN_CK(smin_linear_rows_fwd(cur(), xs, 1, fp(lp(k, L_C_W)), fp(lp(k, L_C_B)), fp(cumean), fp(ls.hbar), 1, n, D, dl, fpm(ls.cum)));
+                else SMIN_CK(smin_linear_rows_gate_fwd(cur(), xs[0], fp(lp(k, L_C_W)), fp(lp(k, L_C_B)), fp(cumean), fp(fm), fp(fs), ip(cells), n, D, dl, fpm(ls.cum)));
             }
             wait_stream(curs, side);
             const bool x1h = bf16_operands;
@@ -624,6 +643,7 @@
             if (scoring) {
                 LayerState keep;
                 keep.cc = ls.cc;
+                if (gmode == 0) keep.fm = ls.fm;
                 ls = keep;
             }
         }
@@ -650,7 +670,9 @@
         visit_state(st, [&](Tensor& t) { flat.push_back(t); });
         for (auto& p : all) flat.push_back(p);
         ctx->save_for_backward(flat);
-        ctx->saved_data["d"] = std::vector<int64_t>{N, T, L, C, nl, flags, H, Nq_in};
+        const int gmode = gate_mode(flags, nl);
+        const int64_t flags_bwd = (flags & ~(int64_t)(F_STORE_GATE | F_STORE_GATE_BUT_LAST)) | (gmode == 1 ? F_STORE_GATE : gmode == 2 ? F_STORE_GATE_BUT_LAST : 0);
+        ctx->saved_data["d"] = std::vector<int64_t>{N, T, L, C, nl, flags_bwd, H, Nq_in};
         if (!keep_maps) return {pm, psea[0], psea[1], psea[2]};
         if (flags & F_ATTN_PACKED) cmaps.push_back(cellmap.clone());
         variable_list out{pm, psea[0], psea[1], psea[2]};
@@ -664,7 +686,7 @@
     {
         auto d = ctx->saved_data["d"].toIntVector();
         const int64_t N = d[0], T = d[1], L = d[2], C = d[3], nl = d[4], flags = d[5], H = d[6], Nq_in = d[7];
-        const bool prep_kernel = (flags & F_PARAM_PREP_KERNEL) != 0;
+        const bool prep_kernel = (flags & F_PARAM_PREP_KERNEL) != 0, gate_all = (flags & F_STORE_GATE) != 0, gate_but_last = (flags & F_STORE_GATE_BUT_LAST) != 0;
         auto sv = ctx->get_saved_variables();
         CoreState st;
         size_state(st, nl);
@@ -772,6 +794,7 @@
         hipEvent_t boundary_done = nullptr;
         for (int64_t k = nl - 1; k >= 0; --k) {
             LayerState& ls = st.layer[k];
+            const bool store_gate = gate_all || (gate_but_last && k < nl - 1);
             Tensor dcum = at::empty({N, D}, opt), dfb_mu = at::empty({B, L, D}, opt);
             keep.push_back(dfm); keep.push_back(dcum);
             {
@@ -806,9 +829,10 @@
                 Tensor dfw = at::empty_like(fw), dfs = at::empty_like(fs);
                 Tensor dWq = at::empty({D, D}, opt), dbq = at::empty({D}, opt), dWk = at::empty({D, D}, opt), dbk = at::empty({D}, opt);
                 auto ws = scratch(smin_boundary_unit_bwd_ws_bytes(B, Li, Nq, D), dev);
-                SMIN_CK(smin_boundary_unit_bwd(cur(), fp(dbu), fp(ls.fb), fp(fw), fp(fs), fp(ls.hbar), ip(cells), ip(row_ptr), n, B, Li, Nq, D, fp(trk(k, TR_BQ)), fp(trk(k, TR_BK)),
-                                               fp(qmf), fp(lmf), fp(ls.Qb), fp(ls.Kb), fp(ls.P), fp(ls.baq), fp(ls.bqv), fp(ls.A), fpm(dfb_k), fpm(dfw), fpm(dfs), nullptr,
-                                               fpm(dWq), fpm(dbq), fpm(dWk), fpm(dbk), ws.p, ws.n));
+                SMIN_CK((store_gate ? smin_boundary_unit_bwd : smin_boundary_unit_bwd_fm)(
+                    cur(), fp(dbu), fp(ls.fb), fp(fw), fp(fs), store_gate ? fp(ls.hbar) : fp(ls.fm), ip(cells), ip(row_ptr), n, B, Li, Nq, D, fp(trk(k, TR_BQ)),
+                    fp(trk(k, TR_BK)), fp(qmf), fp(lmf), fp(ls.Qb), fp(ls.Kb), fp(ls.P), fp(ls.baq), fp(ls.bqv), fp(ls.A), fpm(dfb_k), fpm(dfw), fpm(dfs), nullptr,
+                    fpm(dWq), fpm(dbq), fpm(dWk), fpm(dbk), ws.p, ws.n));
                 dlp(k, L_BQ_W) = dWq; dlp(k, L_BQ_B) = dbq; dlp(k, L_BK_W) = dWk; dlp(k, L_BK_B) = dbk;
                 sync.reduce({dWq, dbq, dWk, dbk}, side);
                 dfs_parts.push_back(dfs); dfw_parts.push_back(dfw);
@@ -851,7 +875,7 @@
                 keep.push_back(dhp);
                 SMIN_CK(smin_group_sum(cur(), fp(dchat[k]), n, Ci, dl, fpm(dhp)));
                 dHs[k] = at::empty({N, D}, opt);
-                const float* xs[1] = {fp(ls.Hs)}; float* dxs[1] = {fpm(dHs[k])};
+                const float* xs[1] = {nullptr}; float* dxs[1] = {fpm(dHs[k])};
                 auto ws = scratch(smin_linear_rows_bwd_workspace_bytes(n, dl, D), dev);
                 SMIN_CK(smin_linear_rows_bwd(cur(), fp(dhp), xs, 1, fp(trk(k, TR_CH)), n, dl, D, dxs, nullptr, nullptr, ws.p, ws.n));
             }
@@ -884,9 +908,15 @@
                 }
                 if (k > 0) {
                     Tensor dWch = at::empty_like(lp(k, L_CH_W));
-                    const float* xs[1] = {fp(ls.Hs)};
                     auto ws = scratch(smin_linear_rows_bwd_workspace_bytes(n, dl, D), dev);
-                    SMIN_CK(smin_linear_rows_bwd(cur(), fp(dhp), xs, 1, nullptr, n, dl, D, nullptr, fpm(dWch), nullptr, ws.p, ws.n));
+                    if (gate_all || gate_but_last) {
+                        const float* xs[1] = {fp(ls.Hs)};
+                        SMIN_CK(smin_linear_rows_bwd(cur(), fp(dhp), xs, 1, nullptr, n, dl, D, nullptr, fpm(dWch), nullptr, ws.p, ws.n));
+                    } else {
+                        const float* fms[4];
+                        for (int64_t l = 0; l < k; ++l) fms[l] = fp(st.layer[l].fm);
+                        SMIN_CK(smin_gate_sum_rows_bwd_w(cur(), fp(dhp), fms, i32(k), fp(fs), ip(cells), n, dl, D, fpm(dWch), ws.p, ws.n));
+                    }
                     if (prep_kernel) base_ch[k] = dWch; else acc(dlp(k, L_CH_W), dWch);
                 }
             }
@@ -1132,7 +1162,7 @@
 std::tuple<Tensor, Tensor, Tensor, Tensor, std::vector<Tensor>, std::vector<Tensor>> smin_forward(
     const Tensor& video_features, const Tensor& video_mask, const Tensor& query_features, const Tensor& query_mask_in, const Tensor& length_mask,
     const Tensor& moment_mask, at::TensorList prm, int64_t T, int64_t L, int64_t C, int64_t num_smi_layers, int64_t max_query_length, int64_t lstm_hidden_size,
-    bool overlap_boundary, bool overlap_prep, bool param_prep_kernel, bool async_weights, bool bf16_operand_storage, bool grad_sync,
+    bool store_gate, bool overlap_boundary, bool overlap_prep, bool param_prep_kernel, bool async_weights, bool bf16_operand_storage, bool grad_sync,
     std::optional<int64_t> known_cell_count, bool tail_split, bool input_grads, std::optional<c10::string_view> attention)
 {
     TORCH_CHECK(video_features.is_cuda(), "smin_forward runs on a HIP device only (there is no CPU fallback)");
@@ -1149,7 +1179,7 @@
                           (param_prep_kernel ? SminCore::F_PARAM_PREP_KERNEL : 0) | (async_weights ? SminCore::F_ASYNC_WEIGHTS : 0) |
                           (bf16_operand_storage ? SminCore::F_BF16_OPERANDS : 0) | (grad_sync ? SminCore::F_GRAD_SYNC : 0) |
                           (tail_split ? SminCore::F_TAIL_SPLIT : 0) | (input_grads ? SminCore::F_INPUT_GRADS : 0) |
-                          (attention ? SminCore::F_KEEP_ATTENTION : 0) | (packed ? SminCore::F_ATTN_PACKED : 0);
+                          (attention ? SminCore::F_KEEP_ATTENTION : 0) | (packed ? SminCore::F_ATTN_PACKED : 0) | (store_gate ? SminCore::F_STORE_GATE : 0);
     auto out = SminCore::apply(video_features, video_mask, query_features, query_mask, length_mask, moment_mask, T, L, C, nl, maxq, lstm_hidden_size, flags,
                                known_cell_count.value_or(-1), prm);
     const int64_t nc = attention ? nl + (packed ? 1 : 0) : 0, nb = attention ? nl : 0;
@@ -1161,7 +1191,7 @@
 std::tuple<Tensor, Tensor, Tensor, Tensor> smin_score(
     const Tensor& video_features, const Tensor& video_mask, const Tensor& query_features, const Tensor& query_mask_in, const Tensor& length_mask,
     const Tensor& moment_mask, at::TensorList prm, int64_t T, int64_t L, int64_t C, int64_t num_smi_layers, int64_t max_query_length, int64_t lstm_hidden_size,
-    bool overlap_boundary, bool overlap_prep, bool param_prep_kernel, bool bf16_operand_storage, std::optional<int64_t> known_cell_count)
+    bool store_gate, bool overlap_boundary, bool overlap_prep, bool param_prep_kernel, bool bf16_operand_storage, std::optional<int64_t> known_cell_count)
 {
     TORCH_CHECK(video_features.is_cuda(), "smin_score runs on a HIP device only (there is no CPU fallback)");
     at::NoGradGuard no_grad;
@@ -1170,7 +1200,8 @@
     TORCH_CHECK((int64_t)prm.size() == P_LAYER0 + nl * L_COUNT + 8, "smin_score: expected ", P_LAYER0 + nl * L_COUNT + 8, " parameters, got ", prm.size());
     c10::hip::HIPGuard device_guard(video_features.device().index());
     const int64_t flags = (overlap_boundary ? SminCore::F_OVERLAP_BOUNDARY : 0) | (overlap_prep ? SminCore::F_OVERLAP_PREP : 0) |
-                          (param_prep_kernel ? SminCore::F_PARAM_PREP_KERNEL : 0) | (bf16_operand_storage ? SminCore::F_BF16_OPERANDS : 0);
+                          (param_prep_kernel ? SminCore::F_PARAM_PREP_KERNEL : 0) | (bf16_operand_storage ? SminCore::F_BF16_OPERANDS : 0) |
+                          (store_gate ? SminCore::F_STORE_GATE : 0);
     CoreState st;
     std::vector<Tensor> all, cmaps, bmaps;
     SminCore::run(st, all, cmaps, bmaps, true, video_features.detach(), video_mask, query_features.detach(), query_mask, length_mask, moment_mask, T, L, C, nl,
@@ -1310,11 +1341,11 @@
 TORCH_LIBRARY(smin_hip, m)
 {
     m.def("smin_forward(Tensor video_features, Tensor video_mask, Tensor query_features, Tensor query_mask, Tensor length_mask, Tensor moment_mask, "
-          "Tensor[] params, int T, int L, int C, int num_smi_layers, int max_query_length, int lstm_hidden_size, *, bool overlap_boundary, "
+          "Tensor[] params, int T, int L, int C, int num_smi_layers, int max_query_length, int lstm_hidden_size, bool store_gate=False, *, bool overlap_boundary, "
           "bool overlap_prep, bool param_prep_kernel, bool async_weights, bool bf16_operand_storage, bool grad_sync, int? known_cell_count, "
           "bool tail_split, bool input_grads, str? attention) -> (Tensor, Tensor, Tensor, Tensor, Tensor[], Tensor[])", &smin_forward);
     m.def("smin_score(Tensor video_features, Tensor video_mask, Tensor query_features, Tensor query_mask, Tensor length_mask, Tensor moment_mask, "
-          "Tensor[] params, int T, int L, int C, int num_smi_layers, int max_query_length, int lstm_hidden_size, *, bool overlap_boundary, "
+          "Tensor[] params, int T, int L, int C, int num_smi_layers, int max_query_length, int lstm_hidden_size, bool store_gate=False, *, bool overlap_boundary, "
           "bool overlap_prep, bool param_prep_kernel, bool bf16_operand_storage, int? known_cell_count) -> (Tensor, Tensor, Tensor, Tensor)", &smin_score);
     m.def("smin_encode_videos(Tensor video_features, Tensor video_mask, Tensor[] params) -> Tensor", &smin_encode_videos);
     m.def("smin_encode_queries(Tensor query_features, Tensor query_mask, Tensor[] params, int max_query_length, int lstm_hidden_size) -> (Tensor, Tensor)",
diff --git a/video-moment-localization_amd/modules.py b/video-moment-localization_amd/modules.py
--- a/video-moment-localization_amd/modules.py
+++ b/video-moment-localization_amd/modules.py
@@ -389,6 +389,7 @@
     tail_split = True
     grad_sync = False
     bf16_operand_storage = True
+    store_gate = False
     content_stream = True
     overlap_boundary = True
     overlap_prep = True
@@ -529,7 +530,7 @@
             query_mask = query_mask_rows(query_features, query_mask, self.max_query_length)
             return _lib.load_torch().smin_score(
                 video_features, video_mask, query_features, query_mask, length_mask, moment_mask, self._native_params(), self.T, self.L, self.C,
-                len(self.smis), self.max_query_length, self.lstm_hidden_size, **self._score_options())
+                len(self.smis), self.max_query_length, self.lstm_hidden_size, store_gate=self.store_gate, **self._score_options())
 
     def _record_attention(self, maps):
         for smi, (cmap, bmap) in zip(self.smis, maps):
@@ -563,7 +564,8 @@
         if plan == "node":
             pm, ps, pe, pa, content, boundary = _lib.load_torch().smin_forward(
                 video_features, video_mask, query_features, query_mask, length_mask, moment_mask, self._native_params(), self.T, self.L, self.C,
-                len(self.smis), self.max_query_length, self.lstm_hidden_size, **self._node_options(None if maps is None else maps.mode))
+                len(self.smis), self.max_query_length, self.lstm_hidden_size, store_gate=self.store_gate,
+                **self._node_options(None if maps is None else maps.mode))
             if maps is not None:
                 if maps.mode == "packed":
                     maps.cellmap, content = content[-1], content[:-1]
```
